# pyranha-labs/hypergrep

Measured on AMD Instinct MI355X. Metric: GiB/s scanned (256 patterns, 32 GiB synthetic log per GPU, text resident in HBM), higher is better.
Workload: dtype u8

## Files before the change

hypergrep_amd/csrc/hg_always_on.hip:

```cpp
#include <hip/hip_runtime.h>

#include "hg_confirm_dev.h"
#include "hg_core.h"
#include "hg_engine.h"
#include "hg_sink_dev.h"
#include "hg_tables_dev.h"

namespace {

__device__ __forceinline__ uint32_t wave_inclusive_scan(uint32_t v, uint32_t lane) {
#pragma unroll
  for (int o = 1; o < 64; o <<= 1) {
    uint32_t u = __shfl_up(v, o, 64);
    if (lane >= static_cast<uint32_t>(o)) v += u;
  }
  return v;
}

}

__global__ __launch_bounds__(256) void hg_always_on_kernel(HgConfirmArgs a, uint32_t first, uint32_t last) {
  __shared__ uint32_t s_n, s_base;
  if (threadIdx.x == 0) s_n = 0;
  __syncthreads();
  const uint64_t seg0 = static_cast<uint64_t>(blockIdx.x) * a.hit_seg_cap;
  const HitSink sink{a.tmp_hits + seg0, a.tmp_aux + seg0, a.hit_seg_cap, &s_n};
  const uint32_t lane = threadIdx.x & 63u;
  const uint64_t waves = (static_cast<uint64_t>(gridDim.x) * blockDim.x) >> 6;
  for (uint64_t tile = a.tile_begin + ((static_cast<uint64_t>(blockIdx.x) * blockDim.x + threadIdx.x) >> 6); tile < a.tile_end; tile += waves) {
    const uint64_t lo = (tile << HG_TILE_SHIFT) + lane * 256ull;
    uint64_t hi = lo + 256;
    if (hi > a.nbytes) hi = a.nbytes;
    uint32_t cnt = 0;
    for (uint64_t s = lo; s < hi; s++) cnt += a.text[s] == '\n';
    uint32_t rank = wave_inclusive_scan(cnt, lane) - cnt;
    for (uint64_t s = lo; s < hi; s++) {
      const bool starts = s == 0 || a.text[s - 1] == '\n';
      if (starts)
        hg_scan_line_always_on(a.db, a.text, a.nbytes, a.sums, a.bases, a.bs1, s, rank, first, last,
                               [&](uint32_t pi, uint64_t line_no, uint32_t to, uint64_t start, uint32_t len) {
                                 sink.push(a, line_no, a.db.patterns[pi].id, to, start, len, pi, a.db.patterns[pi].single != 0);
                               });
      rank += a.text[s] == '\n';
    }
  }
  flush_hits(a, &s_n, &s_base);
}

struct AlwaysOnCtx {
  const uint8_t *text;
  uint64_t nbytes;
  HgDeferred *list;
  uint32_t list_cap;
  hgdev::lds_u32 *list_count;
};
__device__ __forceinline__ void always_on_note(const AlwaysOnCtx &cx, uint32_t pi, uint64_t end, uint32_t rank_at_last) {
  const uint32_t slot = __hip_atomic_fetch_add(cx.list_count, 1u, __ATOMIC_RELAXED, __HIP_MEMORY_SCOPE_WORKGROUP);
  if (slot < cx.list_cap) cx.list[slot] = HgDeferred{end, pi, rank_at_last};
}

template <int NW, bool SIMPLE>
__device__ __forceinline__ void always_on_segment(const AlwaysOnCtx &a, const HgPattern &p, uint32_t pi, const hgdev::lds_u32 *tab, uint64_t lo, uint64_t hi,
                                                  uint64_t line_start, uint64_t bs1, uint32_t rank_lo) {
  if (lo >= hi) return;
  const hgdev::lds_u32 *reach = tab + CT_REACH, *follow = tab + CT_FOLLOW, *amask = tab + CT_AMASK, *acct = tab + CT_ACC;
  const uint8_t *text = a.text;
  uint64_t q = line_start;
  if (p.max_len && p.max_len <= HG_ALWAYS_ON_FAST_MAX_LEN) {
    const uint32_t lead = p.max_len - 1;
    q = lo > lead ? lo - lead : 0;
  } else if (lo - line_start >= bs1) {
    q = line_start + (lo - line_start) / bs1 * bs1;
  }
  const uint64_t base = q & ~15ull;
  const uint32_t first = static_cast<uint32_t>(q - base), own = static_cast<uint32_t>(lo - base), stop = static_cast<uint32_t>(hi - base);
  const bool text_ends = hi >= a.nbytes;
  uint32_t S[NW], I[NW];
#pragma unroll
  for (int u = 0; u < NW; u++) { S[u] = 0; I[u] = SIMPLE ? p.init_word : tab[CT_INIT + u]; }
  uint32_t pc = HG_PC_START;
  if (q) {
    const uint32_t before = text[q - 1];
    pc = (before == '\n' || before == 0) ? HG_PC_START : hg_prev_ctx(before);
  }
  constexpr uint32_t NO_BREAK = 0xFFFFFFFFu;
  uint32_t next_break = NO_BREAK;
  auto break_after = [&](uint64_t piece_start) {
    const uint64_t at = piece_start + bs1 - base;
    return at < 0x7FFFFFFFull ? static_cast<uint32_t>(at) : NO_BREAK;
  };
  if (q >= line_start) {
    const uint64_t d = q - line_start, k = d < bs1 ? 0 : d / bs1;
    next_break = break_after(line_start + k * bs1);
    if (k && d == k * bs1) pc = HG_PC_START;
  }
  uint32_t rank = rank_lo;
  bool reported = false;
  const bool single = p.single != 0;
  const uint32_t acc_all = p.acc_all;
  auto load16 = [&](uint32_t at) { return (at <= stop && base + at < a.nbytes) ? *reinterpret_cast<const uint4 *>(text + base + at) : make_uint4(0, 0, 0, 0); };
  uint4 chunk = make_uint4(0, 0, 0, 0), ahead = load16(0);
#pragma unroll 1
  for (uint32_t off = 0; off <= stop; off += 4) {
    if ((off & 15u) == 0) {
      chunk = ahead;
      ahead = load16(off + 16);
    }
    const uint32_t sel = (off >> 2) & 3u;
    const uint32_t v = sel == 0 ? chunk.x : (sel == 1 ? chunk.y : (sel == 2 ? chunk.z : chunk.w));
    uint32_t rc[4][NW];
#pragma unroll
    for (uint32_t i = 0; i < 4; i++)
#pragma unroll
      for (int u = 0; u < NW; u++) rc[i][u] = reach[((v >> (8 * i)) & 0xFFu) * NW + u];
#pragma unroll
    for (uint32_t i = 0; i < 4; i++) {
      const uint32_t r = off + i;
      if (r < first || r > stop) continue;
      const bool beyond = r == stop;
      const uint32_t c = (beyond && text_ends) ? 0u : ((v >> (8 * i)) & 0xFFu);
      if (r == next_break) {
        if (!SIMPLE) {
// ... 697 lines not shown
#pragma unroll
          for (uint32_t k = 0; k < 4; k++) {
            const uint32_t at = b + 16 * k;
            uint32_t m = hgdev::eq_mask16(v[k], 0x0a0a0a0au);
            if (at + 16 > seg) m &= at < seg ? (1u << (seg - at)) - 1u : 0u;
            cnt += __popc(m);
            if (m) after_last = seg_off + at + (31 - __clz(m)) + 1;
          }
        }
      }
      rank_lo = wave_inclusive_scan(cnt, lane) - cnt;
      const HgTileBase tb = a.bases[tile];
      uint32_t prev = after_last;
#pragma unroll
      for (int o = 1; o < 64; o <<= 1) {
        const uint32_t up = __shfl_up(prev, o, 64);
        if (lane >= static_cast<uint32_t>(o) && up > prev) prev = up;
      }
      prev = __shfl_up(prev, 1, 64);
      if (lane == 0) prev = 0;
      line_start = prev ? tile_start + prev : tb.cs;
    }
    for (uint32_t u = 0; u < nunits; u++) {
      if (!one_unit) {
        __syncthreads();
        always_on_stage(tab, a, u, threadIdx.x);
        __syncthreads();
      }
      if (!have) continue;
      AoUnit unit;
      bool ctx;
      if (u < ngroups) {
        const HgSlowGroup &g = a.db.groups[u];
        unit = AoUnit{g.init_word, g.acc_all, g.max_len, g.nmembers, g.single_mask, g.nnodes};
        ctx = g.ctx_off != 0;
      } else {
        const uint32_t pi = a.db.slow[a.db.nslow_grouped + (u - ngroups)];
        const HgPattern &p = a.db.patterns[pi];
        if (!p.simple && p.nw != 1) {
          always_on_word2(cx, p, pi, tab, lo, hi, line_start, a.bs1, rank_lo);
          continue;
        }
        unit = AoUnit{p.init_word, p.acc_all, p.max_len, 1u, p.single ? 1u : 0u, p.nnodes};
        ctx = !p.simple;
      }
      const uint32_t nt = (unit.nnodes + 7u) >> 3;
      const bool shift_form = nt >= 2 && tab[CT_SHIFT] <= 2u;
      if (shift_form) {
        if (ctx) always_on_word<true, 0>(cx, unit, tab, lo, hi, line_start, a.bs1, rank_lo);
        else always_on_word<false, 0>(cx, unit, tab, lo, hi, line_start, a.bs1, rank_lo);
      } else if (ctx) {
        if (nt <= 1) always_on_word<true, 1>(cx, unit, tab, lo, hi, line_start, a.bs1, rank_lo);
        else if (nt == 2) always_on_word<true, 2>(cx, unit, tab, lo, hi, line_start, a.bs1, rank_lo);
        else if (nt == 3) always_on_word<true, 3>(cx, unit, tab, lo, hi, line_start, a.bs1, rank_lo);
        else always_on_word<true, 4>(cx, unit, tab, lo, hi, line_start, a.bs1, rank_lo);
      } else {
        if (nt <= 1) always_on_word<false, 1>(cx, unit, tab, lo, hi, line_start, a.bs1, rank_lo);
        else if (nt == 2) always_on_word<false, 2>(cx, unit, tab, lo, hi, line_start, a.bs1, rank_lo);
        else if (nt == 3) always_on_word<false, 3>(cx, unit, tab, lo, hi, line_start, a.bs1, rank_lo);
        else always_on_word<false, 4>(cx, unit, tab, lo, hi, line_start, a.bs1, rank_lo);
      }
    }
  }
  __syncthreads();
  if (threadIdx.x == 0) {
    const uint32_t n = s_n;
    a.always_count[blockIdx.x] = n < list_cap ? n : list_cap;
    if (n > list_cap) atomicMax(&a.counters[HG_CNT_DEFER_NEED], static_cast<uint32_t>((static_cast<uint64_t>(n) * gridDim.x + HG_DEFER_SHARDS - 1) / HG_DEFER_SHARDS));
  }
}

__global__ __launch_bounds__(256) void hg_always_on_finish_kernel(HgConfirmArgs a) {
  __shared__ uint32_t s_n, s_base;
  if (threadIdx.x == 0) s_n = 0;
  __syncthreads();
  const uint64_t seg0 = static_cast<uint64_t>(blockIdx.x) * a.hit_seg_cap;
  const HitSink sink{a.tmp_hits + seg0, a.tmp_aux + seg0, a.hit_seg_cap, &s_n};
  const HgDeferred *list = a.deferred + static_cast<uint64_t>(blockIdx.x) * a.always_list_cap;
  const uint32_t n = a.always_count[blockIdx.x];
  for (uint32_t i = threadIdx.x; i < n; i += blockDim.x) {
    const HgDeferred d = list[i];
    const uint64_t end = d.pos, pos = end - 1;
    hgdev::PieceView pv;
    if (!hgdev::piece_view(a.text, a.nbytes, a.sums, a.bases, a.bs1, pos, d.rank, pos, &pv)) continue;
    if (!pv.whole) {
      if (pv.a > pos) continue;
      bool blocked = false;
      for (uint64_t i = pv.a; i < pos && !blocked; i++) blocked = a.text[i] == 0;
      if (blocked) continue;
    }
    const uint64_t z = a.text[pos] == '\n' ? end : hgdev::scanned_end(a.text, end, pv.limit);
    const HgPattern &pat = a.db.patterns[d.pattern];
    sink.push(a, pv.line_no, pat.id, static_cast<uint32_t>(end - pv.a), pv.a, static_cast<uint32_t>(z - pv.a), d.pattern, pat.single != 0);
  }
  flush_hits(a, &s_n, &s_base);
}
```

hypergrep_amd/csrc/hg_confirm_dev.h:

```cpp
#pragma once
#include <hip/hip_runtime.h>

#include "hg_core.h"

namespace hgdev {

using lds_u32 = __attribute__((address_space(3))) uint32_t;

__device__ __forceinline__ uint32_t load_u32_unaligned(const uint8_t *text, uint64_t off) {
  const uint32_t *p = reinterpret_cast<const uint32_t *>(text + (off & ~3ull));
  const uint32_t sh = static_cast<uint32_t>(off & 3u) * 8u;
  const uint32_t lo = p[0];
  if (sh == 0) return lo;
  return (lo >> sh) | (p[1] << (32u - sh));
}

__device__ __forceinline__ uint32_t byte_of(const uint4 &v, uint32_t i) {
  const uint32_t w = i < 8 ? (i < 4 ? v.x : v.y) : (i < 12 ? v.z : v.w);
  return (w >> ((i & 3u) * 8u)) & 0xFFu;
}
__device__ __forceinline__ uint32_t eq_mask16(const uint4 &v, uint32_t c4) {
  const uint32_t m0 = hg_zero_bytes(v.x ^ c4), m1 = hg_zero_bytes(v.y ^ c4), m2 = hg_zero_bytes(v.z ^ c4), m3 = hg_zero_bytes(v.w ^ c4);
#ifdef HG_EQMASK_BITWISE
  auto pack = [](uint32_t m) { return ((m >> 7) & 1u) | ((m >> 14) & 2u) | ((m >> 21) & 4u) | ((m >> 28) & 8u); };
// ... 36 lines not shown
      uint64_t c = base + 16u * j;
      if (c < chunk || c >= end) c = chunk;
      v[j] = *reinterpret_cast<const uint4 *>(text + c);
    }
#pragma unroll
    for (int j = 0; j < 4; j++) {
      const uint64_t c = base + 16u * j;
      if (c < chunk) continue;
      if (c >= end) return;
      if (visit(c, v[j])) return;
    }
    chunk = base + 64u;
  }
}

__device__ __forceinline__ uint64_t line_start_in_tile(const uint8_t *text, uint64_t tile_start, uint64_t pos) {
  uint64_t s = tile_start;
  walk_back4(text, (pos - 1) & ~15ull, tile_start, [&](uint64_t chunk, const uint4 &v) {
    uint32_t m = eq_mask16(v, 0x0a0a0a0au);
    if (chunk + 16 > pos) m &= (1u << static_cast<uint32_t>(pos - chunk)) - 1u;
    if (!m) return false;
    s = chunk + (31 - __clz(m)) + 1;
    return true;
  });
  return s;
}

__device__ __forceinline__ uint64_t scanned_end(const uint8_t *text, uint64_t from, uint64_t limit) {
  uint64_t z = limit;
  walk_fwd4(text, from & ~15ull, limit, [&](uint64_t chunk, const uint4 &v) {
    const uint32_t lo = chunk < from ? static_cast<uint32_t>(from - chunk) : 0u;
    const uint32_t hi = limit - chunk < 16 ? static_cast<uint32_t>(limit - chunk) : 16u;
    const uint32_t range = ((1u << hi) - 1u) & ~((1u << lo) - 1u);
    const uint32_t nl = eq_mask16(v, 0x0a0a0a0au) & range, nul = eq_mask16(v, 0u) & range;
    if (!(nl | nul)) return false;
    const uint32_t e = __ffs(nl | nul) - 1;
    z = chunk + (((nl >> e) & 1u) ? e + 1 : e);
    return true;
  });
  return z;
}

struct LineHead {
  uint64_t s;
  uint64_t a;
  bool blocked;
};
__device__ __forceinline__ LineHead line_head(const uint8_t *text, uint64_t tile_start, uint64_t carry_start, uint32_t rank, uint64_t upto) {
  const uint64_t floor = rank == 0 ? carry_start : tile_start;
  LineHead h{floor, upto, false};
  bool nul_above = false;
  if (upto > floor) {
    walk_back4(text, (upto - 1) & ~15ull, floor & ~15ull, [&](uint64_t chunk, const uint4 &v) {
      const uint32_t hi = upto - chunk < 16 ? static_cast<uint32_t>(upto - chunk) : 16u;
      uint32_t range = (1u << hi) - 1u;
      if (chunk < floor) range &= ~((1u << static_cast<uint32_t>(floor - chunk)) - 1u);
      bool stop = false;
      if (rank > 0) {
        const uint32_t nl = eq_mask16(v, 0x0a0a0a0au) & range;
        if (nl) {
          const uint32_t q = 31 - __clz(nl);
          h.s = chunk + q + 1;
          range &= ~((2u << q) - 1u);
          stop = true;
        }
      }
      const uint32_t zero = eq_mask16(v, 0u);
      const uint32_t nul = zero & range, data = ~zero & range;
      if (data) {
        if (nul_above || (nul && (data & ((1u << (31 - __clz(nul))) - 1u)))) h.blocked = true;
        h.a = chunk + (__ffs(data) - 1);
      }
      if (nul) nul_above = true;
      return stop || (h.blocked && rank == 0);
    });
  }
  return h;
}

struct PieceView {
  uint64_t line_no, a, limit;
  bool whole;
};
__device__ __forceinline__ bool piece_view(const uint8_t *text, uint64_t nbytes, const HgTileSum *sums, const HgTileBase *bases, uint64_t bs1, uint64_t pos,
                                           uint32_t rank, uint64_t upto, PieceView *out) {
  const uint64_t t = pos >> HG_TILE_SHIFT, tile_start = t << HG_TILE_SHIFT;
  const HgTileBase tb = bases[t];
  const LineHead h = line_head(text, tile_start, tb.cs, rank, upto);
  const uint64_t k = (pos - h.s) / bs1;
  const uint64_t ps = h.s + k * bs1;
  out->limit = ps + bs1 < nbytes ? ps + bs1 : nbytes;
  out->line_no = hg_line_index(text, sums[t], tb, tile_start, rank, h.s, bs1, bs1 < HG_TILE_BYTES) + k;
  out->whole = k == 0;
  if (k == 0) {
    if (h.blocked) return false;
    out->a = h.a;
    return true;
  }
  uint64_t a = ps;
  while (a < out->limit && text[a] == 0) a++;
  out->a = a;
  return a < out->limit;
}

template <typename Emit>
__device__ __forceinline__ void confirm_literal(const uint8_t *text, uint64_t nbytes, const HgTileSum *sums, const HgTileBase *bases, uint64_t bs1,
                                                uint64_t pos, uint32_t rank, uint64_t fs, uint32_t len, Emit &&emit) {
  const uint32_t last_byte = text[fs + len - 1];
  PieceView pv;
  if (!piece_view(text, nbytes, sums, bases, bs1, pos, rank, fs, &pv)) return;
  const uint64_t from = fs + len;
  if (from > pv.limit) return;
  uint64_t a = pv.a;
  if (!pv.whole) {
    if (a > fs) return;
    for (uint64_t i = a; i < fs; i++)
      if (text[i] == 0) return;
  }
  const uint64_t z = last_byte == '\n' ? from : scanned_end(text, from, pv.limit);
  emit(pv.line_no, static_cast<uint32_t>(from - a), a, static_cast<uint32_t>(z - a));
}

struct MatchWindow {
  uint64_t line_no, a, limit, q;
  uint32_t pc;
};
__device__ __forceinline__ bool match_window(const uint8_t *text, uint64_t nbytes, const HgTileSum *sums, const HgTileBase *bases, uint64_t bs1, uint64_t pos,
                                             uint32_t rank, uint64_t fs, uint32_t lead, MatchWindow *w) {
  PieceView pv;
  if (!piece_view(text, nbytes, sums, bases, bs1, pos, rank, pos, &pv)) return false;
  if (!pv.whole) {
    if (pv.a > pos) return false;
    for (uint64_t i = pv.a; i < pos; i++)
      if (text[i] == 0) return false;
  }
  if (fs < pv.a) return false;
  w->line_no = pv.line_no;
  w->a = pv.a;
  w->limit = pv.limit;
  w->q = (lead != 0xFFFFFFFFu && fs - pv.a > lead) ? fs - lead : pv.a;
  w->pc = w->q == pv.a ? static_cast<uint32_t>(HG_PC_START) : hg_prev_ctx(text[w->q - 1]);
  return true;
}
__device__ __forceinline__ uint64_t window_scanned_end(const uint8_t *text, uint64_t e, uint64_t limit) {
  return text[e - 1] == '\n' ? e : scanned_end(text, e, limit);
}

template <typename Emit>
__device__ __forceinline__ void confirm_simple(const uint8_t *text, uint64_t nbytes, const HgTileSum *sums, const HgTileBase *bases, uint64_t bs1, uint64_t pos,
                                                   uint32_t rank, uint64_t fs, uint32_t lead, uint32_t init, uint32_t acc, const lds_u32 *reach, const lds_u32 *follow,
                                                   Emit &&emit) {
  MatchWindow w;
  if (!match_window(text, nbytes, sums, bases, bs1, pos, rank, fs, lead, &w)) return;
  const uint64_t a = w.a, limit = w.limit, q = w.q;
  uint32_t S = 0, first_to = HG_NONE32;
  bool alive = true;
  for (uint64_t chunk = q & ~15ull; chunk < limit && alive; chunk += 16) {
    const uint4 v = *reinterpret_cast<const uint4 *>(text + chunk);
    const uint32_t lo = chunk < q ? static_cast<uint32_t>(q - chunk) : 0u;
    const uint32_t hi = limit - chunk < 16 ? static_cast<uint32_t>(limit - chunk) : 16u;
    const uint32_t below_lo = (1u << lo) - 1u;
    const uint32_t nl = eq_mask16(v, 0x0a0a0a0au) & ~below_lo, nul = eq_mask16(v, 0u) & ~below_lo;
    uint32_t end = hi;
    bool stop = false;
    const uint32_t stops = (nl | nul) & ((1u << hi) - 1u);
    if (stops) {
      const uint32_t e = __ffs(stops) - 1;
      end = ((nl >> e) & 1u) ? e + 1 : e;
      stop = true;
    }
    uint32_t r[16];
#pragma unroll
    for (int i = 0; i < 16; i++) r[i] = reach[byte_of(v, i)];
#pragma unroll
    for (int i = 0; i < 16; i++) {
      if (static_cast<uint32_t>(i) >= lo && static_cast<uint32_t>(i) < end && alive) {
        const uint64_t at = chunk + i;
        uint32_t T = at <= fs ? init : 0u;
        for (uint32_t x = S; x; x &= x - 1) T |= follow[__ffs(x) - 1];
        S = T & r[i];
        if (S & acc) {
          first_to = static_cast<uint32_t>(at + 1 - a);
          alive = false;
        } else if (S == 0 && at >= fs) {
          alive = false;
        }
      }
    }
    if (stop || hi < 16) break;
  }
  if (first_to != HG_NONE32) {
    const uint64_t z = window_scanned_end(text, a + first_to, limit);
    emit(w.line_no, first_to, a, static_cast<uint32_t>(z - a));
  }
}

template <int NW, typename Emit>
__device__ __forceinline__ void confirm_ctx(const uint8_t *text, uint64_t nbytes, const HgTileSum *sums, const HgTileBase *bases, uint64_t bs1, uint64_t pos,
                                                uint32_t rank, uint64_t fs, uint32_t lead, const lds_u32 *reach, const lds_u32 *follow, const lds_u32 *init,
                                                const lds_u32 *amask, const lds_u32 *acct, Emit &&emit) {
  MatchWindow w;
  if (!match_window(text, nbytes, sums, bases, bs1, pos, rank, fs, lead, &w)) return;
  const uint64_t a = w.a, limit = w.limit, q = w.q;
  uint32_t S[NW], I[NW];
#pragma unroll
  for (int u = 0; u < NW; u++) { S[u] = 0; I[u] = init[u]; }
  uint32_t pc = w.pc, first_to = HG_NONE32;
  bool alive = true;
  uint64_t z = limit;
  for (uint64_t chunk = q & ~15ull; chunk < limit && alive; chunk += 16) {
    const uint4 v = *reinterpret_cast<const uint4 *>(text + chunk);
    const uint32_t lo = chunk < q ? static_cast<uint32_t>(q - chunk) : 0u;
    const uint32_t hi = limit - chunk < 16 ? static_cast<uint32_t>(limit - chunk) : 16u;
    const uint32_t below_lo = (1u << lo) - 1u;
    const uint32_t nl = eq_mask16(v, 0x0a0a0a0au) & ~below_lo, nul = eq_mask16(v, 0u) & ~below_lo;
    uint32_t end = hi;
    bool stop = false;
    const uint32_t stops = (nl | nul) & ((1u << hi) - 1u);
    if (stops) {
      const uint32_t e = __ffs(stops) - 1;
      end = ((nl >> e) & 1u) ? e + 1 : e;
      stop = true;
    }
#pragma unroll
    for (int i = 0; i < 16; i++) {
      if (static_cast<uint32_t>(i) >= lo && static_cast<uint32_t>(i) < end && alive) {
        const uint64_t at = chunk + i;
        const uint32_t c = byte_of(v, i);
        const uint32_t cc = c == '\n' ? HG_NC_NLFINAL : (hg_is_word(c) ? HG_NC_WORD : HG_NC_OTHER);
        const lds_u32 *ac = acct + (pc * 5 + cc) * NW, *am = amask + (pc * 4 + cc) * NW, *rc = reach + c * NW;
        uint32_t hit = 0;
#pragma unroll
        for (int u = 0; u < NW; u++) hit |= S[u] & ac[u];
        if (hit) {
          first_to = static_cast<uint32_t>(at - a);
          alive = false;
        } else {
          uint32_t T[NW];
#pragma unroll
          for (int u = 0; u < NW; u++) T[u] = at <= fs ? I[u] : 0u;
#pragma unroll
          for (int u = 0; u < NW; u++)
            for (uint32_t x = S[u]; x; x &= x - 1) {
              const lds_u32 *f = follow + (u * 32 + (__ffs(x) - 1)) * NW;
#pragma unroll
              for (int k = 0; k < NW; k++) T[k] |= f[k];
            }
          uint32_t any = 0;
#pragma unroll
          for (int u = 0; u < NW; u++) any |= S[u] = T[u] & rc[u] & am[u];
          pc = hg_prev_ctx(c);
          if (any == 0 && at >= fs) alive = false;
        }
      }
    }
    if (stop || hi < 16) {
      z = chunk + end;
      break;
    }
  }
  if (first_to == HG_NONE32 && alive) {
    const lds_u32 *ac = acct + (pc * 5 + HG_NC_END) * NW;
    uint32_t hit = 0;
#pragma unroll
    for (int u = 0; u < NW; u++) hit |= S[u] & ac[u];
    if (hit) {
      first_to = static_cast<uint32_t>(z - a);
      emit(w.line_no, first_to, a, static_cast<uint32_t>(z - a));
    }
    return;
  }
  if (first_to != HG_NONE32) {
    const uint64_t e = a + first_to;
    emit(w.line_no, first_to, a, static_cast<uint32_t>((e > a ? window_scanned_end(text, e, limit) : scanned_end(text, e, limit)) - a));
  }
}

}
```

hypergrep_amd/csrc/hg_core.h:

```cpp
#pragma once
#include "hg_db.h"

constexpr uint32_t HG_TILE_BYTES = 16384;
constexpr uint32_t HG_TILE_SHIFT = 14;
constexpr uint32_t HG_NONE32 = 0xFFFFFFFFu;

struct HgTileSum {
  uint32_t nl_count;
  uint32_t first_nl;
  uint32_t last_nl;
  uint32_t inner;
};
struct HgTileBase {
  uint64_t cs;
  uint64_t L;
};
struct HgCand {
  uint64_t pos;
  uint32_t word;
  uint32_t rank;
};
struct HgHit {
  uint64_t line_no;
  uint32_t id;
  uint32_t to;
};
struct HgHitAux {
  uint64_t start;
  uint32_t len;
  uint32_t pattern;
};

struct HgDbView {
  const HgPattern *patterns;
  const uint32_t *pool;
  const HgFactor *factors;
  const HgWindow *windows;
  const uint32_t *bucket_off;
  const uint16_t *disc;
  const uint32_t *bucket_off2;
  const HgWindow *windows2;
  const HgWinBucket *wtab;
  uint32_t wtab_mask;
  uint32_t wtab_first;
  const uint32_t *slow;
  uint32_t npatterns, nslow, fold_mask;
  uint32_t window_mask;
  uint32_t nslow_fast;
  uint32_t nslow_grouped;
  uint32_t nslow_huge;
  uint32_t ngroups;
  const HgSlowGroup *groups;
  const uint32_t *bounds;
};

constexpr uint32_t HG_BOUND_NONE = 0x7FFFFFFFu;

HG_HD uint32_t hg_zero_bytes(uint32_t x) {
  uint32_t y = ((x & 0x7f7f7f7fu) + 0x7f7f7f7fu) | x;
  return ~y & 0x80808080u;
}
HG_HD uint32_t hg_newline_mask(uint32_t w) { return hg_zero_bytes(w ^ 0x0a0a0a0au); }

HG_HD uint32_t hg_popc(uint32_t x) {
#if defined(__HIP_DEVICE_COMPILE__)
  return __popc(x);
#else
  return static_cast<uint32_t>(__builtin_popcount(x));
#endif
}
HG_HD uint32_t hg_clz32(uint32_t x) {
#if defined(__HIP_DEVICE_COMPILE__)
  return static_cast<uint32_t>(__clz(static_cast<int>(x)));
#else
  return static_cast<uint32_t>(__builtin_clz(x));
#endif
}
HG_HD uint32_t hg_ctz(uint32_t x) {
#if defined(__HIP_DEVICE_COMPILE__)
  return __ffs(x) - 1;
#else
  return static_cast<uint32_t>(__builtin_ctz(x));
#endif
}

constexpr uint32_t HG_CONFIRM_MODES = 5;
HG_HD uint32_t hg_confirm_mode(const HgPattern &p) {
  if (p.nw > HG_MAX_W) return 4;
  if (p.single && p.literal_only) return 0;
  if (p.single && p.simple) return 1;
  if (p.single && p.nw <= 2) return 2;
  return 3;
}

HG_HD uint32_t hg_prev_ctx(uint32_t c) { return c == '\n' ? HG_PC_NL : (hg_is_word(c) ? HG_PC_WORD : HG_PC_OTHER); }

HG_HD void hg_disc_range(const HgDbView &db, const uint8_t *text, uint64_t nbytes, uint64_t pos, uint32_t folded, uint32_t *j0, uint32_t *j1) {
  const uint32_t h = hg_hash_window(folded);
  const uint32_t d = db.disc[h];
  const uint32_t sel = d >> 8;
  uint32_t key = 0;
  *j0 = *j1 = 0;
  if (sel) {
    const int64_t at = static_cast<int64_t>(pos) + static_cast<int8_t>(d & 0xFFu);
    const uint32_t lo = hg_ctz(sel), hi = 31u - hg_clz32(sel);
    if (at + static_cast<int64_t>(lo) < 0 || static_cast<uint64_t>(at + hi) >= nbytes) return;
    uint32_t v = 0;
    for (uint32_t b = lo; b <= hi; b++) v |= static_cast<uint32_t>(text[at + b]) << (8 * b);
    key = (v | db.fold_mask) & hg_disc_bytes(sel);
  }
  const uint32_t h2 = hg_disc_bucket(h, key);
  *j0 = db.bucket_off2[h2];
  *j1 = db.bucket_off2[h2 + 1];
}

template <typename Emit>
HG_HD void hg_verify_window(const HgDbView &db, const uint8_t *text, uint64_t nbytes, uint64_t pos, uint32_t w,
                            Emit &&emit) {
  uint32_t folded = (w | db.fold_mask) & db.window_mask;
  auto check = [&](uint32_t factor_off) {
    uint32_t off = factor_off & 0xff;
    const HgFactor &f = db.factors[factor_off >> 8];
    if (pos < off) return;
    uint64_t start = pos - off;
    if (start + f.len > nbytes) return;
    for (uint32_t b = 0; b < f.len; b++)
      if ((text[start + b] ^ f.lit[b]) & hg_factor_cmask(f, b)) return;
    emit(f.pattern, start, f.len);
  };
  const uint32_t owner = hg_wtab_find(db.wtab, db.wtab_mask, folded);
  if (owner == HG_WTAB_EMPTY) return;
  if (owner != HG_WTAB_SHARED) {
    check(owner);
    return;
  }
  uint32_t j0, j1;
  hg_disc_range(db, text, nbytes, pos, folded, &j0, &j1);
  for (uint32_t j = j0; j < j1; j++) {
    HgWindow win = db.windows2[j];
    if (win.value != folded) continue;
    check(win.factor_off);
  }
}

HG_HD uint64_t hg_pieces(uint64_t len, uint64_t bs1) { return (len + bs1 - 1) / bs1; }

HG_HD uint64_t hg_inner_pieces(const uint8_t *text, uint64_t from, uint64_t to, uint64_t bs1) {
  uint64_t total = 0, start = from;
  for (uint64_t i = from; i < to; i++)
    if (text[i] == '\n') {
      total += hg_pieces(i + 1 - start, bs1);
      start = i + 1;
    }
  return total;
}

HG_HD uint64_t hg_line_index(const uint8_t *text, const HgTileSum &ts, const HgTileBase &tb, uint64_t tile_start, uint32_t rank,
                             uint64_t s, uint64_t bs1, bool small) {
  if (rank == 0) return tb.L;
  uint64_t after_first = tile_start + ts.first_nl + 1;
  uint64_t base = tb.L + hg_pieces(after_first - tb.cs, bs1);
  if (!small) return base + (rank - 1);
  return base + hg_inner_pieces(text, after_first, s, bs1);
}

HG_HD void hg_trim_piece(const uint8_t *text, uint64_t ps, uint64_t limit, uint64_t &a, uint64_t &z) {
  a = ps;
  while (a < limit && text[a] == 0) a++;
  z = a;
  while (z < limit) {
    uint32_t c = text[z];
    if (c == 0) break;
    z++;
    if (c == '\n') break;
  }
}

struct HgHugeView {
  uint32_t nw, ncls, ctxfree, init_hi;
  const uint32_t *cls;
  const uint32_t *reach;
  const uint32_t *init, *smask, *xsrc, *xrank, *xlist, *xt;
  const uint32_t *amask;
  const uint32_t *acc;
};
HG_HD HgHugeView hg_huge_view(const uint32_t *pool, const HgPattern &p) {
  const HgHugeHeader *h = reinterpret_cast<const HgHugeHeader *>(pool + p.follow_off);
  HgHugeView v;
  v.nw = p.nw;
  v.ncls = h->ncls;
  v.ctxfree = h->ctxfree;
  v.init_hi = h->init_hi;
  v.cls = pool + h->cls_off;
  v.reach = pool + p.reach_off;
  v.init = pool + p.init_off;
  v.smask = pool + h->smask_off;
  v.xsrc = pool + h->xsrc_off;
  v.xrank = pool + h->xrank_off;
  v.xlist = pool + h->xlist_off;
  v.xt = pool + h->xt_off;
  v.amask = pool + p.amask_off;
  v.acc = pool + p.acc_off;
  return v;
}
HG_HD uint32_t hg_huge_class(const HgHugeView &v, uint32_t c) { return (v.cls[c >> 2] >> ((c & 3u) * 8u)) & 0xFFu; }
HG_HD const uint32_t *hg_huge_acc(const HgHugeView &v, uint32_t pc, uint32_t nc) { return v.ctxfree ? v.acc : v.acc + (pc * 5 + nc) * v.nw; }
HG_HD uint32_t hg_bits_from(uint32_t lo) { return 0xFFFFFFFFu << (lo & 31u); }
HG_HD uint32_t hg_bits_upto(uint32_t hi) { return 0xFFFFFFFFu >> (31u - (hi & 31u)); }

#if !defined(__HIP_DEVICE_COMPILE__)
template <typename Emit>
inline void hg_huge_scan_slice(const uint32_t *pool, const HgPattern &p, const uint8_t *data, uint64_t len, uint64_t from, uint64_t upto, Emit &&emit) {
  const HgHugeView v = hg_huge_view(pool, p);
  const uint32_t nw = v.nw;
  const bool single = p.single != 0;
  uint32_t *S = new uint32_t[2 * static_cast<size_t>(nw)](), *T = S + nw;
  uint32_t pc = from ? hg_prev_ctx(data[from - 1]) : HG_PC_START;
  bool alive = false;
  auto any_accept = [&](const uint32_t *a) {
    uint32_t any = 0;
    for (uint32_t w = 0; w < nw; w++) any |= S[w] & a[w];
    return any != 0;
  };
  for (uint64_t i = from; i < len; i++) {
    if (i >= upto && !alive) { delete[] S; return; }
    const uint32_t c = data[i];
    const uint32_t cc = c == '\n' ? (i + 1 == len ? HG_NC_NLFINAL : HG_NC_NL) : (hg_is_word(c) ? HG_NC_WORD : HG_NC_OTHER);
    if (alive && any_accept(hg_huge_acc(v, pc, cc))) {
      emit(static_cast<uint32_t>(i));
      if (single) { delete[] S; return; }
    }
    for (uint32_t w = 0; w < nw; w++) T[w] = i < upto ? v.init[w] : 0u;
    for (uint32_t w = 0; w < nw; w++) {
      const uint32_t x = S[w] & v.smask[w];
      T[w] |= x << 1;
      if (w + 1 < nw) T[w + 1] |= x >> 31;
    }
    for (uint32_t w = 0; w < nw; w++)
      for (uint32_t x = S[w] & v.xsrc[w]; x; x &= x - 1) {
        const uint32_t b = hg_ctz(x), k = v.xrank[w] + hg_popc(v.xsrc[w] & ((1u << b) - 1u));
        for (uint32_t r = v.xlist[k]; r < v.xlist[k + 1]; r++) {
          const uint32_t lo = v.xt[2 * r], hi = v.xt[2 * r + 1];
          for (uint32_t tw = lo >> 5; tw <= (hi >> 5); tw++)
            T[tw] |= (tw == (lo >> 5) ? hg_bits_from(lo) : 0xFFFFFFFFu) & (tw == (hi >> 5) ? hg_bits_upto(hi) : 0xFFFFFFFFu);
        }
      }
    const uint32_t *r = v.reach + hg_huge_class(v, c) * nw, *m = v.ctxfree ? nullptr : v.amask + (pc * 4 + cc) * nw;
// ... 404 lines not shown
}

template <typename Emit>
HG_HD uint32_t hg_flow_som_write(const uint32_t *pool, const HgPattern &p, const uint8_t *data, uint32_t len, bool close, uint32_t hdr, uint32_t *S,
                                 HgSomStarts *st, HgSomStarts *tmp, int32_t *carried, Emit &&emit) {
  uint32_t pc = hdr & HG_FLOW_PC;
  bool held = (hdr & HG_FLOW_HELD) != 0, acc_done = (hdr & HG_FLOW_ACC_DONE) != 0;
  int32_t stop = held ? -1 : 0;
  if (len > 0) {
    if (held) {
      hg_flow_som_unhold(pool, p, S, st, tmp, &pc, -1, false, acc_done, emit);
      acc_done = false;
    }
    const bool held_now = !close && data[len - 1] == '\n' && (hdr & HG_FLOW_HOLD);
    const uint32_t stop_w = held_now ? len - 1 : len;
    if (stop_w > 0) {
      hg_flow_som_scan(pool, p, data, 0, stop_w, close ? len - 1 : HG_NONE32, S, st, tmp, pc, acc_done, emit);
      pc = hg_prev_ctx(data[stop_w - 1]);
      acc_done = false;
    }
    held = held_now;
    stop = static_cast<int32_t>(stop_w);
  }
  *carried = stop;
  hdr = hg_flow_som_finish(pool, p, S, st, tmp, pc, hdr, stop, held, acc_done, close, emit);
  if (close) *carried = 0;
  return hdr;
}

HG_HD void hg_flow_som_load(const uint32_t *words, uint32_t width, const uint32_t *S, uint32_t nw, int64_t pos, HgSomStarts st) {
  for (uint32_t w = 0; w < nw; w++)
    for (uint32_t x = S[w]; x; x &= x - 1) {
      const uint32_t t = w * 32 + hg_ctz(x);
      uint64_t v;
      bool sat;
      if (width == 2) {
        v = (words[t >> 1] >> ((t & 1u) * 16u)) & 0xFFFFu;
        sat = v == 0xFFFFu;
      } else if (width == 4) {
        v = words[t];
        sat = v == 0xFFFFFFFFu;
      } else {
        v = words[2 * t] | (static_cast<uint64_t>(words[2 * t + 1]) << 32);
        sat = false;
      }
      st[t] = sat ? HG_SOM_FAR : pos - 1 - static_cast<int64_t>(v);
    }
}
HG_HD uint64_t hg_flow_som_dist(const uint32_t *S, HgSomStarts st, uint32_t t, int64_t pos, uint64_t sat) {
  if (!((S[t >> 5] >> (t & 31u)) & 1u)) return 0;
  if (st[t] == HG_SOM_FAR) return sat;
  const uint64_t d = static_cast<uint64_t>(pos - st[t] - 1);
  return d < sat ? d : sat;
}
HG_HD void hg_flow_som_store(uint32_t *words, uint32_t width, const uint32_t *S, uint32_t nnodes, int64_t pos, HgSomStarts st) {
  const uint32_t n = hg_flow_som_words(nnodes, width);
  for (uint32_t k = 0; k < n; k++) {
    uint32_t v;
    if (width == 2) {
      v = static_cast<uint32_t>(hg_flow_som_dist(S, st, 2 * k, pos, 0xFFFFu));
      if (2 * k + 1 < nnodes) v |= static_cast<uint32_t>(hg_flow_som_dist(S, st, 2 * k + 1, pos, 0xFFFFu)) << 16;
    } else if (width == 4) {
      v = static_cast<uint32_t>(hg_flow_som_dist(S, st, k, pos, 0xFFFFFFFFu));
    } else {
      v = static_cast<uint32_t>(hg_flow_som_dist(S, st, k >> 1, pos, ~0ull) >> ((k & 1u) * 32u));
    }
    words[k] = v;
  }
}

template <typename Emit>
HG_HD void hg_confirm_window(const HgDbView &db, const uint8_t *text, uint64_t nbytes, const HgTileSum *sums, const HgTileBase *bases, uint64_t bs1, uint64_t pos,
                             uint64_t fs, uint32_t pattern, uint32_t rank, Emit &&emit) {
  uint64_t t = pos >> HG_TILE_SHIFT, tile_start = t << HG_TILE_SHIFT;
  uint64_t s;
  if (rank == 0) {
    s = bases[t].cs;
  } else {
    s = pos;
    while (s > tile_start && text[s - 1] != '\n') s--;
  }
  uint64_t k = (pos - s) / bs1;
  uint64_t ps = s + k * bs1;
  uint64_t line_no = hg_line_index(text, sums[t], bases[t], tile_start, rank, s, bs1, bs1 < HG_TILE_BYTES) + k;
  uint64_t limit = ps + bs1 < nbytes ? ps + bs1 : nbytes;
  uint64_t a, z;
  hg_trim_piece(text, ps, limit, a, z);
  if (z <= a || pos < a || pos >= z || fs < a) return;
  const HgPattern &p = db.patterns[pattern];
  const uint64_t q = (p.lit_lead != 0xFFFFFFFFu && fs - a > p.lit_lead) ? fs - p.lit_lead : a;
  hg_nfa_scan_slice(db.pool, p, text + a, static_cast<uint32_t>(z - a), static_cast<uint32_t>(q - a), static_cast<uint32_t>(fs - a + 1),
                    [&](uint32_t to) { emit(line_no, to, a, static_cast<uint32_t>(z - a)); });
}

template <typename Emit, typename Claim>
HG_HD void hg_confirm(const HgDbView &db, const uint8_t *text, uint64_t nbytes, const HgTileSum *sums,
                      const HgTileBase *bases, uint64_t bs1, uint64_t pos, uint32_t pattern, uint32_t rank, Emit &&emit, Claim &&claim) {
  uint64_t t = pos >> HG_TILE_SHIFT, tile_start = t << HG_TILE_SHIFT;
  uint64_t s;
  if (rank == 0) {
    s = bases[t].cs;
  } else {
    s = pos;
    while (s > tile_start && text[s - 1] != '\n') s--;
  }
  uint64_t k = (pos - s) / bs1;
  uint64_t ps = s + k * bs1;
  uint64_t line_no = hg_line_index(text, sums[t], bases[t], tile_start, rank, s, bs1, bs1 < HG_TILE_BYTES) + k;
  uint64_t limit = ps + bs1 < nbytes ? ps + bs1 : nbytes;
  uint64_t a, z;
  hg_trim_piece(text, ps, limit, a, z);
  if (z <= a) return;
  if (!claim(ps)) return;
  const HgPattern &p = db.patterns[pattern];
  hg_nfa_scan(db.pool, p, text + a, z - a, [&](uint32_t to) { emit(line_no, to, a, static_cast<uint32_t>(z - a)); });
}
template <typename Emit>
HG_HD void hg_confirm(const HgDbView &db, const uint8_t *text, uint64_t nbytes, const HgTileSum *sums,
                      const HgTileBase *bases, uint64_t bs1, uint64_t pos, uint32_t pattern, uint32_t rank, Emit &&emit) {
  hg_confirm(db, text, nbytes, sums, bases, bs1, pos, pattern, rank, emit, [](uint64_t) { return true; });
}

template <typename Emit>
HG_HD void hg_scan_line_always_on(const HgDbView &db, const uint8_t *text, uint64_t nbytes, const HgTileSum *sums,
                                  const HgTileBase *bases, uint64_t bs1, uint64_t s, uint32_t rank, uint32_t first, uint32_t last, Emit &&emit) {
  uint64_t t = s >> HG_TILE_SHIFT, tile_start = t << HG_TILE_SHIFT;
  uint64_t line_no = hg_line_index(text, sums[t], bases[t], tile_start, rank, s, bs1, bs1 < HG_TILE_BYTES);
  uint64_t ps = s;
  for (;;) {
    uint64_t limit = ps + bs1 < nbytes ? ps + bs1 : nbytes;
    uint64_t a, z;
    hg_trim_piece(text, ps, limit, a, z);
    if (z > a) {
      for (uint32_t j = first; j < last; j++) {
        uint32_t pi = db.slow[j];
        hg_nfa_scan(db.pool, db.patterns[pi], text + a, z - a,
                    [&](uint32_t to) { emit(pi, line_no, to, a, static_cast<uint32_t>(z - a)); });
      }
    }
    uint64_t e = ps;
    bool nl = false;
    while (e < limit) {
      if (text[e++] == '\n') { nl = true; break; }
    }
    if (nl || e >= nbytes) return;
    ps = e;
    line_no++;
  }
}
```

hypergrep_amd/csrc/hg_engine.h:

```cpp
#pragma once
#include <hip/hip_runtime.h>

#include <memory>
#include <string>

#include "../../include/hypergrep_amd.h"
#include "hg_compile.h"
#include "hg_core.h"
#include "hg_post.h"

#ifndef HG_STREAM_WG_WAVES
#define HG_STREAM_WG_WAVES 8
#endif
constexpr uint32_t HG_STREAM_WG_WAVES_DEFAULT = HG_STREAM_WG_WAVES;

constexpr uint32_t HG_CONFIRM_SPLIT = 4;
constexpr uint32_t HG_DEFER_SHARDS = 64;

struct HgDeferred {
  uint64_t pos;
  uint32_t pattern;
  uint32_t rank;
};
enum { HG_ST_MINLEN_KEPT = 16, HG_ST_FIN_TOTAL = 24, HG_ST_SELECTED = 28, HG_ST_FINAL = 32, HG_ST_WORDS = 36, HG_ST_ZERO_WORDS = 32,
// ... 107 lines not shown
  uint32_t nfeed;
  uint32_t *count;
  const uint64_t *pos;
  HgHit *out_hits;
  HgHitAux *out_aux;
};
hipError_t hg_comb_launch(const HgCombArgs &a, bool emit, hipStream_t stream);

struct HgEngineKnobs {
  uint64_t fin_target = 48;
  bool no_bucket_finalize = false;
  uint64_t chunk_tiles = 0;
  uint32_t max_chunks = 0;
  std::vector<double> chunk_weights;
  long stream_wgs_per_cu = 0;
  long joiner = -1;
  bool joiner_ahead = false;
  bool no_early_finalize = false;
  uint32_t confirm_mode_mask = 0x1F;
  long confirm_blocks_per_cu = 0;
  uint64_t hit_limit = 0;
  uint64_t cand_limit = 0;
  bool verbose = false;
  static HgEngineKnobs from_env();
};

class HgScanner {
 public:
  static int create(std::shared_ptr<const HgDb> db, int device, HgScanner **out, std::string *err);
  const std::shared_ptr<const HgDb> &database() const { return db_; }
  ~HgScanner();
  int scan(const void *d_text, uint64_t nbytes, int buffer_size, uint64_t line_base, hipStream_t stream, HgScanOutput *out);
  int scan_block(const void *d_text, uint64_t nbytes, hipStream_t stream, HgScanOutput *out);
  uint32_t launch_block_small(const uint8_t *h_text, uint32_t nbytes, hipStream_t stream, HgHit *h_out, uint32_t *h_counts, uint32_t *h_flag, uint32_t seq);
  const std::string &last_error() const { return err_; }
  int device() const { return device_; }
  const HgDbView &view() const { return view_; }

 private:
  HgScanner() = default;
  int init();
  int ensure(uint64_t nbytes);
  int alloc_cands(uint64_t n);
  int alloc_hits(uint64_t n);
  int scan_impl(const void *d_text, uint64_t nbytes, int buffer_size, uint64_t line_base, bool block_mode, hipStream_t stream, HgScanOutput *out);
  struct PassRange {
    uint64_t tile_lo, tile_hi, cs0, piece0, own_lo, own_hi;
    bool last;
  };
  int scan_segments(const uint8_t *text, uint64_t nbytes, uint64_t bs1, uint64_t line_base, hipStream_t stream, HgScanOutput *out, uint32_t nsegments);
  int run_fitting(const uint8_t *text, uint64_t nbytes, uint64_t bs1, uint64_t line_base, const PassRange &range, bool block_mode, hipStream_t stream, HgScanOutput *out);
  int run_once(const uint8_t *text, uint64_t nbytes, uint64_t bs1, uint64_t line_base, const PassRange &range, bool block_mode, hipStream_t stream, HgScanOutput *out);
  struct PassPlan;
  PassPlan plan_pass(const uint8_t *text, uint64_t nbytes, uint64_t bs1, uint64_t line_base, const PassRange &range, bool block_mode, hipStream_t stream) const;
  int alloc_fin(uint32_t nb, hipStream_t stream);
  int launch_stream(PassPlan &p, uint32_t c, HgScanOutput *out);
  int launch_side(PassPlan &p, uint32_t c);
  int finalize_last(PassPlan &p, uint32_t c);
  int launch_fin(const PassPlan &p, hipStream_t s, uint32_t lo, uint32_t hi, bool beside_stream = false);
  int regrow(const PassPlan &p, uint64_t n_raw);
  int finalize_compact(const HgHit *hits, const HgHitAux *aux, uint32_t n, uint32_t id_bits, uint32_t to_bits, uint64_t line_bound, hipStream_t stream);
  int comb_pass(HgScanOutput *out, uint64_t bs1, uint64_t line_bound, hipStream_t stream);
  int minlen_pass(const uint8_t *text, uint32_t *n, hipStream_t stream);
  int huge_lds_error() { return error(HG_ERR_HIP, "the huge-automaton kernel cannot have its LDS"); }
  bool fail(hipError_t e, const char *what);
  int error(int rc, const std::string &what) { err_ = what; return rc; }

  HgEngineKnobs knobs_;
  int device_ = 0;
  int num_cus_ = 256;
  int stream_wgs_per_cu_ = 0;
  std::string err_;
  HgDbView view_{};
  std::shared_ptr<const HgDb> db_;
  void *d_disc_ = nullptr, *d_bucket2_ = nullptr, *d_windows2_ = nullptr, *d_groups_ = nullptr, *d_wtab_ = nullptr, *d_bounds_ = nullptr;
  void *d_patterns_ = nullptr, *d_pool_ = nullptr, *d_factors_ = nullptr, *d_windows_ = nullptr, *d_bucket_ = nullptr,
       *d_filter_ = nullptr, *d_ext_ = nullptr, *d_slow_ = nullptr;
  uint64_t cap_tiles_ = 0;
  uint32_t cand_cap_ = 0, hit_cap_ = 0;
  uint64_t chunk_limit_tiles_ = 0;
  uint32_t defer_spread_boost_ = 1;
  bool hit_direct_ = false;
  HgTileSum *d_sums_ = nullptr;
  HgTileBase *d_bases_ = nullptr, *d_block_base_ = nullptr, *d_final_ = nullptr;
  HgTileElem *d_agg_ = nullptr;
  HgCand *d_cands_ = nullptr;
  HgDeferred *d_deferred_ = nullptr;
  uint32_t *d_defer_count_ = nullptr;
  HgHit *d_hits_raw_ = nullptr, *d_hits_out_ = nullptr;
  HgHitAux *d_aux_raw_ = nullptr, *d_aux_out_ = nullptr;
  HgHit *d_acc_hits_ = nullptr;
  HgHitAux *d_acc_aux_ = nullptr;
  uint64_t acc_cap_ = 0;
  bool side_bound_ = false;
  uint64_t *d_key_a_ = nullptr, *d_key_b_ = nullptr;
  uint32_t *d_perm_a_ = nullptr, *d_perm_b_ = nullptr;
  uint8_t *d_keep_ = nullptr;
  uint32_t *d_counters_ = nullptr, *d_selected_ = nullptr, *d_seg_count_ = nullptr;
  uint32_t max_segs_ = 0;
  uint32_t *d_pflags_ = nullptr;
  void *d_temp_ = nullptr;
  size_t temp_bytes_ = 0;
  uint32_t *h_counters_ = nullptr;
  HgTileBase *h_final_ = nullptr;
  hipEvent_t ev_[4] = {nullptr, nullptr, nullptr, nullptr};
  static constexpr int kMaxChunks = 64;
  hipStream_t side_stream_ = nullptr;
  hipEvent_t ev_tile_done_ = nullptr;
  hipEvent_t ev_fin_early_ = nullptr;
  hipEvent_t ev_k1_begin_[kMaxChunks] = {}, ev_k1_end_[kMaxChunks] = {}, ev_side_done_[kMaxChunks] = {};
  uint32_t *d_fin_fill_ = nullptr, *d_fin_kept_ = nullptr, *d_fin_total_ = nullptr, *d_fin_big_ = nullptr;
  bool fin_fallback_ = false;
  uint32_t fin_alloc_ = 0;
  uint32_t fin_epoch_ = 0;
  uint64_t fin_expect_hits_ = 0;
  void *d_huge_claim_ = nullptr;
  uint64_t huge_claim_slots_ = 0;
  uint32_t *d_from_ = nullptr;
  uint64_t from_cap_ = 0;
  uint32_t som_max_nw_ = 0;
  uint32_t *d_min_lengths_ = nullptr;
  HgHit *d_minlen_hits_ = nullptr;
  HgHitAux *d_minlen_aux_ = nullptr;
  uint64_t minlen_cap_ = 0;
  uint32_t minlen_max_nw_ = 0;
  HgComb *d_combs_ = nullptr;
  uint32_t *d_comb_words_ = nullptr, *d_comb_feed_ = nullptr;
  uint32_t *d_comb_count_ = nullptr;
  uint64_t *d_comb_pos_ = nullptr;
  uint64_t comb_in_cap_ = 0;
  HgHit *d_comb_hits_ = nullptr;
  HgHitAux *d_comb_aux_ = nullptr;
  uint64_t comb_out_cap_ = 0;
  uint8_t *d_comb_temp_ = nullptr;
  size_t comb_temp_bytes_ = 0;
  uint32_t *d_seg_count2_ = nullptr;
  HgCand *d_cands2_ = nullptr;
};
```

hypergrep_amd/csrc/hg_engine.hip:

```cpp
#include <algorithm>
#include <array>
#include <cstdio>
#include <cstdlib>
#include <cstring>
#include <memory>

#include "hg_engine.h"
#include "hg_mem.h"

#include <rocprim/rocprim.hpp>

bool hg_launch_stream(const HgStreamArgs &a, uint32_t grid, hipStream_t stream);
bool hg_launch_stream_join(const HgStreamArgs &a, uint32_t grid, hipStream_t stream);
int hg_stream_blocks_per_cu(uint32_t filter_log2, uint32_t filter_wide, uint32_t dense);
__global__ void hg_tile_reduce_kernel(const HgTileSum *sums, uint64_t tile_begin, uint64_t tile_end, uint64_t bs1, HgTileElem *agg);
__global__ void hg_tile_spine_kernel(const HgTileElem *agg, uint32_t nblocks, uint64_t bs1, HgTileBase *block_base, HgTileBase *state);
__global__ void hg_tile_apply_kernel(const HgTileSum *sums, uint64_t tile_begin, uint64_t tile_end, uint64_t bs1, const HgTileBase *block_base,
                                     HgTileBase *bases);
__global__ void hg_tile_inner_kernel(const uint8_t *text, HgTileSum *sums, uint64_t tile_begin, uint64_t tile_end, uint64_t bs1);
__global__ void hg_verify_kernel(HgConfirmArgs a);
__global__ void hg_confirm_fast_kernel(HgConfirmArgs a, uint32_t blocks_per_mode);
__global__ void hg_confirm_generic_kernel(HgConfirmArgs a);
__global__ void hg_always_on_kernel(HgConfirmArgs a, uint32_t first, uint32_t last);
__global__ void hg_always_on_fast_kernel(HgConfirmArgs a);
__global__ void hg_always_on_finish_kernel(HgConfirmArgs a);
__global__ void hg_block_mark_kernel(HgConfirmArgs a, uint32_t *pattern_flags);
__global__ void hg_block_scan_kernel(HgConfirmArgs a, const uint32_t *pattern_flags);
__global__ void hg_block_small_kernel(HgDbView db, const uint8_t *h_text, uint32_t length, HgHit *h_out, uint32_t seg_cap, uint32_t *h_counts, uint32_t *d_done,
                                      uint32_t *h_flag, uint32_t seq, uint32_t ppw);
__global__ void hg_reset_kernel(uint32_t *state, uint32_t state_words, HgTileBase *final_state, uint64_t carry_start, uint64_t first_piece, uint32_t *fill, uint32_t nb, uint32_t *defer_count,
                                uint32_t ndefer);
__global__ void hg_fin_sort_small_kernel(const HgHit *hits, uint32_t *idx, const uint32_t *fill, uint32_t b_lo, uint32_t b_hi, uint32_t cap, uint32_t id_bits,
                                         uint32_t to_bits, uint32_t *kept_count, uint32_t *big_list, uint32_t *big_count, uint32_t big_stride);
template <uint32_t LCAP, bool IN_LDS>
__global__ void hg_fin_sort_big_kernel(const HgHit *hits, uint32_t *idx, const uint32_t *fill, const uint32_t *big_list, const uint32_t *big_count, uint32_t cap,
                                       uint32_t id_bits, uint32_t to_bits, uint32_t *kept_count, uint32_t *overflow, uint64_t *scratch_key, uint32_t *scratch_idx);
template <uint32_t THREADS>
__global__ void hg_fin_scan_kernel(uint32_t *kept_count, uint32_t b_lo, uint32_t b_hi, uint32_t *total, const uint32_t *fill, uint32_t cap, uint32_t *part, uint32_t epoch);
__global__ void hg_confirm_literal_kernel(HgConfirmArgs a);
__global__ void hg_verify_lean_kernel(HgConfirmArgs a);
__global__ void hg_fin_gather_kernel(const HgHit *hits, const HgHitAux *aux, const uint32_t *idx, const uint32_t *kept_base, const uint32_t *total, uint32_t b_lo,
                                     uint32_t b_hi, uint32_t cap, HgHit *oh, HgHitAux *oa);
__global__ void hg_key_kernel(const HgHit *hits, const HgHitAux *aux, const HgPattern *patterns, uint32_t n, uint64_t *key, uint32_t *idx);
__global__ void hg_line_key_kernel(const HgHit *hits, const uint32_t *perm, uint32_t n, uint64_t *key);
__global__ void hg_offset_kernel(uint32_t *idx, uint32_t n, uint32_t add);
__global__ void hg_key_packed_kernel(const HgHit *hits, const HgHitAux *aux, const HgPattern *patterns, uint32_t n, uint32_t id_bits, uint32_t to_bits,
                                     uint64_t *key, uint32_t *idx);
__global__ void hg_keep_kernel(const HgHit *hits, const HgHitAux *aux, const uint32_t *perm, const HgPattern *patterns, uint32_t n, uint8_t *keep);
__global__ void hg_scatter_kernel(const HgHit *hits, const HgHitAux *aux, const uint32_t *perm, const uint8_t *keep, const uint32_t *pos, uint32_t n,
                                  HgHit *oh, HgHitAux *oa, uint32_t *count);

size_t hg_huge_lds_bytes(uint32_t nw_max, uint32_t stage_cap);
bool hg_launch_confirm_huge(const HgConfirmArgs &a, uint32_t grid, uint32_t nw_max, uint32_t stage_cap, void *claim, uint32_t claim_mask, hipStream_t stream);
bool hg_launch_always_on_huge(const HgConfirmArgs &a, uint32_t grid, uint32_t nw_max, uint32_t stage_cap, uint32_t first, uint32_t last, hipStream_t stream);
bool hg_launch_block_huge(const HgConfirmArgs &a, uint32_t grid, uint32_t nw_max, uint32_t stage_cap, const uint32_t *pattern_flags, hipStream_t stream);

namespace {
constexpr int TS_BLOCK_TILES = 1024;
constexpr int STREAM_WG_WAVES = HG_STREAM_WG_WAVES;

template <typename T>
hipError_t upload(void **dst, const std::vector<T> &src, const char *name) {
  size_t bytes = std::max<size_t>(src.size() * sizeof(T), 16);
  hipError_t e = hgmem::dev_alloc(dst, bytes, name);
  if (e != hipSuccess) return e;
  if (!src.empty()) e = hipMemcpy(*dst, src.data(), src.size() * sizeof(T), hipMemcpyHostToDevice);
  return e;
}
template <typename T>
hipError_t realloc_dev(T *&ptr, size_t count, const char *name) {
  hgmem::dev_free(ptr, name);
  ptr = nullptr;
  return hgmem::dev_alloc(&ptr, std::max<size_t>(count * sizeof(T), 16), name);
}
uint32_t bits_for(uint64_t v) {
  uint32_t b = 1;
  while (b < 64 && (v >> b)) b++;
  return b;
}
}

#define HG_TRY(call, what) \
  do { if (fail((call), what)) return HG_ERR_HIP; } while (0)

HgEngineKnobs HgEngineKnobs::from_env() {
  HgEngineKnobs k;
  auto num = [](const char *name, uint64_t dflt) -> uint64_t {
    const char *env = std::getenv(name);
    return env ? std::strtoull(env, nullptr, 10) : dflt;
  };
  k.fin_target = std::max<uint64_t>(4, num("HG_FIN_TARGET", 48));
  k.no_bucket_finalize = std::getenv("HG_NO_BUCKET_FINALIZE") != nullptr;
  k.chunk_tiles = num("HG_CHUNK_TILES", 0);
  k.max_chunks = static_cast<uint32_t>(std::min<uint64_t>(num("HG_MAX_CHUNKS", 0), 1u << 20));
  if (const char *env = std::getenv("HG_CHUNK_WEIGHTS")) {
    for (const char *q = env; *q;) {
      char *e = nullptr;
      const double v = std::strtod(q, &e);
      if (e == q) break;
      if (v > 0) k.chunk_weights.push_back(v);
      q = *e ? e + 1 : e;
    }
  }
  k.stream_wgs_per_cu = static_cast<long>(num("HG_STREAM_WGS_PER_CU", 0));
  if (const char *env = std::getenv("HG_JOINER")) k.joiner = std::max(0l, std::min(2l, std::strtol(env, nullptr, 10)));
  k.joiner_ahead = std::getenv("HG_JOINER_AHEAD") != nullptr;
  k.no_early_finalize = std::getenv("HG_NO_EARLY_FINALIZE") != nullptr;
#ifdef HG_PROFILE_CONFIRM
  if (const char *env = std::getenv("HG_DEBUG_CONFIRM_MODES")) k.confirm_mode_mask = static_cast<uint32_t>(std::strtoul(env, nullptr, 0));
#endif
  k.confirm_blocks_per_cu = static_cast<long>(std::min<uint64_t>(num("HG_CONFIRM_BLOCKS_PER_CU", 0), 16));
  k.hit_limit = num("HG_HIT_LIMIT", 0);
  k.cand_limit = num("HG_CAND_LIMIT", 0);
// ... 4 lines not shown
bool HgScanner::fail(hipError_t e, const char *what) {
  if (e == hipSuccess) return false;
  err_ = std::string(what) + ": " + hipGetErrorString(e);
  return true;
}

int HgScanner::create(std::shared_ptr<const HgDb> db, int device, HgScanner **out, std::string *err) {
  *out = nullptr;
  std::unique_ptr<HgScanner> s(new HgScanner());
  s->device_ = device;
  s->db_ = std::move(db);
  if (int rc = s->init()) {
    if (err) *err = s->err_;
    return rc;
  }
  *out = s.release();
  return HG_OK;
}

int HgScanner::init() {
  if (!db_) return error(HG_ERR_ARG, "no database");
  int count = 0;
  const hipError_t e = hipGetDeviceCount(&count);
  if (e != hipSuccess || count == 0) return error(HG_ERR_HIP, std::string("no HIP device available (") + hipGetErrorString(e) + "); the scan path has no CPU fallback");
  if (device_ < 0 || device_ >= count) return error(HG_ERR_ARG, "device index out of range");
  knobs_ = HgEngineKnobs::from_env();
  const HgDb &db = *db_;
  HG_TRY(hipSetDevice(device_), "hipSetDevice");
  hipDeviceProp_t prop;
  HG_TRY(hipGetDeviceProperties(&prop, device_), "hipGetDeviceProperties");
  num_cus_ = prop.multiProcessorCount;
  HG_TRY(upload(&d_patterns_, db.patterns, "d_patterns_"), "upload patterns");
  HG_TRY(upload(&d_pool_, db.pool, "d_pool_"), "upload tables");
  HG_TRY(upload(&d_factors_, db.factors, "d_factors_"), "upload factors");
  HG_TRY(upload(&d_windows_, db.windows, "d_windows_"), "upload windows");
  HG_TRY(upload(&d_bucket_, db.bucket_off, "d_bucket_"), "upload buckets");
  HG_TRY(upload(&d_disc_, db.disc, "d_disc_"), "upload discriminators");
  HG_TRY(upload(&d_bucket2_, db.bucket_off2, "d_bucket2_"), "upload buckets");
  HG_TRY(upload(&d_windows2_, db.windows2, "d_windows2_"), "upload windows");
  HG_TRY(upload(&d_wtab_, db.wtab, "d_wtab_"), "upload window table");
  HG_TRY(upload(&d_filter_, db.filter, "d_filter_"), "upload filter");
  HG_TRY(upload(&d_ext_, db.ext, "d_ext_"), "upload filter conditions");
  HG_TRY(upload(&d_slow_, db.slow, "d_slow_"), "upload always-on list");
  HG_TRY(upload(&d_groups_, db.groups, "d_groups_"), "upload always-on groups");
  view_.patterns = static_cast<const HgPattern *>(d_patterns_);
  view_.pool = static_cast<const uint32_t *>(d_pool_);
  view_.factors = static_cast<const HgFactor *>(d_factors_);
  view_.windows = static_cast<const HgWindow *>(d_windows_);
  view_.bucket_off = static_cast<const uint32_t *>(d_bucket_);
  view_.disc = static_cast<const uint16_t *>(d_disc_);
  view_.bucket_off2 = static_cast<const uint32_t *>(d_bucket2_);
  view_.windows2 = static_cast<const HgWindow *>(d_windows2_);
  view_.wtab = static_cast<const HgWinBucket *>(d_wtab_);
  view_.wtab_mask = db.wtab_mask;
  view_.wtab_first = db.wtab_first;
  view_.slow = static_cast<const uint32_t *>(d_slow_);
  view_.npatterns = static_cast<uint32_t>(db.patterns.size());
  view_.nslow = static_cast<uint32_t>(db.slow.size());
  view_.nslow_fast = db.nslow_fast;
  view_.nslow_grouped = db.nslow_grouped;
  view_.nslow_huge = db.nslow_huge;
  view_.ngroups = static_cast<uint32_t>(db.groups.size());
  view_.groups = static_cast<const HgSlowGroup *>(d_groups_);
  if (!db.bounds.empty()) HG_TRY(upload(&d_bounds_, db.bounds, "d_bounds_"), "upload offset bounds");
  view_.bounds = static_cast<const uint32_t *>(d_bounds_);
  if (!db.min_lengths.empty()) HG_TRY(upload(reinterpret_cast<void **>(&d_min_lengths_), db.min_lengths, "d_min_lengths_"), "upload min_length");
  for (uint32_t i = 0; i < db.patterns.size(); i++) {
    const HgPattern &p = db.patterns[i];
    if (p.flags & HG_FLAG_SOM_LEFTMOST) som_max_nw_ = std::max(som_max_nw_, p.nw);
    if (!db.min_lengths.empty() && db.min_lengths[i]) minlen_max_nw_ = std::max(minlen_max_nw_, p.nw);
  }
  if (db.comb_pass()) {
    HG_TRY(upload(reinterpret_cast<void **>(&d_combs_), db.combs, "d_combs_"), "upload combinations");
    HG_TRY(upload(reinterpret_cast<void **>(&d_comb_words_), db.comb_words, "d_comb_words_"), "upload combinations");
    HG_TRY(upload(reinterpret_cast<void **>(&d_comb_feed_), db.comb_feed, "d_comb_feed_"), "upload combinations");
  }
  view_.fold_mask = db.fold_mask;
  view_.window_mask = db.window_mask;
  static_assert(HG_CNT_CURSORS == kMaxChunks, "one tile cursor per pipeline chunk");
  HG_TRY(hgmem::dev_alloc(&d_counters_, HG_ST_ALLOC_WORDS * 4, "d_state_"), "alloc state");
  HG_TRY(hipMemset(d_counters_, 0, HG_ST_ALLOC_WORDS * 4), "clear state");
  d_fin_total_ = d_counters_ + HG_ST_FIN_TOTAL;
  d_selected_ = d_counters_ + HG_ST_SELECTED;
  d_final_ = reinterpret_cast<HgTileBase *>(d_counters_ + HG_ST_FINAL);
  HG_TRY(hgmem::dev_alloc(&d_pflags_, db.patterns.size() * 4 + 16, "d_pflags_"), "alloc pattern flags");
  HG_TRY(hgmem::host_alloc(&h_counters_, (HG_CNT_WORDS + 4 + HG_DEFER_SHARDS) * 4, "h_counters_"), "alloc pinned");
  h_final_ = reinterpret_cast<HgTileBase *>(h_counters_ + HG_ST_FINAL);
  for (auto &ev : ev_) HG_TRY(hipEventCreate(&ev), "hipEventCreate");
  HG_TRY(hipStreamCreateWithFlags(&side_stream_, hipStreamNonBlocking), "hipStreamCreate");
  HG_TRY(hipEventCreateWithFlags(&ev_fin_early_, hipEventDisableTiming), "hipEventCreate");
  HG_TRY(hipEventCreateWithFlags(&ev_tile_done_, hipEventDisableTiming), "hipEventCreate");
  return HG_OK;
}

HgScanner::~HgScanner() {
  (void)hipSetDevice(device_);
  void *ptrs[] = {d_patterns_, d_pool_, d_factors_, d_windows_, d_bucket_, d_filter_, d_ext_, d_slow_, d_sums_, d_bases_, d_block_base_,
                  d_agg_, d_cands_, d_hits_raw_, d_hits_out_, d_aux_raw_, d_aux_out_,
                  d_key_a_, d_key_b_, d_perm_a_, d_perm_b_, d_keep_, d_counters_, d_temp_, d_seg_count_, d_pflags_, d_deferred_, d_defer_count_, d_seg_count2_, d_cands2_, d_disc_, d_bucket2_, d_windows2_, d_groups_, d_acc_hits_, d_acc_aux_, d_huge_claim_, d_wtab_, d_from_, d_fin_fill_, d_fin_kept_, d_fin_big_,
                  d_combs_, d_comb_words_, d_comb_feed_, d_comb_count_, d_comb_pos_, d_comb_hits_, d_comb_aux_, d_comb_temp_, d_bounds_,
                  d_min_lengths_, d_minlen_hits_, d_minlen_aux_};
  for (void *p : ptrs) hgmem::dev_free(p, "scanner");
  hgmem::host_free(h_counters_, "h_counters_");
  for (auto &ev : ev_)
    if (ev) (void)hipEventDestroy(ev);
  for (int i = 0; i < kMaxChunks; i++) {
    if (ev_k1_begin_[i]) (void)hipEventDestroy(ev_k1_begin_[i]);
    if (ev_k1_end_[i]) (void)hipEventDestroy(ev_k1_end_[i]);
    if (ev_side_done_[i]) (void)hipEventDestroy(ev_side_done_[i]);
  }
  if (side_stream_) (void)hipStreamDestroy(side_stream_);
  if (ev_fin_early_) (void)hipEventDestroy(ev_fin_early_);
  if (ev_tile_done_) (void)hipEventDestroy(ev_tile_done_);
}

int HgScanner::alloc_cands(uint64_t n) {
  n = std::min<uint64_t>(n, 0x7FFFFFF0u);
  HG_TRY(realloc_dev(d_cands_, n, "d_cands_"), "workspace alloc (candidates)");
  HG_TRY(realloc_dev(d_cands2_, n, "d_cands2_"), "workspace alloc (candidates)");
  uint32_t modes = 0;
  for (uint32_t m = 0; m < HG_CONFIRM_MODES; m++) modes += db_->n_confirm_mode[m] ? 1 : 0;
  HG_TRY(realloc_dev(d_deferred_, std::max<uint64_t>(modes, 1) * n, "d_deferred_"), "workspace alloc (deferred)");
  hgmem::dev_free(d_huge_claim_, "d_huge_claim_");
  d_huge_claim_ = nullptr;
  huge_claim_slots_ = 0;
  if (db_->n_confirm_mode[4]) {
    uint64_t slots = 1u << 12;
    while (slots < 2 * n) slots <<= 1;
    HG_TRY(hgmem::dev_alloc(&d_huge_claim_, slots * 8, "d_huge_claim_"), "workspace alloc (claim table)");
    huge_claim_slots_ = slots;
  }
  cand_cap_ = static_cast<uint32_t>(n);
  return HG_OK;
}

int HgScanner::alloc_hits(uint64_t n64) {
  const uint32_t n = static_cast<uint32_t>(std::min<uint64_t>(n64, 0x7FFFFFF0u));
  auto re = [&](auto *&ptr, size_t count, const char *name) { return fail(realloc_dev(ptr, count, name), "workspace alloc (hits)"); };
  if (re(d_hits_raw_, n, "d_hits_raw_") || re(d_hits_out_, n, "d_hits_out_") || re(d_aux_raw_, n, "d_aux_raw_") || re(d_aux_out_, n, "d_aux_out_") ||
      re(d_key_a_, n, "d_key_a_") || re(d_key_b_, n, "d_key_b_") || re(d_perm_a_, n, "d_perm_a_") || re(d_perm_b_, n, "d_perm_b_") || re(d_keep_, n, "d_keep_"))
    return HG_ERR_HIP;
  hit_cap_ = n;
  size_t t1 = 0, t2 = 0;
  (void)rocprim::radix_sort_pairs(nullptr, t1, d_key_a_, d_key_b_, d_perm_a_, d_perm_b_, n, 0, 64, hipStream_t(nullptr));
  (void)rocprim::exclusive_scan(nullptr, t2, d_keep_, d_perm_a_, 0u, n, rocprim::plus<uint32_t>(), hipStream_t(nullptr));
  size_t t3 = 0;
  (void)rocprim::merge(nullptr, t3, d_key_a_, d_key_a_, d_key_b_, d_perm_a_, d_perm_a_, d_perm_b_, n, n, rocprim::less<uint64_t>(), hipStream_t(nullptr));
  size_t need = std::max(std::max(t1, t2), t3) + 256;
  if (need > temp_bytes_) {
    hgmem::dev_free(d_temp_, "d_temp_");
    d_temp_ = nullptr;
    HG_TRY(hgmem::dev_alloc(&d_temp_, need, "d_temp_"), "workspace alloc (sort)");
    temp_bytes_ = need;
  }
  return HG_OK;
}

int HgScanner::ensure(uint64_t nbytes) {
  uint64_t ntiles = std::max<uint64_t>((nbytes + HG_TILE_BYTES - 1) / HG_TILE_BYTES, 1);
  auto re = [&](auto *&ptr, size_t count, const char *name) { return fail(realloc_dev(ptr, count, name), "workspace alloc"); };
  if (ntiles > cap_tiles_) {
    uint64_t nblocks = (ntiles + TS_BLOCK_TILES - 1) / TS_BLOCK_TILES;
    if (re(d_sums_, ntiles, "d_sums_") || re(d_bases_, ntiles + 1, "d_bases_") || re(d_agg_, nblocks, "d_agg_") || re(d_block_base_, nblocks, "d_block_base_")) return HG_ERR_HIP;
    cap_tiles_ = ntiles;
  }
  if (!d_seg_count_) {
    max_segs_ = static_cast<uint32_t>(num_cus_) * 16;
    if (re(d_seg_count_, max_segs_, "d_seg_count_") || re(d_seg_count2_, max_segs_, "d_seg_count2_") || re(d_defer_count_, HG_CONFIRM_MODES * HG_DEFER_SHARDS, "d_defer_count_")) return HG_ERR_HIP;
  }
  uint64_t want = std::max<uint64_t>(nbytes / 1024, 1u << 16);
// ... 85 lines not shown
  p.chunk_tiles = chunk_tiles;
  p.piped = nchunks > 1;
  p.side = p.piped ? side_stream_ : stream;

  if (ntiles) {
    uint32_t per_cu = p.piped ? std::max(1, stream_wgs_per_cu_ - 1) : stream_wgs_per_cu_;
    if (knobs_.stream_wgs_per_cu) {
      const long v = knobs_.stream_wgs_per_cu;
      if (v >= 1 && v <= stream_wgs_per_cu_) per_cu = static_cast<uint32_t>(v);
    }
    auto grid_for = [&](uint32_t wgs_per_cu) {
      return static_cast<uint32_t>(std::min<uint64_t>((std::min<uint64_t>(chunk_tiles, ntiles) + STREAM_WG_WAVES - 1) / STREAM_WG_WAVES,
                                                      std::min<uint64_t>(static_cast<uint64_t>(num_cus_) * wgs_per_cu, max_segs_)));
    };
    p.wgs_shared = grid_for(per_cu);
    p.wgs_alone = knobs_.stream_wgs_per_cu ? p.wgs_shared : grid_for(static_cast<uint32_t>(stream_wgs_per_cu_));
    p.joiner_wgs = (p.piped && stream_wgs_per_cu_ >= 3 && per_cu < static_cast<uint32_t>(stream_wgs_per_cu_) && chunk_limit_tiles_ == 0 && !side_bound_) ? static_cast<uint32_t>(num_cus_) : 0u;
    if (knobs_.joiner >= 0) p.joiner_wgs = p.piped ? static_cast<uint32_t>(knobs_.joiner) * static_cast<uint32_t>(num_cus_) : 0u;
    if (p.wgs_shared + p.joiner_wgs > max_segs_ || db_->filter_wide || db_->filter_log2 > 13) p.joiner_wgs = 0;
    p.wgs = std::max(p.wgs_shared + p.joiner_wgs, p.wgs_alone);
    for (uint32_t c = 0; c < std::min(nchunks, 2u); c++)
      p.cand_seg_cap[c] = static_cast<uint32_t>(static_cast<uint64_t>(cand_cap_) * 4 / (4ull * p.wgs_of(c) + p.joiners_of(c)));
  }
  HgStreamArgs &sa = p.sa;
  sa.text = text;
  sa.nbytes = nbytes;
  sa.db = view_;
  sa.filter = static_cast<const uint32_t *>(d_filter_);
  sa.filter_log2 = db_->filter_log2;
  sa.weights_a = db_->weights_a;
  sa.weights_b = db_->weights_b;
  sa.filter_wide = db_->filter_wide;
  sa.dense = db_->dense;
  sa.weights_c = db_->weights_c;
  sa.ext = static_cast<const HgSlotInfo *>(d_ext_);
  sa.sums = d_sums_;
  sa.counters = d_counters_;
  HgConfirmArgs &ca = p.ca;
  ca.text = text;
  ca.nbytes = nbytes;
  ca.bs1 = bs1;
  ca.db = view_;
  ca.sums = d_sums_;
  ca.bases = d_bases_;
  ca.hits = d_hits_raw_;
  ca.aux = d_aux_raw_;
  ca.tmp_hits = d_hits_out_;
  ca.tmp_aux = d_aux_out_;
  ca.hit_cap = hit_cap_;
  ca.hit_direct = hit_direct_ ? 1u : 0u;
  ca.bucket_shift = p.fin_shift;
  ca.counters = d_counters_;
  ca.own_lo = range.own_lo;
  ca.own_hi = range.own_hi;
  if (!block_mode && p.has_anchored) {
    const uint32_t mode_mask = knobs_.confirm_mode_mask;
    ca.deferred = d_deferred_;
    ca.defer_count = d_defer_count_;
    ca.defer_shard_cap = cand_cap_ / HG_DEFER_SHARDS;
    for (uint32_t m = 0, next = 0; m < HG_CONFIRM_MODES; m++) {
      ca.mode_present[m] = (db_->n_confirm_mode[m] && ((mode_mask >> m) & 1u)) ? 1 : 0;
      ca.list_of_mode[m] = db_->n_confirm_mode[m] ? next++ : 0;
      ca.list_spread[m] = std::min<uint32_t>(HG_DEFER_SHARDS, std::max<uint32_t>(1, HG_DEFER_SHARDS / std::max<uint32_t>(1, db_->n_confirm_mode[m])) * defer_spread_boost_);
    }
  }
  return p;
}

int HgScanner::alloc_fin(uint32_t nb, hipStream_t stream) {
  uint32_t want = 1u << 16;
  while (want < nb) want <<= 1;
  fin_alloc_ = 0;
  HG_TRY(realloc_dev(d_fin_fill_, want, "d_fin_fill_"), "alloc finalize buckets");
  HG_TRY(realloc_dev(d_fin_kept_, want, "d_fin_kept_"), "alloc finalize buckets");
  HG_TRY(realloc_dev(d_fin_big_, 2 * static_cast<size_t>(want) + 3 * 128, "d_fin_big_"), "alloc finalize buckets");
  HG_TRY(hipMemsetAsync(d_fin_big_ + 2 * static_cast<size_t>(want), 0, 3 * 128 * 4, stream), "clear scan flags");
  fin_alloc_ = want;
  return HG_OK;
}

int HgScanner::launch_fin(const PassPlan &p, hipStream_t s, uint32_t lo, uint32_t hi, bool beside_stream) {
  if (hi <= lo) return HG_OK;
  const uint32_t nbk = hi - lo, cu = static_cast<uint32_t>(num_cus_), fin_cap = p.fin_cap, id_bits = p.id_bits, to_bits = p.to_bits;
  HG_TRY(hipMemsetAsync(d_fin_total_ + 2, 0, 8, s), "memset work list");
  hipLaunchKernelGGL(hg_fin_sort_small_kernel, dim3(std::min<uint32_t>((nbk + 3) / 4, cu * 8)), dim3(256), 0, s, d_hits_raw_, d_perm_a_, d_fin_fill_, lo, hi, fin_cap, id_bits, to_bits,
                     d_fin_kept_, d_fin_big_, d_fin_total_ + 2, fin_alloc_);
  hipLaunchKernelGGL((hg_fin_sort_big_kernel<HG_FIN_MEDIUM_CAP, true>), dim3(std::min<uint32_t>(nbk, cu * 4)), dim3(256), 0, s, d_hits_raw_, d_perm_a_, d_fin_fill_, d_fin_big_, d_fin_total_ + 2,
                     fin_cap, id_bits, to_bits, d_fin_kept_, d_selected_ + 1, static_cast<uint64_t *>(nullptr), static_cast<uint32_t *>(nullptr));
  const uint32_t big_blocks = std::min<uint32_t>(std::min<uint32_t>(nbk, 64u), hit_cap_ / HG_FIN_BUCKET_CAP);
  if (big_blocks)
    hipLaunchKernelGGL((hg_fin_sort_big_kernel<HG_FIN_BUCKET_CAP, false>), dim3(big_blocks), dim3(256), 0, s, d_hits_raw_, d_perm_a_, d_fin_fill_, d_fin_big_ + fin_alloc_,
                       d_fin_total_ + 3, fin_cap, id_bits, to_bits, d_fin_kept_, d_selected_ + 1, d_key_a_, d_perm_b_);
  const uint32_t scan_blocks = std::max<uint32_t>(1, std::min<uint32_t>(128, (nbk + 8191) / 8192));
  uint32_t *part = d_fin_big_ + 2 * static_cast<size_t>(fin_alloc_);
  const uint32_t epoch = ++fin_epoch_ ? fin_epoch_ : ++fin_epoch_;
  if (beside_stream) hipLaunchKernelGGL(hg_fin_scan_kernel<512u>, dim3(scan_blocks), dim3(512), 0, s, d_fin_kept_, lo, hi, d_fin_total_, d_fin_fill_, fin_cap, part, epoch);
  else hipLaunchKernelGGL(hg_fin_scan_kernel<1024u>, dim3(scan_blocks), dim3(1024), 0, s, d_fin_kept_, lo, hi, d_fin_total_, d_fin_fill_, fin_cap, part, epoch);
  hipLaunchKernelGGL(hg_fin_gather_kernel, dim3(std::min<uint32_t>((nbk + 3) / 4, cu * 8)), dim3(256), 0, s, d_hits_raw_, d_aux_raw_, d_perm_a_, d_fin_kept_, d_fin_total_, lo, hi, fin_cap,
                     d_hits_out_, d_aux_out_);
  HG_TRY(hipGetLastError(), "finalize launch");
  return HG_OK;
}

int HgScanner::launch_stream(PassPlan &p, uint32_t c, HgScanOutput *out) {
  const uint32_t wgs_c = p.wgs_of(c), joiners_c = p.joiners_of(c);
  HgStreamArgs sa = p.sa;
  sa.tile_begin = p.cut[c];
  sa.tile_end = p.cut[c + 1];
  sa.cursor_slot = HG_CNT_CURSOR0 + c;
  sa.cands = p.set_of(c) ? d_cands2_ : d_cands_;
  sa.seg_count = p.set_of(c) ? d_seg_count2_ : d_seg_count_;
  sa.cand_seg_cap = p.cand_seg_cap[c ? 1 : 0];
  sa.alone = (c == 0 && wgs_c == p.wgs_alone && !knobs_.stream_wgs_per_cu) ? 1u : 0u;
  HgStreamArgs ja = sa;
  ja.cands = sa.cands + static_cast<uint64_t>(wgs_c) * sa.cand_seg_cap;
  ja.cand_seg_cap = sa.cand_seg_cap / 4;
  ja.seg_count = sa.seg_count + wgs_c;
  ja.alone = 0;
  auto launch_joiner = [&](hipStream_t s) -> int {
    if (!hg_launch_stream_join(ja, joiners_c, s)) return HG_ERR_ARG;
    out->joiner_launches++;
    HG_TRY(hipGetLastError(), "hg_stream_kernel launch (joiner)");
    return HG_OK;
  };
  HG_TRY(hipEventRecord(p.piped ? ev_k1_begin_[c] : ev_[1], p.stream), "event");
  if (joiners_c && knobs_.joiner_ahead)
    if (int rc = launch_joiner(p.stream)) return rc;
  if (!hg_launch_stream(sa, wgs_c, p.stream)) return error(HG_ERR_ARG, "no stream kernel for this database's filter size / mode");
  HG_TRY(hipGetLastError(), "hg_stream_kernel launch");
  HG_TRY(hipEventRecord(p.piped ? ev_k1_end_[c] : ev_[2], p.stream), "event");
  if (p.piped && p.bucketed && joiners_c && c + 1 == p.nchunks && !knobs_.no_early_finalize) {
    const uint32_t lim = p.settled_buckets(c);
    if (lim > p.fin_done) {
      if (int rc = launch_fin(p, p.side, p.fin_done, lim, true)) return rc;
      p.fin_done = lim;
    }
  }
  if (joiners_c && !knobs_.joiner_ahead)
    if (int rc = launch_joiner(p.side)) return rc;
  if (p.piped) HG_TRY(hipStreamWaitEvent(p.side, ev_k1_end_[c], 0), "stream wait");
  return HG_OK;
}

int HgScanner::launch_side(PassPlan &p, uint32_t c) {
  const uint64_t t0 = p.cut[c], t1 = p.cut[c + 1];
  const uint32_t segs_c = p.wgs_of(c) + p.joiners_of(c);
  const hipStream_t side = p.side;
  HgConfirmArgs ca = p.ca;
  ca.tile_begin = t0;
  ca.tile_end = t1;
  uint32_t *seg_count = p.set_of(c) ? d_seg_count2_ : d_seg_count_;
  ca.cands = p.set_of(c) ? d_cands2_ : d_cands_;
  ca.seg_count = seg_count;
  ca.cand_seg_cap = p.cand_seg_cap[c ? 1 : 0];
  ca.join_seg0 = p.wgs_of(c);
  ca.join_seg_cap = ca.cand_seg_cap / 4;
  uint32_t confirm_blocks = 1, always_blocks = 1;
  if (p.block_mode) {
    HG_TRY(hipMemsetAsync(d_pflags_, 0, db_->patterns.size() * 4, side), "memset pattern flags");
    if (p.has_anchored) hipLaunchKernelGGL(hg_block_mark_kernel, dim3(segs_c), dim3(256), 0, side, ca, d_pflags_);
    always_blocks = std::max<uint32_t>(static_cast<uint32_t>((db_->patterns.size() + 255) / 256), std::min<uint32_t>(db_->nhuge, 1024u));
    ca.hit_seg_cap = hit_cap_ / always_blocks;
    hipLaunchKernelGGL(hg_block_scan_kernel, dim3(static_cast<uint32_t>((db_->patterns.size() + 255) / 256)), dim3(256), 0, side, ca, d_pflags_);
    if (db_->nhuge && !hg_launch_block_huge(ca, std::min<uint32_t>(db_->nhuge, 1024u), db_->huge_max_nw, db_->huge_stage_words, d_pflags_, side)) return huge_lds_error();
    HG_TRY(hipGetLastError(), "block-mode launch");
    p.stage_blocks = std::max(confirm_blocks, always_blocks);
    return HG_OK;
  }
  const uint64_t span = t1 - t0;
  const uint32_t nblocks = static_cast<uint32_t>((span + TS_BLOCK_TILES - 1) / TS_BLOCK_TILES);
  if (p.bs1 < HG_TILE_BYTES) {
    uint32_t blocks = static_cast<uint32_t>(std::min<uint64_t>((span + 255) / 256, 4096));
    hipLaunchKernelGGL(hg_tile_inner_kernel, dim3(blocks), dim3(256), 0, side, p.text, d_sums_, t0, t1, p.bs1);
  }
  hipLaunchKernelGGL(hg_tile_reduce_kernel, dim3(nblocks), dim3(256), 0, side, d_sums_, t0, t1, p.bs1, d_agg_);
  hipLaunchKernelGGL(hg_tile_spine_kernel, dim3(1), dim3(256), 0, side, d_agg_, nblocks, p.bs1, d_block_base_, d_final_);
  hipLaunchKernelGGL(hg_tile_apply_kernel, dim3(nblocks), dim3(256), 0, side, d_sums_, t0, t1, p.bs1, d_block_base_, d_bases_);
  HG_TRY(hipGetLastError(), "tile scan launch");
  if (p.piped && c + 1 == p.nchunks) HG_TRY(hipEventRecord(ev_tile_done_, side), "event");
  if (p.has_anchored) {
    const uint32_t verify_blocks = segs_c * HG_CONFIRM_SPLIT;
    uint32_t fast_modes = 0;
    const uint32_t mode_mask = knobs_.confirm_mode_mask;
    for (uint32_t m = 0; m < 3; m++) fast_modes += (db_->n_confirm_mode[m] && ((mode_mask >> m) & 1u)) ? 1 : 0;
    uint32_t per_cu = c + 1 == p.nchunks ? 6 : 3;
    if (knobs_.confirm_blocks_per_cu) per_cu = static_cast<uint32_t>(knobs_.confirm_blocks_per_cu);
    const uint32_t mode_blocks = std::max<uint32_t>(HG_DEFER_SHARDS, static_cast<uint32_t>(num_cus_) * per_cu * (256 / HG_CONFIRM_THREADS));
    const uint32_t huge_blocks = db_->n_confirm_mode[4] ? std::max<uint32_t>(HG_DEFER_SHARDS, static_cast<uint32_t>(num_cus_) * static_cast<uint32_t>(std::max<size_t>(1, std::min<size_t>(8, (160u << 10) / std::max<size_t>(hg_huge_lds_bytes(db_->huge_max_nw, db_->huge_stage_words), 1))))) : 0u;
    confirm_blocks = std::max(std::max(mode_blocks * std::max(fast_modes, 1u), verify_blocks), huge_blocks);
    ca.hit_seg_cap = hit_cap_ / confirm_blocks;
    if (c > 0) HG_TRY(hipMemsetAsync(d_defer_count_, 0, HG_CONFIRM_MODES * HG_DEFER_SHARDS * 4, side), "memset deferred counts");
    if (ca.mode_present[1] || ca.mode_present[2]) hipLaunchKernelGGL(hg_verify_kernel, dim3(verify_blocks), dim3(256), 0, side, ca);
    else hipLaunchKernelGGL(hg_verify_lean_kernel, dim3(verify_blocks), dim3(256), 0, side, ca);
    const bool literal_only_set = ca.mode_present[0] && !ca.mode_present[1] && !ca.mode_present[2];
    if (literal_only_set) {
      hipLaunchKernelGGL(hg_confirm_literal_kernel, dim3(mode_blocks), dim3(256), 0, side, ca);
    } else if (fast_modes) {
      hipLaunchKernelGGL(hg_confirm_fast_kernel, dim3(mode_blocks * fast_modes), dim3(HG_CONFIRM_THREADS), 0, side, ca, mode_blocks);
    }
    if (db_->n_confirm_mode[3]) hipLaunchKernelGGL(hg_confirm_generic_kernel, dim3(mode_blocks), dim3(256), 0, side, ca);
    if (huge_blocks && ((mode_mask >> 4) & 1u)) {
      HG_TRY(hipMemsetAsync(d_huge_claim_, 0, huge_claim_slots_ * 8, side), "memset claim table");
      if (!hg_launch_confirm_huge(ca, huge_blocks, db_->huge_max_nw, db_->huge_stage_words, d_huge_claim_, static_cast<uint32_t>(huge_claim_slots_ - 1), side)) return huge_lds_error();
    }
    HG_TRY(hipGetLastError(), "confirm launch");
  }
  if (!db_->slow.empty()) {
    always_blocks = static_cast<uint32_t>(std::min<uint64_t>((span + 3) / 4, static_cast<uint64_t>(num_cus_) * 8));
    const uint32_t huge_always_blocks = db_->nslow_huge ? static_cast<uint32_t>(std::min<uint64_t>(span, static_cast<uint64_t>(num_cus_) * 16)) : 0u;
    ca.hit_seg_cap = hit_cap_ / std::max(always_blocks, huge_always_blocks);
    const uint32_t nfast = db_->nslow_fast, nhuge = db_->nslow_huge, nall = static_cast<uint32_t>(db_->slow.size()) - nhuge;
    if (nfast) {
      ca.deferred = d_deferred_;
      ca.always_count = seg_count;
      ca.always_list_cap = cand_cap_ / always_blocks;
      hipLaunchKernelGGL(hg_always_on_fast_kernel, dim3(always_blocks), dim3(256), 0, side, ca);
      hipLaunchKernelGGL(hg_always_on_finish_kernel, dim3(always_blocks), dim3(256), 0, side, ca);
    }
    if (nall > nfast) hipLaunchKernelGGL(hg_always_on_kernel, dim3(always_blocks), dim3(256), 0, side, ca, nfast, nall);
    if (nhuge && !hg_launch_always_on_huge(ca, huge_always_blocks, db_->huge_max_nw, db_->huge_stage_words, nall, nall + nhuge, side)) return huge_lds_error();
    always_blocks = std::max(always_blocks, huge_always_blocks);
    HG_TRY(hipGetLastError(), "hg_always_on_kernel launch");
  }
  p.stage_blocks = std::max(confirm_blocks, always_blocks);
  return HG_OK;
}

int HgScanner::finalize_last(PassPlan &p, uint32_t c) {
  bool fin_early = false;
  if (p.piped && c >= 1 && !knobs_.no_early_finalize) {
    const uint32_t lim = p.settled_buckets(c);
    if (lim > p.fin_done) {
      HG_TRY(hipStreamWaitEvent(p.stream, ev_side_done_[c - 1], 0), "stream wait");
      HG_TRY(hipStreamWaitEvent(p.stream, ev_tile_done_, 0), "stream wait");
      if (int rc = launch_fin(p, p.stream, p.fin_done, lim)) return rc;
      HG_TRY(hipEventRecord(ev_fin_early_, p.stream), "event");
      p.fin_done = lim;
      fin_early = true;
    }
  }
  if (fin_early) HG_TRY(hipStreamWaitEvent(p.side, ev_fin_early_, 0), "stream wait");
  return launch_fin(p, p.side, p.fin_done, p.fin_nb);
}

int HgScanner::regrow(const PassPlan &p, uint64_t n_raw) {
  const bool block_mode = p.block_mode, bucketed = p.bucketed;
  const uint64_t cand_need = h_counters_[HG_CNT_CAND_NEED], hit_need = h_counters_[HG_CNT_HIT_NEED];
  const uint64_t defer_need = h_counters_[HG_CNT_DEFER_NEED];
  const bool fin_overflow = bucketed && h_counters_[HG_ST_SELECTED + 1] != 0;
  uint64_t kHitLimit = 1ull << 28;
  if (knobs_.hit_limit) kHitLimit = std::max<uint64_t>(1u << 10, knobs_.hit_limit);
  if (!block_mode && (n_raw > kHitLimit || h_counters_[HG_CNT_HITS_WRAPPED])) return HG_SPLIT;
  if (!(cand_need || defer_need || hit_need || fin_overflow || (!bucketed && n_raw > hit_cap_))) return HG_OK;
  if (cand_need || defer_need) {
    if (defer_need && defer_spread_boost_ < HG_DEFER_SHARDS) defer_spread_boost_ *= 4;
    uint64_t want = std::max<uint64_t>((cand_need + cand_need / 4 + 64) * p.wgs, (defer_need + defer_need / 4 + 64) * HG_DEFER_SHARDS);
    want = std::max<uint64_t>(want, static_cast<uint64_t>(cand_cap_) * 2);
    uint64_t kCandLimit = 1ull << 30;
    if (knobs_.cand_limit) kCandLimit = std::max<uint64_t>(1u << 16, knobs_.cand_limit);
    if (want > kCandLimit) {
      const uint64_t cur = (std::min<uint64_t>(p.chunk_tiles, p.ntiles) + TS_BLOCK_TILES - 1) / TS_BLOCK_TILES * TS_BLOCK_TILES;
      if (block_mode || cur <= TS_BLOCK_TILES) return error(HG_ERR_ARG, "the candidate limit is below what one 16 MiB chunk of this text produces");
      chunk_limit_tiles_ = std::max<uint64_t>(TS_BLOCK_TILES, cur / 2 / TS_BLOCK_TILES * TS_BLOCK_TILES);
      want = std::min<uint64_t>(want / 2, kCandLimit);
    }
    if (want > cand_cap_)
      if (int rc = alloc_cands(want)) return rc;
  }
  if (bucketed && (hit_need || fin_overflow)) {
    const uint64_t want = (hit_need + hit_need / 4 + 16) * p.fin_nb;
    fin_expect_hits_ = std::max<uint64_t>(fin_expect_hits_ * 2, n_raw);
    if (fin_overflow || hit_need > HG_FIN_BUCKET_CAP || want > (128ull << 20)) {
      fin_fallback_ = true;
    } else if (int rc = alloc_hits(std::max<uint64_t>(want, static_cast<uint64_t>(hit_cap_) * 2))) {
// ... 338 lines not shown
```

hypergrep_amd/csrc/hg_huge.hip:

```cpp
#include <hip/hip_runtime.h>

#include <algorithm>

#include "hg_core.h"
#include "hg_engine.h"
#include "hg_sink_dev.h"

namespace {

__device__ __forceinline__ uint32_t wave_max_u32(uint32_t v) {
#pragma unroll
  for (int o = 32; o; o >>= 1) {
    const uint32_t u = static_cast<uint32_t>(__shfl_xor(static_cast<int>(v), o, 64));
    v = u > v ? u : v;
  }
  return v;
}

template <typename Pred>
__device__ __forceinline__ uint64_t wave_find(const uint8_t *text, uint64_t from, uint64_t limit, uint32_t lane, Pred &&pred) {
  for (uint64_t base = from; base < limit; base += 64) {
    const uint64_t p = base + lane;
    const bool hit = p < limit && pred(static_cast<uint32_t>(text[p]));
    const uint64_t m = __builtin_amdgcn_ballot_w64(hit);
// ... 228 lines not shown
      s[k] = nx[k] & r[k] & m[k];
      live |= s[k];
    }
    alive = __builtin_amdgcn_ballot_w64(live != 0) != 0;
    pc = hg_prev_ctx(c);
  }
  if (alive) {
    uint32_t any = 0;
#pragma unroll
    for (int k = 0; k < K; k++) {
      const uint32_t w = lane + 64u * k, wc = w < nw ? w : 0u;
      any |= s[k] & (v.ctxfree ? c_acc[k] : t.acc[(pc * 5 + HG_NC_END) * nw + wc]);
    }
    if (__builtin_amdgcn_ballot_w64(any != 0) && lane == 0) emit(static_cast<uint32_t>(len));
  }
}

struct HugeUnit {
  HgHugeView v;
  HugeStaged t;
  uint32_t k;
};
__device__ __forceinline__ HugeUnit huge_prepare(const HgHugeView &view, uint32_t *stage, uint32_t cap_words, uint32_t lane) {
  HugeUnit u;
  const bool fits = huge_stage_words(view) <= cap_words;
  u.v = huge_stage(view, stage, cap_words, lane);
  u.k = 0;
  u.t = HugeStaged{nullptr, nullptr, nullptr, nullptr};
  if (fits && view.nw <= 256u) {
    u.k = view.nw <= 64u ? 1u : (view.nw <= 128u ? 2u : 4u);
    const lds_u32 *base = (const lds_u32 *)stage;
    u.t.cls = base;
    u.t.reach = base + 64u;
    u.t.acc = base + 64u + view.nw * (view.ncls + 4u);
    u.t.amask = u.t.acc + (view.ctxfree ? 1u : 20u) * view.nw;
  }
  return u;
}
template <typename Emit>
__device__ __forceinline__ void huge_run_unit(const HugeUnit &u, uint32_t *S, uint32_t *T, const uint8_t *data, uint64_t len, bool single, uint32_t lane, Emit &&emit) {
  if (u.k == 1) huge_run_reg<1>(u.v, u.t, (lds_u32 *)T, data, len, 0, len, single, lane, emit);
  else if (u.k == 2) huge_run_reg<2>(u.v, u.t, (lds_u32 *)T, data, len, 0, len, single, lane, emit);
  else if (u.k == 4) huge_run_reg<4>(u.v, u.t, (lds_u32 *)T, data, len, 0, len, single, lane, emit);
  else huge_run(u.v, S, T, data, len, 0, len, single, lane, emit);
}

__device__ __forceinline__ bool claim_piece(unsigned long long *table, uint32_t mask, uint64_t ps, uint32_t pattern) {
  const unsigned long long key = ((static_cast<unsigned long long>(ps) << 24) | pattern) + 1ull;
  uint32_t h = static_cast<uint32_t>((key * 0x9E3779B97F4A7C15ull) >> 32) & mask;
  for (;;) {
    const unsigned long long old = atomicCAS(&table[h], 0ull, key);
    if (old == 0ull) return true;
    if (old == key) return false;
    h = (h + 1u) & mask;
  }
}

extern __shared__ uint32_t s_dyn[];

__global__ __launch_bounds__(64) void hg_confirm_huge_kernel(HgConfirmArgs a, uint32_t nw_max, uint32_t stage_cap, unsigned long long *claim, uint32_t claim_mask) {
  __shared__ uint32_t s_n, s_base;
  if (threadIdx.x == 0) s_n = 0;
  __syncthreads();
  uint32_t *S = s_dyn, *T = s_dyn + nw_max;
  const uint32_t lane = threadIdx.x;
  const uint64_t seg0 = static_cast<uint64_t>(blockIdx.x) * a.hit_seg_cap;
  const HitSink sink{a.tmp_hits + seg0, a.tmp_aux + seg0, a.hit_seg_cap, &s_n};
  constexpr uint32_t MODE = 4;
  uint32_t staged_pattern = HG_NONE32;
  HugeUnit unit{};
  const uint32_t shard = blockIdx.x % HG_DEFER_SHARDS, peer = blockIdx.x / HG_DEFER_SHARDS, peers = (gridDim.x + HG_DEFER_SHARDS - 1 - shard) / HG_DEFER_SHARDS;
  const HgDeferred *dlist = a.deferred + (static_cast<uint64_t>(a.list_of_mode[MODE]) * HG_DEFER_SHARDS + shard) * a.defer_shard_cap;
  uint32_t n = a.defer_count[MODE * HG_DEFER_SHARDS + shard];
  if (n > a.defer_shard_cap) n = a.defer_shard_cap;
  for (uint32_t i = peer; i < n; i += peers) {
    const HgDeferred d = dlist[i];
    const uint32_t pattern = d.pattern & (HG_MAX_PATTERNS - 1u);
    const uint64_t pos = d.pos, t = pos >> HG_TILE_SHIFT, tile_start = t << HG_TILE_SHIFT;
    const uint64_t s = d.rank == 0 ? a.bases[t].cs : wave_line_start(a.text, tile_start, pos, lane);
    const uint64_t k = (pos - s) / a.bs1, ps = s + k * a.bs1;
    uint32_t mine = 0;
    if (lane == 0) mine = claim_piece(claim, claim_mask, ps, pattern) ? 1u : 0u;
    if (!__builtin_amdgcn_readfirstlane(mine)) continue;
    const uint64_t line_no = hg_line_index(a.text, a.sums[t], a.bases[t], tile_start, d.rank, s, a.bs1, a.bs1 < HG_TILE_BYTES) + k;
    const uint64_t limit = ps + a.bs1 < a.nbytes ? ps + a.bs1 : a.nbytes;
    uint64_t pa, pz;
    wave_trim_piece(a.text, ps, limit, lane, pa, pz);
    if (pz <= pa) continue;
    const HgPattern &p = a.db.patterns[pattern];
    if (pattern != staged_pattern) {
      __syncthreads();
      unit = huge_prepare(hg_huge_view(a.db.pool, p), s_dyn + 2 * nw_max, stage_cap, lane);
      staged_pattern = pattern;
    }
    const uint32_t id = p.id, len = static_cast<uint32_t>(pz - pa);
    const bool single = p.single != 0;
    huge_run_unit(unit, S, T, a.text + pa, len, single, lane, [&](uint32_t to) { sink.push(a, line_no, id, to, pa, len, pattern, single); });
  }
  flush_hits(a, &s_n, &s_base);
}

__global__ __launch_bounds__(64) void hg_always_on_huge_kernel(HgConfirmArgs a, uint32_t nw_max, uint32_t stage_cap, uint32_t first, uint32_t last) {
  __shared__ uint32_t s_n, s_base;
  if (threadIdx.x == 0) s_n = 0;
  __syncthreads();
  uint32_t *S = s_dyn, *T = s_dyn + nw_max;
  const uint32_t lane = threadIdx.x;
  const uint64_t seg0 = static_cast<uint64_t>(blockIdx.x) * a.hit_seg_cap;
  const HitSink sink{a.tmp_hits + seg0, a.tmp_aux + seg0, a.hit_seg_cap, &s_n};
  const bool small = a.bs1 < HG_TILE_BYTES;
  uint32_t staged_pattern = HG_NONE32;
  HugeUnit unit{};
  for (uint64_t tile = a.tile_begin + blockIdx.x; tile < a.tile_end; tile += gridDim.x) {
    const uint64_t tile_start = tile << HG_TILE_SHIFT;
    uint32_t rank_base = 0;
    for (uint32_t off = 0; off < HG_TILE_BYTES && tile_start + off < a.nbytes; off += 64) {
      const uint64_t p = tile_start + off + lane;
      const bool inside = p < a.nbytes;
      const bool starts = inside && (p == 0 || a.text[p - 1] == '\n');
      const bool is_nl = inside && a.text[p] == '\n';
      const uint64_t nlm = __builtin_amdgcn_ballot_w64(is_nl);
      for (uint64_t sm = __builtin_amdgcn_ballot_w64(starts); sm; sm &= sm - 1) {
        const uint32_t b = static_cast<uint32_t>(__builtin_ctzll(sm));
        const uint64_t s = tile_start + off + b;
        const uint32_t rank = rank_base + static_cast<uint32_t>(__popcll(nlm & ((1ull << b) - 1ull)));
        uint64_t line_no = hg_line_index(a.text, a.sums[tile], a.bases[tile], tile_start, rank, s, a.bs1, small);
        for (uint64_t ps = s;;) {
          const uint64_t limit = ps + a.bs1 < a.nbytes ? ps + a.bs1 : a.nbytes;
          uint64_t pa, pz;
          wave_trim_piece(a.text, ps, limit, lane, pa, pz);
          if (pz > pa) {
            const uint32_t len = static_cast<uint32_t>(pz - pa);
            for (uint32_t j = first; j < last; j++) {
              const uint32_t pi = a.db.slow[j];
              const HgPattern &pat = a.db.patterns[pi];
              if (pi != staged_pattern) {
                __syncthreads();
                unit = huge_prepare(hg_huge_view(a.db.pool, pat), s_dyn + 2 * nw_max, stage_cap, lane);
                staged_pattern = pi;
              }
              const uint32_t id = pat.id;
              const bool single = pat.single != 0;
              huge_run_unit(unit, S, T, a.text + pa, len, single, lane, [&](uint32_t to) { sink.push(a, line_no, id, to, pa, len, pi, single); });
            }
          }
          uint64_t q;
          if (pz > pa && a.text[pz - 1] == '\n') q = pz - 1;
          else q = wave_find(a.text, pz, limit, lane, [](uint32_t c) { return c == '\n'; });
          const bool nl = q < limit;
          const uint64_t e = nl ? q + 1 : limit;
          if (nl || e >= a.nbytes) break;
          ps = e;
          line_no++;
        }
      }
      rank_base += static_cast<uint32_t>(__popcll(nlm));
    }
  }
  flush_hits(a, &s_n, &s_base);
}

__global__ __launch_bounds__(64) void hg_block_huge_kernel(HgConfirmArgs a, uint32_t nw_max, uint32_t stage_cap, const uint32_t *pattern_flags) {
  __shared__ uint32_t s_n, s_base;
  if (threadIdx.x == 0) s_n = 0;
  __syncthreads();
  uint32_t *S = s_dyn, *T = s_dyn + nw_max;
  const uint32_t lane = threadIdx.x;
  const uint64_t seg0 = static_cast<uint64_t>(blockIdx.x) * a.hit_seg_cap;
  const HitSink sink{a.tmp_hits + seg0, a.tmp_aux + seg0, a.hit_seg_cap, &s_n};
  uint32_t seen = 0;
  for (uint32_t p = 0; p < a.db.npatterns; p++) {
    const HgPattern &pat = a.db.patterns[p];
    if (pat.nw <= HG_MAX_W) continue;
    if (seen++ % gridDim.x != blockIdx.x) continue;
    if (pat.tier == 0 && !pattern_flags[p]) continue;
    __syncthreads();
    const HugeUnit unit = huge_prepare(hg_huge_view(a.db.pool, pat), s_dyn + 2 * nw_max, stage_cap, lane);
    const uint32_t id = pat.id;
    const bool single = pat.single != 0;
    huge_run_unit(unit, S, T, a.text, a.nbytes, single, lane, [&](uint32_t to) { sink.push(a, 0, id, to, 0, static_cast<uint32_t>(a.nbytes), p, single); });
  }
  flush_hits(a, &s_n, &s_base);
}

template <typename K>
bool allow_lds(K kernel, size_t bytes) {
  if (bytes <= 48 * 1024) return true;
  return hipFuncSetAttribute(reinterpret_cast<const void *>(kernel), hipFuncAttributeMaxDynamicSharedMemorySize, static_cast<int>(bytes)) == hipSuccess;
}

}

static uint32_t clamp_stage(uint32_t nw_max, uint32_t stage_cap) {
  const size_t room = (160u * 1024u - 256u) / 4u;
  const size_t state = static_cast<size_t>(nw_max) * 2u;
  return static_cast<uint32_t>(state >= room ? 0u : std::min<size_t>(stage_cap, room - state));
}
size_t hg_huge_lds_bytes(uint32_t nw_max, uint32_t stage_cap) { return (static_cast<size_t>(nw_max) * 2u + clamp_stage(nw_max, stage_cap)) * 4u; }

bool hg_launch_confirm_huge(const HgConfirmArgs &a, uint32_t grid, uint32_t nw_max, uint32_t stage_cap, void *claim, uint32_t claim_mask, hipStream_t stream) {
  const size_t lds = hg_huge_lds_bytes(nw_max, stage_cap);
  if (!allow_lds(hg_confirm_huge_kernel, lds)) return false;
  hipLaunchKernelGGL(hg_confirm_huge_kernel, dim3(grid), dim3(64), lds, stream, a, nw_max, clamp_stage(nw_max, stage_cap), static_cast<unsigned long long *>(claim), claim_mask);
  return true;
}
bool hg_launch_always_on_huge(const HgConfirmArgs &a, uint32_t grid, uint32_t nw_max, uint32_t stage_cap, uint32_t first, uint32_t last, hipStream_t stream) {
  const size_t lds = hg_huge_lds_bytes(nw_max, stage_cap);
  if (!allow_lds(hg_always_on_huge_kernel, lds)) return false;
  hipLaunchKernelGGL(hg_always_on_huge_kernel, dim3(grid), dim3(64), lds, stream, a, nw_max, clamp_stage(nw_max, stage_cap), first, last);
// ... 9 lines not shown
```

hypergrep_amd/csrc/hg_kernels.hip:

```cpp
#include <hip/hip_runtime.h>
#include <cstdlib>

#include "hg_confirm_dev.h"
#include "hg_core.h"
#include "hg_engine.h"
#include "hg_post.h"
#include "hg_sink_dev.h"
#include "hg_tables_dev.h"

namespace {

__device__ __forceinline__ uint32_t wave_inclusive_scan(uint32_t v, uint32_t lane) {
#pragma unroll
  for (int o = 1; o < 64; o <<= 1) {
    uint32_t u = __shfl_up(v, o, 64);
    if (lane >= static_cast<uint32_t>(o)) v += u;
  }
  return v;
}

}

namespace {
constexpr int TS_THREADS = 256;
constexpr int TS_PER_THREAD = 4;

__device__ HgTileElem identity_elem() {
  HgTileElem e;
  e.k1 = e.d = e.new_cs = 0;
  e.has_nl = 0;
  e.pad = 0;
  return e;
}
__device__ HgTileElem block_scan(HgTileElem v, HgTileElem *sh, uint64_t bs1) {
  const int t = threadIdx.x;
  sh[t] = v;
  __syncthreads();
  for (int o = 1; o < TS_THREADS; o <<= 1) {
    HgTileElem left = identity_elem();
    if (t >= o) left = sh[t - o];
    __syncthreads();
    if (t >= o) {
      v = hg_tile_combine(left, v, bs1);
      sh[t] = v;
    }
    __syncthreads();
  }
  return v;
}
__device__ HgTileElem thread_elems(const HgTileSum *sums, uint64_t tile_end, uint64_t first, uint64_t bs1, HgTileElem *each) {
  HgTileElem acc = identity_elem();
  for (int k = 0; k < TS_PER_THREAD; k++) {
    uint64_t t = first + k;
    HgTileElem e = identity_elem();
    if (t < tile_end) e = hg_tile_elem(sums[t], t << HG_TILE_SHIFT);
    if (each) each[k] = e;
    acc = hg_tile_combine(acc, e, bs1);
  }
  return acc;
}
}

__global__ __launch_bounds__(TS_THREADS) void hg_tile_reduce_kernel(const HgTileSum *sums, uint64_t tile_begin, uint64_t tile_end, uint64_t bs1,
                                                                    HgTileElem *agg) {
  __shared__ HgTileElem sh[TS_THREADS];
  uint64_t first = tile_begin + (static_cast<uint64_t>(blockIdx.x) * TS_THREADS + threadIdx.x) * TS_PER_THREAD;
  HgTileElem v = thread_elems(sums, tile_end, first, bs1, nullptr);
  v = block_scan(v, sh, bs1);
  if (threadIdx.x == TS_THREADS - 1) agg[blockIdx.x] = v;
}

__global__ __launch_bounds__(TS_THREADS) void hg_tile_spine_kernel(const HgTileElem *agg, uint32_t nblocks, uint64_t bs1, HgTileBase *block_base,
                                                                   HgTileBase *state) {
  __shared__ HgTileElem sh[TS_THREADS];
  __shared__ HgTileBase carry;
  if (threadIdx.x == 0) carry = *state;
  __syncthreads();
  for (uint32_t base = 0; base < nblocks; base += TS_THREADS) {
    uint32_t i = base + threadIdx.x;
    HgTileElem v = identity_elem();
    if (i < nblocks) v = agg[i];
    HgTileElem inc = block_scan(v, sh, bs1);
    HgTileBase st = carry;
    HgTileElem excl = identity_elem();
    if (threadIdx.x > 0) excl = sh[threadIdx.x - 1];
    if (i < nblocks) block_base[i] = hg_tile_apply(st, excl, bs1);
    __syncthreads();
    if (threadIdx.x == TS_THREADS - 1) carry = hg_tile_apply(st, inc, bs1);
    __syncthreads();
  }
  if (threadIdx.x == 0) *state = carry;
}

__global__ __launch_bounds__(TS_THREADS) void hg_tile_apply_kernel(const HgTileSum *sums, uint64_t tile_begin, uint64_t tile_end, uint64_t bs1,
                                                                   const HgTileBase *block_base, HgTileBase *bases) {
  __shared__ HgTileElem sh[TS_THREADS];
  uint64_t first = tile_begin + (static_cast<uint64_t>(blockIdx.x) * TS_THREADS + threadIdx.x) * TS_PER_THREAD;
  HgTileElem each[TS_PER_THREAD];
  HgTileElem v = thread_elems(sums, tile_end, first, bs1, each);
  block_scan(v, sh, bs1);
  HgTileElem excl = identity_elem();
  if (threadIdx.x > 0) excl = sh[threadIdx.x - 1];
  HgTileBase st = hg_tile_apply(block_base[blockIdx.x], excl, bs1);
  for (int k = 0; k < TS_PER_THREAD; k++) {
    uint64_t t = first + k;
    if (t < tile_end) bases[t] = st;
    st = hg_tile_apply(st, each[k], bs1);
  }
}

__global__ __launch_bounds__(256) void hg_tile_inner_kernel(const uint8_t *text, HgTileSum *sums, uint64_t tile_begin, uint64_t tile_end, uint64_t bs1) {
  for (uint64_t t = tile_begin + static_cast<uint64_t>(blockIdx.x) * blockDim.x + threadIdx.x; t < tile_end; t += static_cast<uint64_t>(gridDim.x) * blockDim.x) {
    HgTileSum s = sums[t];
    if (s.nl_count < 2) continue;
    uint64_t base = t << HG_TILE_SHIFT;
    sums[t].inner = static_cast<uint32_t>(hg_inner_pieces(text, base + s.first_nl + 1, base + s.last_nl + 1, bs1));
  }
}

typedef uint32_t hg_u32x4_unaligned __attribute__((ext_vector_type(4), aligned(1)));

constexpr uint32_t VERIFY_STAGE_CAP = 768;
struct VerifyStage {
  HgDeferred item[VERIFY_STAGE_CAP];
  uint8_t bin[VERIFY_STAGE_CAP];
  uint32_t n;
  uint32_t bin_count[2 * HG_DEFER_SHARDS], bin_base[2 * HG_DEFER_SHARDS];
};
__device__ __forceinline__ void verify_stage_flush(const HgConfirmArgs &a, VerifyStage &st) {
  __syncthreads();
  const uint32_t n = st.n < VERIFY_STAGE_CAP ? st.n : VERIFY_STAGE_CAP;
  if (threadIdx.x < 2 * HG_DEFER_SHARDS) st.bin_count[threadIdx.x] = 0;
  __syncthreads();
  constexpr uint32_t PER_THREAD = (VERIFY_STAGE_CAP + 255) / 256;
  uint32_t rank[PER_THREAD];
#pragma unroll
  for (uint32_t q = 0; q < PER_THREAD; q++) {
    const uint32_t i = threadIdx.x + q * 256u;
    rank[q] = i < n ? atomicAdd(&st.bin_count[st.bin[i]], 1u) : 0u;
  }
  __syncthreads();
  if (threadIdx.x < 2 * HG_DEFER_SHARDS && st.bin_count[threadIdx.x])
    st.bin_base[threadIdx.x] = atomicAdd(&a.defer_count[HG_DEFER_SHARDS + threadIdx.x], st.bin_count[threadIdx.x]);
  __syncthreads();
#pragma unroll
  for (uint32_t q = 0; q < PER_THREAD; q++) {
    const uint32_t i = threadIdx.x + q * 256u;
    if (i < n) {
      const uint32_t bin = st.bin[i], m = 1u + bin / HG_DEFER_SHARDS, list = bin % HG_DEFER_SHARDS;
      const uint32_t slot = st.bin_base[bin] + rank[q];
      if (slot < a.defer_shard_cap) a.deferred[(static_cast<uint64_t>(a.list_of_mode[m]) * HG_DEFER_SHARDS + list) * a.defer_shard_cap + slot] = st.item[i];
      else atomicMax(&a.counters[HG_CNT_DEFER_NEED], slot + 1);
    }
  }
  __syncthreads();
  if (threadIdx.x == 0) st.n = 0;
  __syncthreads();
}

__device__ __forceinline__ uint32_t wtab_lookup(const HgWinBucket *tab, uint32_t bucket_mask, uint32_t folded) {
  for (uint32_t b = hg_wtab_bucket(folded, bucket_mask);; b = (b + 1u) & bucket_mask) {
    const uint4 *e = reinterpret_cast<const uint4 *>(tab + b);
    uint4 v = e[0], p = e[1];
    asm volatile("" : "+v"(v.x), "+v"(v.y), "+v"(v.z), "+v"(v.w), "+v"(p.x), "+v"(p.y), "+v"(p.z), "+v"(p.w));
    if (v.x == folded) return p.x;
    if (v.y == folded) return p.y;
    if (v.z == folded) return p.z;
    if (v.w == folded) return p.w;
    if (p.w == HG_WTAB_EMPTY) return HG_WTAB_EMPTY;
  }
}
__device__ __forceinline__ bool literal_occurs(const HgFactor *f, uint32_t len, const uint8_t *text, uint64_t fs, uint64_t readable) {
  const uint8_t *tp = text + fs;
  const uint32_t cb = f->casebits;
  uint32_t diff = 0;
  if (fs + (len > 16 ? 32u : 16u) <= readable) {
    const uint4 l0 = *reinterpret_cast<const uint4 *>(f->lit);
    const hg_u32x4_unaligned x0 = *reinterpret_cast<const hg_u32x4_unaligned *>(tp);
    diff = ((x0[0] ^ l0.x) & hg_factor_mask_dword(cb, len, 0)) | ((x0[1] ^ l0.y) & hg_factor_mask_dword(cb, len, 1)) |
           ((x0[2] ^ l0.z) & hg_factor_mask_dword(cb, len, 2)) | ((x0[3] ^ l0.w) & hg_factor_mask_dword(cb, len, 3));
    if (len > 16) {
      const uint4 l1 = *reinterpret_cast<const uint4 *>(f->lit + 16);
      const hg_u32x4_unaligned x1 = *reinterpret_cast<const hg_u32x4_unaligned *>(tp + 16);
      diff |= ((x1[0] ^ l1.x) & hg_factor_mask_dword(cb, len, 4)) | ((x1[1] ^ l1.y) & hg_factor_mask_dword(cb, len, 5)) |
              ((x1[2] ^ l1.z) & hg_factor_mask_dword(cb, len, 6)) | ((x1[3] ^ l1.w) & hg_factor_mask_dword(cb, len, 7));
    }
  } else {
    for (uint32_t b = 0; b < len; b++) diff |= (tp[b] ^ f->lit[b]) & (((cb >> b) & 1u) ? 0xDFu : 0xFFu);
  }
  return diff == 0;
// ... 104 lines not shown
          const uint4 hdr = *reinterpret_cast<const uint4 *>(f);
          const uint32_t len = hdr.y;
          if (pos >= off && pos - off + len <= a.nbytes) {
            const uint64_t fs = pos - off;
            const uint32_t diff = literal_occurs(f, len, a.text, fs, readable) ? 0u : 1u;
            if (diff == 0) {
              ok = true;
              mode = hdr.z;
              mode_rank = hdr.w;
              tag = hdr.x | (off << 24);
            }
          }
        }
      }
      if (!__builtin_amdgcn_ballot_w64(ok)) continue;
#pragma unroll
      for (uint32_t m = 0; m < HG_CONFIRM_MODES; m++) {
        const uint64_t mm = __builtin_amdgcn_ballot_w64(ok && mode == m);
        if (!mm) continue;
        if (STAGED && (m == 1 || m == 2)) {
          uint32_t at0 = 0;
          if (lane == 0) at0 = atomicAdd(&s_stage.n, static_cast<uint32_t>(__popcll(mm)));
          at0 = __builtin_amdgcn_readfirstlane(at0);
          if (ok && mode == m) {
            const uint32_t at = at0 + __builtin_amdgcn_mbcnt_hi(static_cast<uint32_t>(mm >> 32), __builtin_amdgcn_mbcnt_lo(static_cast<uint32_t>(mm), 0u));
            const uint32_t list = (mode_rank * a.list_spread[m] + blockIdx.x % a.list_spread[m]) % HG_DEFER_SHARDS;
            if (at < VERIFY_STAGE_CAP) {
              s_stage.item[at] = HgDeferred{pos, tag, o_rank};
              s_stage.bin[at] = static_cast<uint8_t>((m - 1u) * HG_DEFER_SHARDS + list);
            } else {
              const uint32_t slot = atomicAdd(&a.defer_count[m * HG_DEFER_SHARDS + list], 1u);
              if (slot < a.defer_shard_cap) a.deferred[(static_cast<uint64_t>(a.list_of_mode[m]) * HG_DEFER_SHARDS + list) * a.defer_shard_cap + slot] = HgDeferred{pos, tag, o_rank};
              else atomicMax(&a.counters[HG_CNT_DEFER_NEED], slot + 1);
            }
          }
          continue;
        }
        uint32_t slot0 = 0;
        if (lane == 0) slot0 = atomicAdd(&a.defer_count[m * HG_DEFER_SHARDS + shard], static_cast<uint32_t>(__popcll(mm)));
        slot0 = __builtin_amdgcn_readfirstlane(slot0);
        if (ok && mode == m) {
          const uint32_t slot = slot0 + __builtin_amdgcn_mbcnt_hi(static_cast<uint32_t>(mm >> 32), __builtin_amdgcn_mbcnt_lo(static_cast<uint32_t>(mm), 0u));
          if (slot < a.defer_shard_cap) a.deferred[(static_cast<uint64_t>(a.list_of_mode[m]) * HG_DEFER_SHARDS + shard) * a.defer_shard_cap + slot] = HgDeferred{pos, tag, o_rank};
          else atomicMax(&a.counters[HG_CNT_DEFER_NEED], slot + 1);
        }
      }
    }
  }
  if (STAGED) verify_stage_flush(a, s_stage);
#ifdef HG_PROFILE_CONFIRM
  if (lane == 0) a.tmp_hits[(6u << 20) + 65536u + blockIdx.x * 4u + wave] = HgHit{pf_t0, static_cast<uint32_t>(wall_clock64() - pf_t0), pf_rounds | (pf_pairs << 8)};
#endif
}
#ifndef HG_VERIFY_WAVES
#define HG_VERIFY_WAVES 4
#endif
#ifndef HG_LITERAL_WAVES
#define HG_LITERAL_WAVES 3
#endif
__global__ __launch_bounds__(256) __attribute__((amdgpu_waves_per_eu(HG_VERIFY_WAVES, HG_VERIFY_WAVES))) void hg_verify_kernel(HgConfirmArgs a) {
  __shared__ VerifyStage s_stage;
  verify_body<true>(a, &s_stage);
}
__global__ __launch_bounds__(256) __attribute__((amdgpu_waves_per_eu(HG_VERIFY_WAVES, HG_VERIFY_WAVES))) void hg_verify_lean_kernel(HgConfirmArgs a) { verify_body<false>(a, nullptr); }

template <int MODE>
__device__ __forceinline__ void confirm_body(const HgConfirmArgs &a, uint32_t vblock, uint32_t vgrid) {
  __shared__ uint32_t s_n, s_base;
  if (threadIdx.x == 0) s_n = 0;
  __syncthreads();
  const uint64_t seg0 = static_cast<uint64_t>(blockIdx.x) * a.hit_seg_cap;
  const HitSink sink{a.tmp_hits + seg0, a.tmp_aux + seg0, a.hit_seg_cap, &s_n};
  const uint32_t shard = vblock % HG_DEFER_SHARDS, peer = vblock / HG_DEFER_SHARDS, peers = (vgrid + HG_DEFER_SHARDS - 1 - shard) / HG_DEFER_SHARDS;
  const HgDeferred *dlist = a.deferred + (static_cast<uint64_t>(a.list_of_mode[MODE]) * HG_DEFER_SHARDS + shard) * a.defer_shard_cap;
  uint32_t n = a.defer_count[MODE * HG_DEFER_SHARDS + shard];
  if (n > a.defer_shard_cap) n = a.defer_shard_cap;
  for (uint32_t i = peer * blockDim.x + threadIdx.x; i < n; i += peers * blockDim.x) {
    const HgDeferred d = dlist[i];
    const uint32_t pattern = d.pattern & (HG_MAX_PATTERNS - 1u);
    const HgPattern &p = a.db.patterns[pattern];
    const uint32_t id = p.id;
    const bool single = MODE != 3 || p.single != 0;
    auto emit = [&](uint64_t line_no, uint32_t to, uint64_t start, uint32_t len) { sink.push(a, line_no, id, to, start, len, pattern, single); };
    if (MODE == 0) hgdev::confirm_literal(a.text, a.nbytes, a.sums, a.bases, a.bs1, d.pos, d.rank, d.pos - (d.pattern >> 24), p.max_len, emit);
    else hg_confirm(a.db, a.text, a.nbytes, a.sums, a.bases, a.bs1, d.pos, pattern, d.rank, emit);
  }
  flush_hits(a, &s_n, &s_base);
}

template <bool WITH_CONTEXT>
__device__ __forceinline__ void stage_tables(hgdev::lds_u32 *tab, const uint32_t *pool, const HgPattern &p, uint32_t nw, uint32_t lane) {
  const uint4 *rsrc = reinterpret_cast<const uint4 *>(pool + p.reach_off);
  const uint4 r0 = rsrc[lane];
  tab[CT_REACH + 4 * lane + 0] = r0.x; tab[CT_REACH + 4 * lane + 1] = r0.y; tab[CT_REACH + 4 * lane + 2] = r0.z; tab[CT_REACH + 4 * lane + 3] = r0.w;
  if (nw == 2) {
    const uint4 r1 = rsrc[64 + lane];
    tab[CT_REACH + 256 + 4 * lane + 0] = r1.x; tab[CT_REACH + 256 + 4 * lane + 1] = r1.y; tab[CT_REACH + 256 + 4 * lane + 2] = r1.z; tab[CT_REACH + 256 + 4 * lane + 3] = r1.w;
  }
  const uint32_t nfollow = p.nnodes * nw;
  for (uint32_t i = lane; i < nfollow; i += 64) tab[CT_FOLLOW + i] = pool[p.follow_off + i];
  if (WITH_CONTEXT) {
    if (lane < nw) tab[CT_INIT + lane] = pool[p.init_off + lane];
    if (lane < 16 * nw) tab[CT_AMASK + lane] = pool[p.amask_off + lane];
    if (lane < 20 * nw) tab[CT_ACC + lane] = pool[p.acc_off + lane];
  }
}

template <int MODE>
__device__ __forceinline__ void confirm_tables_body(const HgConfirmArgs &a, uint32_t vblock, uint32_t vgrid, uint32_t *s_tab) {
  __shared__ uint32_t s_n, s_base;
  if (threadIdx.x == 0) s_n = 0;
  __syncthreads();
  const uint64_t seg0 = static_cast<uint64_t>(blockIdx.x) * a.hit_seg_cap;
  const HitSink sink{a.tmp_hits + seg0, a.tmp_aux + seg0, a.hit_seg_cap, &s_n};
  const uint32_t lane = threadIdx.x & 63u, wave = threadIdx.x >> 6;
  hgdev::lds_u32 *tab = (hgdev::lds_u32 *)(&s_tab[0]) + wave * CT_WORDS;
  static_assert(HG_DEFER_SHARDS == 64, "one list per lane");
  uint32_t cnt = a.defer_count[MODE * HG_DEFER_SHARDS + lane];
  if (cnt > a.defer_shard_cap) cnt = a.defer_shard_cap;
  const uint32_t incl = wave_inclusive_scan(cnt, lane), start = incl - cnt;
  const uint32_t total = __shfl(incl, 63, 64);
  const uint32_t busy = total ? (total + HG_CONFIRM_THREADS - 1) / HG_CONFIRM_THREADS : 0u;
  if (busy < vgrid) vgrid = busy;
  if (vblock >= vgrid) return;
  const uint32_t lo = static_cast<uint32_t>(static_cast<uint64_t>(total) * vblock / vgrid), hi = static_cast<uint32_t>(static_cast<uint64_t>(total) * (vblock + 1) / vgrid);
  const HgDeferred *lists = a.deferred + static_cast<uint64_t>(a.list_of_mode[MODE]) * HG_DEFER_SHARDS * a.defer_shard_cap;
#ifdef HG_PROFILE_CONFIRM
  uint64_t pf_load = 0, pf_stage = 0, pf_run = 0;
  uint32_t pf_pats = 0;
#endif
  for (uint32_t g0 = lo + wave * 64u; g0 < hi; g0 += HG_CONFIRM_THREADS) {
#ifdef HG_PROFILE_CONFIRM
    uint64_t pf_t = wall_clock64();
#endif
    const uint32_t g = g0 + lane;
    uint32_t list = 0;
#pragma unroll
    for (uint32_t step = 32; step; step >>= 1) {
      const uint32_t probe = list + step;
      const uint32_t sp = __shfl(start, probe & 63u, 64);
      if (probe < 64u && sp <= g) list = probe;
    }
    const uint32_t l_start = __shfl(start, list, 64);
    const bool valid = g < hi;
    HgDeferred d{0, 0, 0};
    if (valid) d = lists[static_cast<uint64_t>(list) * a.defer_shard_cap + (g - l_start)];
    const uint32_t pattern = d.pattern & (HG_MAX_PATTERNS - 1u);
#ifdef HG_PROFILE_CONFIRM
    { const uint64_t n = wall_clock64(); pf_load += n - pf_t; pf_t = n; }
#endif
    for (uint64_t todo = __builtin_amdgcn_ballot_w64(valid); todo;) {
      const uint32_t pat = __builtin_amdgcn_readlane(pattern, __builtin_ctzll(todo));
      const bool mine = valid && pattern == pat;
      todo &= ~__builtin_amdgcn_ballot_w64(mine);
      const HgPattern &p = a.db.patterns[pat];
      const uint32_t nw = MODE == 1 ? 1u : p.nw;
      stage_tables<MODE == 2>(tab, a.db.pool, p, nw, lane);
      __builtin_amdgcn_fence(__ATOMIC_RELEASE, "wavefront");
      __builtin_amdgcn_wave_barrier();
#ifdef HG_PROFILE_CONFIRM
      { const uint64_t n = wall_clock64(); pf_stage += n - pf_t; pf_t = n; pf_pats++; }
#endif
      if (mine) {
        const uint32_t id = p.id;
        auto emit = [&](uint64_t line_no, uint32_t to, uint64_t start_, uint32_t len) { sink.push(a, line_no, id, to, start_, len, pat, true); };
        const uint64_t fs = d.pos - (d.pattern >> 24);
        const uint32_t lead = p.lit_lead;
        if (MODE == 1) {
          hgdev::confirm_simple(a.text, a.nbytes, a.sums, a.bases, a.bs1, d.pos, d.rank, fs, lead, p.init_word, p.acc_all, tab + CT_REACH, tab + CT_FOLLOW, emit);
        } else if (nw == 1) {
          hgdev::confirm_ctx<1>(a.text, a.nbytes, a.sums, a.bases, a.bs1, d.pos, d.rank, fs, lead, tab + CT_REACH, tab + CT_FOLLOW, tab + CT_INIT, tab + CT_AMASK,
                                    tab + CT_ACC, emit);
        } else {
          hgdev::confirm_ctx<2>(a.text, a.nbytes, a.sums, a.bases, a.bs1, d.pos, d.rank, fs, lead, tab + CT_REACH, tab + CT_FOLLOW, tab + CT_INIT, tab + CT_AMASK,
                                    tab + CT_ACC, emit);
        }
      }
      __builtin_amdgcn_wave_barrier();
#ifdef HG_PROFILE_CONFIRM
      { const uint64_t n = wall_clock64(); pf_run += n - pf_t; pf_t = n; }
#endif
    }
  }
#ifdef HG_PROFILE_CONFIRM
  if (lane == 0) a.tmp_hits[(6u << 20) + 32768u + blockIdx.x * (HG_CONFIRM_THREADS / 64) + wave] = HgHit{pf_load | (pf_stage << 32), static_cast<uint32_t>(pf_run), pf_pats | (MODE << 28)};
#endif
  flush_hits(a, &s_n, &s_base);
}

#ifdef HG_CONFIRM_WAVES
__attribute__((amdgpu_waves_per_eu(HG_CONFIRM_WAVES, HG_CONFIRM_WAVES)))
#endif
__global__ __launch_bounds__(HG_CONFIRM_THREADS) void hg_confirm_fast_kernel(HgConfirmArgs a, uint32_t blocks_per_mode) {
  uint32_t nmodes = 0;
  for (uint32_t m = 0; m < 3; m++) nmodes += a.mode_present[m] ? 1u : 0u;
  if (nmodes == 0) return;
  const uint32_t k = nmodes - 1u - blockIdx.x / blocks_per_mode, vblock = blockIdx.x % blocks_per_mode;
  uint32_t mode = 0, seen = 0;
  for (uint32_t m = 0; m < 3; m++)
    if (a.mode_present[m] && seen++ == k) mode = m;
  __shared__ __attribute__((aligned(16))) uint32_t s_tab[(HG_CONFIRM_THREADS / 64) * CT_WORDS];
#ifdef HG_PROFILE_CONFIRM
  const uint64_t t0 = wall_clock64();
#endif
  if (mode == 0) confirm_body<0>(a, vblock, blocks_per_mode);
  else if (mode == 1) confirm_tables_body<1>(a, vblock, blocks_per_mode, s_tab);
  else confirm_tables_body<2>(a, vblock, blocks_per_mode, s_tab);
#ifdef HG_PROFILE_CONFIRM
  if ((threadIdx.x & 63u) == 0) {
    const uint64_t t1 = wall_clock64();
    const uint32_t w = blockIdx.x * (HG_CONFIRM_THREADS / 64) + (threadIdx.x >> 6);
    a.tmp_hits[(6u << 20) + w] = HgHit{t0, static_cast<uint32_t>(t1 - t0), mode | (vblock << 4)};
  }
#endif
}
__global__ __launch_bounds__(256) void hg_confirm_generic_kernel(HgConfirmArgs a) { confirm_body<3>(a, blockIdx.x, gridDim.x); }
__attribute__((amdgpu_waves_per_eu(HG_LITERAL_WAVES, HG_LITERAL_WAVES)))
__global__ __launch_bounds__(256) void hg_confirm_literal_kernel(HgConfirmArgs a) { confirm_body<0>(a, blockIdx.x, gridDim.x); }

__global__ __launch_bounds__(256) void hg_block_mark_kernel(HgConfirmArgs a, uint32_t *pattern_flags) {
  const HgCand *cseg = a.cands + static_cast<uint64_t>(blockIdx.x) * a.cand_seg_cap;
  const uint32_t n = a.seg_count[blockIdx.x];
  for (uint32_t i = threadIdx.x; i < n; i += blockDim.x) {
    const HgCand c = cseg[i];
    hg_verify_window(a.db, a.text, a.nbytes, c.pos, c.word, [&](uint32_t pattern, uint64_t, uint32_t) { pattern_flags[pattern] = 1; });
  }
}

__global__ __launch_bounds__(256) void hg_block_scan_kernel(HgConfirmArgs a, const uint32_t *pattern_flags) {
  __shared__ uint32_t s_n, s_base;
  if (threadIdx.x == 0) s_n = 0;
  __syncthreads();
  const uint64_t seg0 = static_cast<uint64_t>(blockIdx.x) * a.hit_seg_cap;
  const HitSink sink{a.tmp_hits + seg0, a.tmp_aux + seg0, a.hit_seg_cap, &s_n};
  for (uint32_t p = blockIdx.x * blockDim.x + threadIdx.x; p < a.db.npatterns; p += gridDim.x * blockDim.x) {
    const HgPattern &pat = a.db.patterns[p];
    if (pat.tier == 0 && !pattern_flags[p]) continue;
    if (pat.tier == HG_TIER_COMB) continue;
    if (pat.nw > HG_MAX_W) continue;
    hg_nfa_scan(a.db.pool, pat, a.text, a.nbytes,
                [&](uint32_t to) { sink.push(a, 0, pat.id, to, 0, static_cast<uint32_t>(a.nbytes), p, pat.single != 0); });
  }
  flush_hits(a, &s_n, &s_base);
}

__global__ __launch_bounds__(256) void hg_block_small_kernel(HgDbView db, const uint8_t *h_text, uint32_t length, HgHit *h_out, uint32_t seg_cap, uint32_t *h_counts,
                                                             uint32_t *d_done, uint32_t *h_flag, uint32_t seq, uint32_t ppw) {
  __shared__ __attribute__((aligned(16))) uint8_t s_text[HG_BLOCK_SMALL_MAX + 16];
  __shared__ __attribute__((aligned(16))) uint32_t s_pool[HG_BLOCK_SMALL_POOL];
  __shared__ uint32_t s_seen[32 * HG_BLOCK_SLICED_WORDS];
  __shared__ uint32_t s_n;
  if (threadIdx.x == 0) s_n = 0;
  const uint32_t chunks = (length + 15u) >> 4;
  for (uint32_t i = threadIdx.x; i < chunks; i += blockDim.x) reinterpret_cast<uint4 *>(s_text)[i] = reinterpret_cast<const uint4 *>(h_text)[i];
  const uint32_t first = blockIdx.x * ppw, last = min(first + ppw, db.npatterns);
  const uint32_t npat = last - first;
  const HgPattern &pl = db.patterns[last - 1];
  const uint32_t lo = db.patterns[first].reach_off, hi = pl.acc_off + 20u * pl.nw;
  const bool staged = hi - lo <= HG_BLOCK_SMALL_POOL;
  if (staged)
    for (uint32_t i = threadIdx.x; i < hi - lo; i += blockDim.x) s_pool[i] = db.pool[lo + i];
  const bool sliced = ppw <= 32 && length <= HG_BLOCK_SLICED_MAX;
  uint32_t slice_len = length, nslices = 1;
  if (sliced) {
    const uint32_t most = blockDim.x / npat;
    slice_len = max(8u, (length + most - 1) / most);
    nslices = (length + slice_len - 1) / slice_len;
    const uint32_t words = (length >> 5) + 1;
    for (uint32_t i = threadIdx.x; i < npat * HG_BLOCK_SLICED_WORDS; i += blockDim.x)
      if ((i & (HG_BLOCK_SLICED_WORDS - 1)) < words) s_seen[i] = 0;
  }
  __syncthreads();
  const uint32_t j = threadIdx.x % npat, k = threadIdx.x / npat;
  if (k < nslices) {
    const HgPattern pat = db.patterns[first + j];
    const uint32_t single = pat.single ? HG_HIT_SINGLE_BIT : 0u;
    HgHit *seg = h_out + static_cast<uint64_t>(blockIdx.x) * seg_cap;
    auto emit = [&](uint32_t to) {
      if (sliced && (atomicOr(&s_seen[j * HG_BLOCK_SLICED_WORDS + (to >> 5)], 1u << (to & 31)) >> (to & 31) & 1)) return;
      const uint32_t slot = atomicAdd(&s_n, 1u);
      if (slot < seg_cap) seg[slot] = HgHit{0, pat.id, to | single};
    };
    const uint32_t from = k * slice_len, upto = min(from + slice_len, length);
    if (staged) {
      HgPattern q = pat;
      q.reach_off -= lo, q.follow_off -= lo, q.init_off -= lo, q.amask_off -= lo, q.acc_off -= lo;
      hg_nfa_scan_slice(s_pool, q, s_text, length, from, upto, emit);
    } else {
      hg_nfa_scan_slice(db.pool, pat, s_text, length, from, upto, emit);
    }
  }
  __syncthreads();
  if (threadIdx.x == 0) {
    h_counts[blockIdx.x] = s_n;
    __threadfence_system();
    if (atomicAdd(d_done, 1u) == gridDim.x - 1) {
      *d_done = 0;
      __threadfence_system();
      __hip_atomic_store(h_flag, seq, __ATOMIC_RELEASE, __HIP_MEMORY_SCOPE_SYSTEM);
    }
  }
}

__global__ void hg_reset_kernel(uint32_t *state, uint32_t state_words, HgTileBase *final_state, uint64_t carry_start, uint64_t first_piece, uint32_t *fill, uint32_t nb,
                                uint32_t *defer_count, uint32_t ndefer) {
  const uint32_t i0 = blockIdx.x * blockDim.x + threadIdx.x, stride = gridDim.x * blockDim.x;
  for (uint32_t i = i0; i < state_words; i += stride) state[i] = 0;
  for (uint32_t i = i0; i < HG_CNT_CURSORS; i += stride) state[HG_CNT_CURSOR0 + i] = 0;
  for (uint32_t i = i0; i < nb; i += stride) fill[i] = 0;
  for (uint32_t i = i0; i < ndefer; i += stride) defer_count[i] = 0;
  if (i0 == 0) *final_state = HgTileBase{carry_start, first_piece};
}

__device__ __forceinline__ uint64_t fin_key(const HgHit &h, uint32_t id_bits, uint32_t to_bits) {
  HgHit c = h;
  c.line_no = h.line_no >> HG_HIT_REL_SHIFT;
  c.to &= ~HG_HIT_SINGLE_BIT;
  return hg_sort_key_packed(c, (h.to & HG_HIT_SINGLE_BIT) != 0, id_bits, to_bits);
}
__global__ __launch_bounds__(256) void hg_fin_sort_small_kernel(const HgHit *hits, uint32_t *idx, const uint32_t *fill, uint32_t b_lo, uint32_t b_hi, uint32_t cap,
                                                                uint32_t id_bits, uint32_t to_bits, uint32_t *kept_count, uint32_t *big_list, uint32_t *big_count,
                                                                uint32_t big_stride) {
  const uint32_t lane = threadIdx.x & 63u, wave = (blockIdx.x * blockDim.x + threadIdx.x) >> 6, waves = (gridDim.x * blockDim.x) >> 6;
  const uint32_t group_shift = to_bits + 1;
  const uint4 *hits4 = reinterpret_cast<const uint4 *>(hits);
  static_assert(sizeof(HgHit) == 16, "one 16-byte load per record");
  uint32_t b = b_lo + wave;
  uint32_t n_next = b < b_hi ? fill[b] : 0u;
  uint4 h_next = make_uint4(0, 0, 0, 0);
  if (b < b_hi && lane < cap) h_next = hits4[static_cast<uint64_t>(b) * cap + lane];
  for (; b < b_hi; b += waves) {
    uint32_t n = n_next;
    const uint4 hv = h_next;
    const uint32_t bn = b + waves;
    n_next = bn < b_hi ? fill[bn] : 0u;
    h_next = make_uint4(0, 0, 0, 0);
    if (bn < b_hi && lane < cap) h_next = hits4[static_cast<uint64_t>(bn) * cap + lane];
    if (n > cap) n = cap;
    if (n > 64) {
      if (lane == 0) {
        const uint32_t cls = n <= HG_FIN_MEDIUM_CAP ? 0u : 1u;
        big_list[cls * big_stride + atomicAdd(big_count + cls, 1u)] = b;
      }
      continue;
    }
    if (n == 0) {
      if (lane == 0) kept_count[b] = 0;
      continue;
    }
    const uint32_t b0 = b * cap;
    const HgHit h{(static_cast<uint64_t>(hv.y) << 32) | hv.x, hv.z, hv.w};
    uint64_t k = lane < n ? fin_key(h, id_bits, to_bits) : ~0ull;
    uint32_t x = b0 + lane;
    if (n > 1) {
      const uint32_t klo = static_cast<uint32_t>(k), khi = static_cast<uint32_t>(k >> 32);
      const uint32_t nu = __builtin_amdgcn_readfirstlane(n);
      uint32_t rank = 0;
      for (uint32_t i = 0; i < nu; i++) {
        const uint64_t ki = (static_cast<uint64_t>(static_cast<uint32_t>(__builtin_amdgcn_readlane(khi, i))) << 32) | static_cast<uint32_t>(__builtin_amdgcn_readlane(klo, i));
        rank += (ki < k || (ki == k && i < lane)) ? 1u : 0u;
      }
      if (lane >= nu) rank = lane;
      const uint32_t slo = __builtin_amdgcn_ds_permute(rank << 2, klo), shi = __builtin_amdgcn_ds_permute(rank << 2, khi);
      x = __builtin_amdgcn_ds_permute(rank << 2, x);
      k = (static_cast<uint64_t>(shi) << 32) | slo;
    }
    const uint32_t plo = __shfl_up(static_cast<uint32_t>(k), 1, 64), phi = __shfl_up(static_cast<uint32_t>(k >> 32), 1, 64);
    const uint64_t prev = (static_cast<uint64_t>(phi) << 32) | plo;
    const bool valid = lane < n;
    const bool dup = valid && lane > 0 && (prev >> 1) == (k >> 1);
    const bool head = valid && (lane == 0 || (prev >> group_shift) != (k >> group_shift));
    const uint64_t head_mask = __builtin_amdgcn_ballot_w64(head), single_mask = __builtin_amdgcn_ballot_w64(valid && (k & 1u));
    const uint64_t upto = lane == 63 ? ~0ull : ((2ull << lane) - 1ull), below = (1ull << lane) - 1ull;
    const uint32_t group_start = 63u - static_cast<uint32_t>(__builtin_clzll((head_mask & upto) | 1ull));
    const bool earlier_single = (single_mask & below & ~((1ull << group_start) - 1ull)) != 0;
    const bool keep = valid && !dup && !((k & 1u) && earlier_single);
    const uint64_t km = __builtin_amdgcn_ballot_w64(keep);
    if (keep) idx[b0 + __builtin_amdgcn_mbcnt_hi(static_cast<uint32_t>(km >> 32), __builtin_amdgcn_mbcnt_lo(static_cast<uint32_t>(km), 0u))] = x;
    if (lane == 0) kept_count[b] = static_cast<uint32_t>(__popcll(km));
  }
}
template <uint32_t LCAP, bool IN_LDS>
__global__ __launch_bounds__(256) void hg_fin_sort_big_kernel(const HgHit *hits, uint32_t *idx, const uint32_t *fill, const uint32_t *big_list, const uint32_t *big_count,
                                                              uint32_t cap, uint32_t id_bits, uint32_t to_bits, uint32_t *kept_count, uint32_t *overflow, uint64_t *scratch_key,
                                                              uint32_t *scratch_idx) {
  __shared__ uint64_t l_key[IN_LDS ? LCAP : 1];
  __shared__ uint32_t l_idx[IN_LDS ? LCAP : 1];
  volatile uint64_t *s_key = IN_LDS ? l_key : scratch_key + static_cast<uint64_t>(blockIdx.x) * LCAP;
  volatile uint32_t *s_idx = IN_LDS ? l_idx : scratch_idx + static_cast<uint64_t>(blockIdx.x) * LCAP;
  const uint32_t tid = threadIdx.x, lane = tid & 63u;
  const uint32_t group_shift = to_bits + 1;
  const uint32_t nbig = *big_count;
  for (uint32_t q = blockIdx.x; q < nbig; q += gridDim.x) {
    const uint32_t b = big_list[q];
// ... 49 lines not shown
            }
          }
        }
        const uint64_t km = __builtin_amdgcn_ballot_w64(keep);
        if (keep) idx[b0 + kept + __builtin_amdgcn_mbcnt_hi(static_cast<uint32_t>(km >> 32), __builtin_amdgcn_mbcnt_lo(static_cast<uint32_t>(km), 0u))] = s_idx[i];
        kept += static_cast<uint32_t>(__popcll(km));
      }
      if (lane == 0) kept_count[b] = kept;
    }
    __syncthreads();
  }
}
template __global__ void hg_fin_sort_big_kernel<HG_FIN_MEDIUM_CAP, true>(const HgHit *, uint32_t *, const uint32_t *, const uint32_t *, const uint32_t *, uint32_t, uint32_t, uint32_t,
                                                                          uint32_t *, uint32_t *, uint64_t *, uint32_t *);
template __global__ void hg_fin_sort_big_kernel<HG_FIN_BUCKET_CAP, false>(const HgHit *, uint32_t *, const uint32_t *, const uint32_t *, const uint32_t *, uint32_t, uint32_t, uint32_t,
                                                                           uint32_t *, uint32_t *, uint64_t *, uint32_t *);
template <uint32_t HG_FIN_SCAN_THREADS>
__global__ __launch_bounds__(HG_FIN_SCAN_THREADS) void hg_fin_scan_kernel(uint32_t *kept_count, uint32_t b_lo, uint32_t b_hi, uint32_t *total, const uint32_t *fill,
                                                                          uint32_t cap, uint32_t *part, uint32_t epoch) {
  __shared__ uint32_t s_wave[HG_FIN_SCAN_THREADS / 64], s_raw[HG_FIN_SCAN_THREADS / 64], s_base[2];
  constexpr uint32_t WAVES = HG_FIN_SCAN_THREADS / 64;
  const uint32_t lane = threadIdx.x & 63u, wave = threadIdx.x >> 6;
  const uint32_t carry = total[0], carry_raw = total[1];
  const uint32_t nb = b_hi - b_lo;
  const uint32_t span = (((nb + gridDim.x - 1) / gridDim.x + WAVES * 64u - 1) / (WAVES * 64u)) * (WAVES * 64u);
  const uint32_t s_lo = b_lo + (blockIdx.x * span < nb ? blockIdx.x * span : nb);
  const uint32_t s_hi = s_lo + span < b_hi ? s_lo + span : b_hi;
  const uint32_t share = span / WAVES;
  const uint32_t w_lo = s_lo + wave * share < s_hi ? s_lo + wave * share : s_hi, w_hi = w_lo + share < s_hi ? w_lo + share : s_hi;
  uint32_t sum = 0, raw = 0;
#pragma unroll 4
  for (uint32_t i = w_lo + lane; i < w_hi; i += 64) {
    sum += kept_count[i];
    const uint32_t f = fill[i];
    raw += f < cap ? f : cap;
  }
  sum = wave_inclusive_scan(sum, lane);
  raw = wave_inclusive_scan(raw, lane);
  if (lane == 63) {
    s_wave[wave] = sum;
    s_raw[wave] = raw;
  }
  __syncthreads();
  uint32_t run = 0, all = 0, all_raw = 0;
#pragma unroll
  for (uint32_t w = 0; w < WAVES; w++) {
    const uint32_t t = s_wave[w];
    run += w < wave ? t : 0u;
    all += t;
    all_raw += s_raw[w];
  }
  if (threadIdx.x == 0) {
    part[3 * blockIdx.x] = all;
    part[3 * blockIdx.x + 1] = all_raw;
    __threadfence();
    __hip_atomic_store(&part[3 * blockIdx.x + 2], epoch, __ATOMIC_RELEASE, __HIP_MEMORY_SCOPE_AGENT);
  }
  if (wave == 0) {
    uint32_t before = 0, before_raw = 0;
    for (uint32_t p = lane; p < blockIdx.x; p += 64) {
      while (__hip_atomic_load(&part[3 * p + 2], __ATOMIC_ACQUIRE, __HIP_MEMORY_SCOPE_AGENT) != epoch) __builtin_amdgcn_s_sleep(2);
      before += __hip_atomic_load(&part[3 * p], __ATOMIC_RELAXED, __HIP_MEMORY_SCOPE_AGENT);
      before_raw += __hip_atomic_load(&part[3 * p + 1], __ATOMIC_RELAXED, __HIP_MEMORY_SCOPE_AGENT);
    }
    before = wave_inclusive_scan(before, lane);
    before_raw = wave_inclusive_scan(before_raw, lane);
    if (lane == 63) {
      s_base[0] = before;
      s_base[1] = before_raw;
    }
  }
  __syncthreads();
  run += carry + s_base[0];
  for (uint32_t i0 = w_lo; i0 < w_hi; i0 += 64) {
    const uint32_t i = i0 + lane;
    const uint32_t c = i < w_hi ? kept_count[i] : 0u;
    const uint32_t incl = wave_inclusive_scan(c, lane);
    if (i < w_hi) kept_count[i] = run + incl - c;
    run += __builtin_amdgcn_readlane(incl, 63);
  }
  if (blockIdx.x == gridDim.x - 1 && threadIdx.x == 0) {
    total[0] = carry + s_base[0] + all;
    total[1] = carry_raw + s_base[1] + all_raw;
  }
}
template __global__ void hg_fin_scan_kernel<512u>(uint32_t *, uint32_t, uint32_t, uint32_t *, const uint32_t *, uint32_t, uint32_t *, uint32_t);
template __global__ void hg_fin_scan_kernel<1024u>(uint32_t *, uint32_t, uint32_t, uint32_t *, const uint32_t *, uint32_t, uint32_t *, uint32_t);
__global__ void hg_fin_gather_kernel(const HgHit *hits, const HgHitAux *aux, const uint32_t *idx, const uint32_t *kept_base, const uint32_t *total, uint32_t b_lo,
                                     uint32_t b_hi, uint32_t cap, HgHit *oh, HgHitAux *oa) {
  const uint32_t lane = threadIdx.x & 63u, wave = (blockIdx.x * blockDim.x + threadIdx.x) >> 6, waves = (gridDim.x * blockDim.x) >> 6;
  auto base_of = [&](uint32_t b) { return b < b_hi ? kept_base[b] : *total; };
  uint32_t b = b_lo + wave;
  uint32_t k0_next = b < b_hi ? kept_base[b] : 0u, k1_next = b < b_hi ? base_of(b + 1) : 0u;
  uint32_t src_next = (b < b_hi && lane < cap) ? idx[b * cap + lane] : 0u;
  for (; b < b_hi; b += waves) {
    const uint32_t k0 = k0_next, n = k1_next - k0, b0 = b * cap;
    const uint32_t src0 = src_next;
    const uint32_t bn = b + waves;
    k0_next = bn < b_hi ? kept_base[bn] : 0u;
    k1_next = bn < b_hi ? base_of(bn + 1) : 0u;
    src_next = (bn < b_hi && lane < cap) ? idx[bn * cap + lane] : 0u;
    for (uint32_t i = lane; i < n; i += 64) {
      const uint32_t src = i < 64 ? src0 : idx[b0 + i];
      HgHit h = hits[src];
      h.to &= ~HG_HIT_SINGLE_BIT;
      h.line_no &= (1ull << HG_HIT_REL_SHIFT) - 1ull;
      oh[k0 + i] = h;
      oa[k0 + i] = aux[src];
    }
  }
}

__global__ void hg_key_kernel(const HgHit *hits, const HgHitAux *aux, const HgPattern *patterns, uint32_t n, uint64_t *key, uint32_t *idx) {
  uint32_t i = blockIdx.x * blockDim.x + threadIdx.x;
  if (i >= n) return;
  key[i] = hg_sort_key(hits[i], hg_report_single(patterns[aux[i].pattern]));
  idx[i] = i;
}
__global__ void hg_line_key_kernel(const HgHit *hits, const uint32_t *perm, uint32_t n, uint64_t *key) {
  uint32_t i = blockIdx.x * blockDim.x + threadIdx.x;
  if (i < n) key[i] = hits[perm[i]].line_no;
}
__global__ void hg_offset_kernel(uint32_t *idx, uint32_t n, uint32_t add) {
  uint32_t i = blockIdx.x * blockDim.x + threadIdx.x;
  if (i < n) idx[i] += add;
}
__global__ void hg_key_packed_kernel(const HgHit *hits, const HgHitAux *aux, const HgPattern *patterns, uint32_t n, uint32_t id_bits, uint32_t to_bits,
                                     uint64_t *key, uint32_t *idx) {
  uint32_t i = blockIdx.x * blockDim.x + threadIdx.x;
  if (i >= n) return;
  key[i] = hg_sort_key_packed(hits[i], hg_report_single(patterns[aux[i].pattern]), id_bits, to_bits);
  idx[i] = i;
}
__global__ void hg_keep_kernel(const HgHit *hits, const HgHitAux *aux, const uint32_t *perm, const HgPattern *patterns, uint32_t n, uint8_t *keep) {
  uint32_t i = blockIdx.x * blockDim.x + threadIdx.x;
  if (i >= n) return;
  keep[i] = hg_keep_hit_at([&](size_t j) { return hits[perm[j]]; }, [&](size_t j) { return hg_report_single(patterns[aux[perm[j]].pattern]); }, i) ? 1 : 0;
}
__global__ void hg_scatter_kernel(const HgHit *hits, const HgHitAux *aux, const uint32_t *perm, const uint8_t *keep, const uint32_t *pos, uint32_t n,
                                  HgHit *oh, HgHitAux *oa, uint32_t *count) {
  uint32_t i = blockIdx.x * blockDim.x + threadIdx.x;
  if (i >= n) return;
  if (keep[i]) {
    oh[pos[i]] = hits[perm[i]];
    oa[pos[i]] = aux[perm[i]];
  }
  if (i == n - 1) *count = pos[i] + keep[i];
}
```

hypergrep_amd/csrc/hg_post.h:

```cpp
#pragma once
#include "hg_core.h"

struct HgTileElem {
  uint64_t k1;
  uint64_t d;
  uint64_t new_cs;
  uint32_t has_nl, pad;
};

HG_HD HgTileElem hg_tile_elem(const HgTileSum &s, uint64_t tile_start) {
  HgTileElem e;
  e.has_nl = s.nl_count != 0;
  e.pad = 0;
  e.k1 = e.has_nl ? tile_start + s.first_nl + 1 : 0;
  e.d = e.has_nl ? s.inner : 0;
  e.new_cs = e.has_nl ? tile_start + s.last_nl + 1 : 0;
  return e;
}
HG_HD HgTileElem hg_tile_combine(const HgTileElem &a, const HgTileElem &b, uint64_t bs1) {
  if (!a.has_nl) return b;
  if (!b.has_nl) return a;
  HgTileElem r;
  r.has_nl = 1;
  r.pad = 0;
  r.k1 = a.k1;
  r.d = a.d + hg_pieces(b.k1 - a.new_cs, bs1) + b.d;
  r.new_cs = b.new_cs;
  return r;
}
HG_HD HgTileBase hg_tile_apply(const HgTileBase &st, const HgTileElem &e, uint64_t bs1) {
  if (!e.has_nl) return st;
  HgTileBase r;
  r.L = st.L + hg_pieces(e.k1 - st.cs, bs1) + e.d;
  r.cs = e.new_cs;
  return r;
}

HG_HD uint64_t hg_sort_key(const HgHit &h, uint32_t single) {
  return (static_cast<uint64_t>(h.id) << 32) | (static_cast<uint64_t>(h.to) << 1) | (single ? 1u : 0u);
}
HG_HD uint64_t hg_sort_key_packed(const HgHit &h, uint32_t single, uint32_t id_bits, uint32_t to_bits) {
  return (((h.line_no << id_bits) | h.id) << (to_bits + 1)) | (static_cast<uint64_t>(h.to) << 1) | (single ? 1u : 0u);
}
template <typename HitAt, typename SingleAt>
HG_HD bool hg_keep_hit_at(HitAt &&hit_at, SingleAt &&single_at, size_t i) {
  const HgHit h = hit_at(i);
  bool single = single_at(i);
  if (i > 0) {
    const HgHit p = hit_at(i - 1);
    if (p.line_no == h.line_no && p.id == h.id && p.to == h.to) {
      bool psingle = single_at(i - 1);
      if (!single) return false;
      if (!psingle) return false;
    }
  }
  if (!single) return true;
  for (size_t j = i; j > 0; j--) {
    const HgHit p = hit_at(j - 1);
    if (p.line_no != h.line_no || p.id != h.id) break;
    if (single_at(j - 1)) return false;
  }
  return true;
}
HG_HD bool hg_keep_hit(const HgHit *hits, const HgHitAux *aux, const HgPattern *patterns, size_t i) {
  const HgHit &h = hits[i];
  bool single = hg_report_single(patterns[aux[i].pattern]);
  if (i > 0) {
    const HgHit &p = hits[i - 1];
    if (p.line_no == h.line_no && p.id == h.id && p.to == h.to) {
      bool psingle = hg_report_single(patterns[aux[i - 1].pattern]);
      if (!single) return false;
      if (!psingle) return false;
    }
  }
  if (!single) return true;
  for (size_t j = i; j > 0; j--) {
    const HgHit &p = hits[j - 1];
    if (p.line_no != h.line_no || p.id != h.id) break;
    if (hg_report_single(patterns[aux[j - 1].pattern])) return false;
  }
  return true;
}
```

Measured before the change: 4938.

## Precompute per-tile line-index fields into a 32-byte tile base record

Widens HgTileBase to carry the line index at the first newline (L1) and first_nl offset, computed once in the tile apply kernel, so device confirm paths compute line numbers from one 32-byte record instead of reading both sums and bases. The scan-state carry moves to a separate HgTileState type. Separately, the work-list memset before the fin kernels is dropped: the fin scan kernel now zeroes those two words, and the spine kernel clears the defer counters. This trades a larger bases array and extra apply-time arithmetic for fewer scattered loads in confirmation and fewer host-issued memsets.

Result: no change. 4914 (-0.5%).

```diff
diff --git a/hypergrep_amd/csrc/hg_always_on.hip b/hypergrep_amd/csrc/hg_always_on.hip
--- a/hypergrep_amd/csrc/hg_always_on.hip
+++ b/hypergrep_amd/csrc/hg_always_on.hip
@@ -37,7 +37,7 @@
     for (uint64_t s = lo; s < hi; s++) {
       const bool starts = s == 0 || a.text[s - 1] == '\n';
       if (starts)
-        hg_scan_line_always_on(a.db, a.text, a.nbytes, a.sums, a.bases, a.bs1, s, rank, first, last,
+        hg_scan_line_always_on(a.db, a.text, a.nbytes, a.bases, a.bs1, s, rank, first, last,
                                [&](uint32_t pi, uint64_t line_no, uint32_t to, uint64_t start, uint32_t len) {
                                  sink.push(a, line_no, a.db.patterns[pi].id, to, start, len, pi, a.db.patterns[pi].single != 0);
                                });
@@ -901,7 +901,7 @@
     const HgDeferred d = list[i];
     const uint64_t end = d.pos, pos = end - 1;
     hgdev::PieceView pv;
-    if (!hgdev::piece_view(a.text, a.nbytes, a.sums, a.bases, a.bs1, pos, d.rank, pos, &pv)) continue;
+    if (!hgdev::piece_view(a.text, a.nbytes, a.bases, a.bs1, pos, d.rank, pos, &pv)) continue;
     if (!pv.whole) {
       if (pv.a > pos) continue;
       bool blocked = false;
diff --git a/hypergrep_amd/csrc/hg_confirm_dev.h b/hypergrep_amd/csrc/hg_confirm_dev.h
--- a/hypergrep_amd/csrc/hg_confirm_dev.h
+++ b/hypergrep_amd/csrc/hg_confirm_dev.h
@@ -142,7 +142,7 @@
   uint64_t line_no, a, limit;
   bool whole;
 };
-__device__ __forceinline__ bool piece_view(const uint8_t *text, uint64_t nbytes, const HgTileSum *sums, const HgTileBase *bases, uint64_t bs1, uint64_t pos,
+__device__ __forceinline__ bool piece_view(const uint8_t *text, uint64_t nbytes, const HgTileBase *bases, uint64_t bs1, uint64_t pos,
                                            uint32_t rank, uint64_t upto, PieceView *out) {
   const uint64_t t = pos >> HG_TILE_SHIFT, tile_start = t << HG_TILE_SHIFT;
   const HgTileBase tb = bases[t];
@@ -150,7 +150,7 @@
   const uint64_t k = (pos - h.s) / bs1;
   const uint64_t ps = h.s + k * bs1;
   out->limit = ps + bs1 < nbytes ? ps + bs1 : nbytes;
-  out->line_no = hg_line_index(text, sums[t], tb, tile_start, rank, h.s, bs1, bs1 < HG_TILE_BYTES) + k;
+  out->line_no = hg_line_index(text, tb, tile_start, rank, h.s, bs1, bs1 < HG_TILE_BYTES) + k;
   out->whole = k == 0;
   if (k == 0) {
     if (h.blocked) return false;
@@ -164,11 +164,11 @@
 }
 
 template <typename Emit>
-__device__ __forceinline__ void confirm_literal(const uint8_t *text, uint64_t nbytes, const HgTileSum *sums, const HgTileBase *bases, uint64_t bs1,
+__device__ __forceinline__ void confirm_literal(const uint8_t *text, uint64_t nbytes, const HgTileBase *bases, uint64_t bs1,
                                                 uint64_t pos, uint32_t rank, uint64_t fs, uint32_t len, Emit &&emit) {
   const uint32_t last_byte = text[fs + len - 1];
   PieceView pv;
-  if (!piece_view(text, nbytes, sums, bases, bs1, pos, rank, fs, &pv)) return;
+  if (!piece_view(text, nbytes, bases, bs1, pos, rank, fs, &pv)) return;
   const uint64_t from = fs + len;
   if (from > pv.limit) return;
   uint64_t a = pv.a;
@@ -185,10 +185,10 @@
   uint64_t line_no, a, limit, q;
   uint32_t pc;
 };
-__device__ __forceinline__ bool match_window(const uint8_t *text, uint64_t nbytes, const HgTileSum *sums, const HgTileBase *bases, uint64_t bs1, uint64_t pos,
+__device__ __forceinline__ bool match_window(const uint8_t *text, uint64_t nbytes, const HgTileBase *bases, uint64_t bs1, uint64_t pos,
                                              uint32_t rank, uint64_t fs, uint32_t lead, MatchWindow *w) {
   PieceView pv;
-  if (!piece_view(text, nbytes, sums, bases, bs1, pos, rank, pos, &pv)) return false;
+  if (!piece_view(text, nbytes, bases, bs1, pos, rank, pos, &pv)) return false;
   if (!pv.whole) {
     if (pv.a > pos) return false;
     for (uint64_t i = pv.a; i < pos; i++)
@@ -207,11 +207,11 @@
 }
 
 template <typename Emit>
-__device__ __forceinline__ void confirm_simple(const uint8_t *text, uint64_t nbytes, const HgTileSum *sums, const HgTileBase *bases, uint64_t bs1, uint64_t pos,
+__device__ __forceinline__ void confirm_simple(const uint8_t *text, uint64_t nbytes, const HgTileBase *bases, uint64_t bs1, uint64_t pos,
                                                    uint32_t rank, uint64_t fs, uint32_t lead, uint32_t init, uint32_t acc, const lds_u32 *reach, const lds_u32 *follow,
                                                    Emit &&emit) {
   MatchWindow w;
-  if (!match_window(text, nbytes, sums, bases, bs1, pos, rank, fs, lead, &w)) return;
+  if (!match_window(text, nbytes, bases, bs1, pos, rank, fs, lead, &w)) return;
   const uint64_t a = w.a, limit = w.limit, q = w.q;
   uint32_t S = 0, first_to = HG_NONE32;
   bool alive = true;
@@ -256,11 +256,11 @@
 }
 
 template <int NW, typename Emit>
-__device__ __forceinline__ void confirm_ctx(const uint8_t *text, uint64_t nbytes, const HgTileSum *sums, const HgTileBase *bases, uint64_t bs1, uint64_t pos,
+__device__ __forceinline__ void confirm_ctx(const uint8_t *text, uint64_t nbytes, const HgTileBase *bases, uint64_t bs1, uint64_t pos,
                                                 uint32_t rank, uint64_t fs, uint32_t lead, const lds_u32 *reach, const lds_u32 *follow, const lds_u32 *init,
                                                 const lds_u32 *amask, const lds_u32 *acct, Emit &&emit) {
   MatchWindow w;
-  if (!match_window(text, nbytes, sums, bases, bs1, pos, rank, fs, lead, &w)) return;
+  if (!match_window(text, nbytes, bases, bs1, pos, rank, fs, lead, &w)) return;
   const uint64_t a = w.a, limit = w.limit, q = w.q;
   uint32_t S[NW], I[NW];
 #pragma unroll
diff --git a/hypergrep_amd/csrc/hg_core.h b/hypergrep_amd/csrc/hg_core.h
--- a/hypergrep_amd/csrc/hg_core.h
+++ b/hypergrep_amd/csrc/hg_core.h
@@ -11,10 +11,17 @@
   uint32_t last_nl;
   uint32_t inner;
 };
-struct HgTileBase {
+struct HgTileState {
   uint64_t cs;
   uint64_t L;
 };
+struct HgTileBase {
+  uint64_t cs, L;
+  uint64_t L1;
+  uint32_t first_nl;
+  uint32_t pad;
+};
+static_assert(sizeof(HgTileBase) == 32, "one aligned 32-byte record per tile");
 struct HgCand {
   uint64_t pos;
   uint32_t word;
@@ -163,6 +170,22 @@
   if (!small) return base + (rank - 1);
   return base + hg_inner_pieces(text, after_first, s, bs1);
 }
+template <typename State>
+HG_HD HgTileBase hg_tile_base_record(const State &st, const HgTileSum &ts, uint64_t tile_start, uint64_t bs1) {
+  HgTileBase r;
+  r.cs = st.cs;
+  r.L = st.L;
+  r.L1 = ts.nl_count ? st.L + hg_pieces(tile_start + ts.first_nl + 1 - st.cs, bs1) : 0;
+  r.first_nl = ts.first_nl;
+  r.pad = 0;
+  return r;
+}
+HG_HD uint64_t hg_line_index(const uint8_t *text, const HgTileBase &tb, uint64_t tile_start, uint32_t rank, uint64_t s, uint64_t bs1,
+                             bool small) {
+  if (rank == 0) return tb.L;
+  if (!small) return tb.L1 + (rank - 1);
+  return tb.L1 + hg_inner_pieces(text, tile_start + tb.first_nl + 1, s, bs1);
+}
 
 HG_HD void hg_trim_piece(const uint8_t *text, uint64_t ps, uint64_t limit, uint64_t &a, uint64_t &z) {
   a = ps;
@@ -733,7 +756,7 @@
   }
   uint64_t k = (pos - s) / bs1;
   uint64_t ps = s + k * bs1;
-  uint64_t line_no = hg_line_index(text, sums[t], bases[t], tile_start, rank, s, bs1, bs1 < HG_TILE_BYTES) + k;
+  uint64_t line_no = hg_line_index(text, hg_tile_base_record(bases[t], sums[t], tile_start, bs1), tile_start, rank, s, bs1, bs1 < HG_TILE_BYTES) + k;
   uint64_t limit = ps + bs1 < nbytes ? ps + bs1 : nbytes;
   uint64_t a, z;
   hg_trim_piece(text, ps, limit, a, z);
@@ -745,19 +768,19 @@
 }
 
 template <typename Emit, typename Claim>
-HG_HD void hg_confirm(const HgDbView &db, const uint8_t *text, uint64_t nbytes, const HgTileSum *sums,
-                      const HgTileBase *bases, uint64_t bs1, uint64_t pos, uint32_t pattern, uint32_t rank, Emit &&emit, Claim &&claim) {
+HG_HD void hg_confirm_at(const HgDbView &db, const uint8_t *text, uint64_t nbytes, const HgTileBase &tb, uint64_t bs1, uint64_t pos, uint32_t pattern,
+                         uint32_t rank, Emit &&emit, Claim &&claim) {
   uint64_t t = pos >> HG_TILE_SHIFT, tile_start = t << HG_TILE_SHIFT;
   uint64_t s;
   if (rank == 0) {
-    s = bases[t].cs;
+    s = tb.cs;
   } else {
     s = pos;
     while (s > tile_start && text[s - 1] != '\n') s--;
   }
   uint64_t k = (pos - s) / bs1;
   uint64_t ps = s + k * bs1;
-  uint64_t line_no = hg_line_index(text, sums[t], bases[t], tile_start, rank, s, bs1, bs1 < HG_TILE_BYTES) + k;
+  uint64_t line_no = hg_line_index(text, tb, tile_start, rank, s, bs1, bs1 < HG_TILE_BYTES) + k;
   uint64_t limit = ps + bs1 < nbytes ? ps + bs1 : nbytes;
   uint64_t a, z;
   hg_trim_piece(text, ps, limit, a, z);
@@ -767,16 +790,27 @@
   hg_nfa_scan(db.pool, p, text + a, z - a, [&](uint32_t to) { emit(line_no, to, a, static_cast<uint32_t>(z - a)); });
 }
 template <typename Emit>
+HG_HD void hg_confirm(const HgDbView &db, const uint8_t *text, uint64_t nbytes, const HgTileBase *bases, uint64_t bs1, uint64_t pos, uint32_t pattern,
+                      uint32_t rank, Emit &&emit) {
+  hg_confirm_at(db, text, nbytes, bases[pos >> HG_TILE_SHIFT], bs1, pos, pattern, rank, emit, [](uint64_t) { return true; });
+}
+template <typename Emit, typename Claim>
+HG_HD void hg_confirm(const HgDbView &db, const uint8_t *text, uint64_t nbytes, const HgTileSum *sums,
+                      const HgTileBase *bases, uint64_t bs1, uint64_t pos, uint32_t pattern, uint32_t rank, Emit &&emit, Claim &&claim) {
+  const uint64_t t = pos >> HG_TILE_SHIFT;
+  hg_confirm_at(db, text, nbytes, hg_tile_base_record(bases[t], sums[t], t << HG_TILE_SHIFT, bs1), bs1, pos, pattern, rank, emit, claim);
+}
+template <typename Emit>
 HG_HD void hg_confirm(const HgDbView &db, const uint8_t *text, uint64_t nbytes, const HgTileSum *sums,
                       const HgTileBase *bases, uint64_t bs1, uint64_t pos, uint32_t pattern, uint32_t rank, Emit &&emit) {
   hg_confirm(db, text, nbytes, sums, bases, bs1, pos, pattern, rank, emit, [](uint64_t) { return true; });
 }
 
 template <typename Emit>
-HG_HD void hg_scan_line_always_on(const HgDbView &db, const uint8_t *text, uint64_t nbytes, const HgTileSum *sums,
-                                  const HgTileBase *bases, uint64_t bs1, uint64_t s, uint32_t rank, uint32_t first, uint32_t last, Emit &&emit) {
-  uint64_t t = s >> HG_TILE_SHIFT, tile_start = t << HG_TILE_SHIFT;
-  uint64_t line_no = hg_line_index(text, sums[t], bases[t], tile_start, rank, s, bs1, bs1 < HG_TILE_BYTES);
+HG_HD void hg_scan_line_always_on_at(const HgDbView &db, const uint8_t *text, uint64_t nbytes, const HgTileBase &tb, uint64_t bs1, uint64_t s, uint32_t rank,
+                                     uint32_t first, uint32_t last, Emit &&emit) {
+  uint64_t tile_start = s >> HG_TILE_SHIFT << HG_TILE_SHIFT;
+  uint64_t line_no = hg_line_index(text, tb, tile_start, rank, s, bs1, bs1 < HG_TILE_BYTES);
   uint64_t ps = s;
   for (;;) {
     uint64_t limit = ps + bs1 < nbytes ? ps + bs1 : nbytes;
@@ -799,3 +833,14 @@
     line_no++;
   }
 }
+template <typename Emit>
+HG_HD void hg_scan_line_always_on(const HgDbView &db, const uint8_t *text, uint64_t nbytes, const HgTileBase *bases, uint64_t bs1, uint64_t s, uint32_t rank,
+                                  uint32_t first, uint32_t last, Emit &&emit) {
+  hg_scan_line_always_on_at(db, text, nbytes, bases[s >> HG_TILE_SHIFT], bs1, s, rank, first, last, emit);
+}
+template <typename Emit>
+HG_HD void hg_scan_line_always_on(const HgDbView &db, const uint8_t *text, uint64_t nbytes, const HgTileSum *sums,
+                                  const HgTileBase *bases, uint64_t bs1, uint64_t s, uint32_t rank, uint32_t first, uint32_t last, Emit &&emit) {
+  const uint64_t t = s >> HG_TILE_SHIFT;
+  hg_scan_line_always_on_at(db, text, nbytes, hg_tile_base_record(bases[t], sums[t], t << HG_TILE_SHIFT, bs1), bs1, s, rank, first, last, emit);
+}
diff --git a/hypergrep_amd/csrc/hg_engine.h b/hypergrep_amd/csrc/hg_engine.h
--- a/hypergrep_amd/csrc/hg_engine.h
+++ b/hypergrep_amd/csrc/hg_engine.h
@@ -213,7 +213,8 @@
   uint32_t defer_spread_boost_ = 1;
   bool hit_direct_ = false;
   HgTileSum *d_sums_ = nullptr;
-  HgTileBase *d_bases_ = nullptr, *d_block_base_ = nullptr, *d_final_ = nullptr;
+  HgTileBase *d_bases_ = nullptr;
+  HgTileState *d_block_base_ = nullptr, *d_final_ = nullptr;
   HgTileElem *d_agg_ = nullptr;
   HgCand *d_cands_ = nullptr;
   HgDeferred *d_deferred_ = nullptr;
@@ -233,7 +234,7 @@
   void *d_temp_ = nullptr;
   size_t temp_bytes_ = 0;
   uint32_t *h_counters_ = nullptr;
-  HgTileBase *h_final_ = nullptr;
+  HgTileState *h_final_ = nullptr;
   hipEvent_t ev_[4] = {nullptr, nullptr, nullptr, nullptr};
   static constexpr int kMaxChunks = 64;
   hipStream_t side_stream_ = nullptr;
diff --git a/hypergrep_amd/csrc/hg_engine.hip b/hypergrep_amd/csrc/hg_engine.hip
--- a/hypergrep_amd/csrc/hg_engine.hip
+++ b/hypergrep_amd/csrc/hg_engine.hip
@@ -14,8 +14,9 @@
 bool hg_launch_stream_join(const HgStreamArgs &a, uint32_t grid, hipStream_t stream);
 int hg_stream_blocks_per_cu(uint32_t filter_log2, uint32_t filter_wide, uint32_t dense);
 __global__ void hg_tile_reduce_kernel(const HgTileSum *sums, uint64_t tile_begin, uint64_t tile_end, uint64_t bs1, HgTileElem *agg);
-__global__ void hg_tile_spine_kernel(const HgTileElem *agg, uint32_t nblocks, uint64_t bs1, HgTileBase *block_base, HgTileBase *state);
-__global__ void hg_tile_apply_kernel(const HgTileSum *sums, uint64_t tile_begin, uint64_t tile_end, uint64_t bs1, const HgTileBase *block_base,
+__global__ void hg_tile_spine_kernel(const HgTileElem *agg, uint32_t nblocks, uint64_t bs1, HgTileState *block_base, HgTileState *state, uint32_t *defer_count,
+                                     uint32_t defer_clear);
+__global__ void hg_tile_apply_kernel(const HgTileSum *sums, uint64_t tile_begin, uint64_t tile_end, uint64_t bs1, const HgTileState *block_base,
                                      HgTileBase *bases);
 __global__ void hg_tile_inner_kernel(const uint8_t *text, HgTileSum *sums, uint64_t tile_begin, uint64_t tile_end, uint64_t bs1);
 __global__ void hg_verify_kernel(HgConfirmArgs a);
@@ -28,7 +29,7 @@
 __global__ void hg_block_scan_kernel(HgConfirmArgs a, const uint32_t *pattern_flags);
 __global__ void hg_block_small_kernel(HgDbView db, const uint8_t *h_text, uint32_t length, HgHit *h_out, uint32_t seg_cap, uint32_t *h_counts, uint32_t *d_done,
                                       uint32_t *h_flag, uint32_t seq, uint32_t ppw);
-__global__ void hg_reset_kernel(uint32_t *state, uint32_t state_words, HgTileBase *final_state, uint64_t carry_start, uint64_t first_piece, uint32_t *fill, uint32_t nb, uint32_t *defer_count,
+__global__ void hg_reset_kernel(uint32_t *state, uint32_t state_words, HgTileState *final_state, uint64_t carry_start, uint64_t first_piece, uint32_t *fill, uint32_t nb, uint32_t *defer_count,
                                 uint32_t ndefer);
 __global__ void hg_fin_sort_small_kernel(const HgHit *hits, uint32_t *idx, const uint32_t *fill, uint32_t b_lo, uint32_t b_hi, uint32_t cap, uint32_t id_bits,
                                          uint32_t to_bits, uint32_t *kept_count, uint32_t *big_list, uint32_t *big_count, uint32_t big_stride);
@@ -199,10 +200,10 @@
   HG_TRY(hipMemset(d_counters_, 0, HG_ST_ALLOC_WORDS * 4), "clear state");
   d_fin_total_ = d_counters_ + HG_ST_FIN_TOTAL;
   d_selected_ = d_counters_ + HG_ST_SELECTED;
-  d_final_ = reinterpret_cast<HgTileBase *>(d_counters_ + HG_ST_FINAL);
+  d_final_ = reinterpret_cast<HgTileState *>(d_counters_ + HG_ST_FINAL);
   HG_TRY(hgmem::dev_alloc(&d_pflags_, db.patterns.size() * 4 + 16, "d_pflags_"), "alloc pattern flags");
   HG_TRY(hgmem::host_alloc(&h_counters_, (HG_CNT_WORDS + 4 + HG_DEFER_SHARDS) * 4, "h_counters_"), "alloc pinned");
-  h_final_ = reinterpret_cast<HgTileBase *>(h_counters_ + HG_ST_FINAL);
+  h_final_ = reinterpret_cast<HgTileState *>(h_counters_ + HG_ST_FINAL);
   for (auto &ev : ev_) HG_TRY(hipEventCreate(&ev), "hipEventCreate");
   HG_TRY(hipStreamCreateWithFlags(&side_stream_, hipStreamNonBlocking), "hipStreamCreate");
   HG_TRY(hipEventCreateWithFlags(&ev_fin_early_, hipEventDisableTiming), "hipEventCreate");
@@ -454,7 +455,6 @@
 int HgScanner::launch_fin(const PassPlan &p, hipStream_t s, uint32_t lo, uint32_t hi, bool beside_stream) {
   if (hi <= lo) return HG_OK;
   const uint32_t nbk = hi - lo, cu = static_cast<uint32_t>(num_cus_), fin_cap = p.fin_cap, id_bits = p.id_bits, to_bits = p.to_bits;
-  HG_TRY(hipMemsetAsync(d_fin_total_ + 2, 0, 8, s), "memset work list");
   hipLaunchKernelGGL(hg_fin_sort_small_kernel, dim3(std::min<uint32_t>((nbk + 3) / 4, cu * 8)), dim3(256), 0, s, d_hits_raw_, d_perm_a_, d_fin_fill_, lo, hi, fin_cap, id_bits, to_bits,
                      d_fin_kept_, d_fin_big_, d_fin_total_ + 2, fin_alloc_);
   hipLaunchKernelGGL((hg_fin_sort_big_kernel<HG_FIN_MEDIUM_CAP, true>), dim3(std::min<uint32_t>(nbk, cu * 4)), dim3(256), 0, s, d_hits_raw_, d_perm_a_, d_fin_fill_, d_fin_big_, d_fin_total_ + 2,
@@ -545,8 +545,9 @@
     uint32_t blocks = static_cast<uint32_t>(std::min<uint64_t>((span + 255) / 256, 4096));
     hipLaunchKernelGGL(hg_tile_inner_kernel, dim3(blocks), dim3(256), 0, side, p.text, d_sums_, t0, t1, p.bs1);
   }
+  const uint32_t defer_clear = (c > 0 && p.has_anchored) ? HG_CONFIRM_MODES * HG_DEFER_SHARDS : 0u;
   hipLaunchKernelGGL(hg_tile_reduce_kernel, dim3(nblocks), dim3(256), 0, side, d_sums_, t0, t1, p.bs1, d_agg_);
-  hipLaunchKernelGGL(hg_tile_spine_kernel, dim3(1), dim3(256), 0, side, d_agg_, nblocks, p.bs1, d_block_base_, d_final_);
+  hipLaunchKernelGGL(hg_tile_spine_kernel, dim3(1), dim3(256), 0, side, d_agg_, nblocks, p.bs1, d_block_base_, d_final_, d_defer_count_, defer_clear);
   hipLaunchKernelGGL(hg_tile_apply_kernel, dim3(nblocks), dim3(256), 0, side, d_sums_, t0, t1, p.bs1, d_block_base_, d_bases_);
   HG_TRY(hipGetLastError(), "tile scan launch");
   if (p.piped && c + 1 == p.nchunks) HG_TRY(hipEventRecord(ev_tile_done_, side), "event");
@@ -561,7 +562,6 @@
     const uint32_t huge_blocks = db_->n_confirm_mode[4] ? std::max<uint32_t>(HG_DEFER_SHARDS, static_cast<uint32_t>(num_cus_) * static_cast<uint32_t>(std::max<size_t>(1, std::min<size_t>(8, (160u << 10) / std::max<size_t>(hg_huge_lds_bytes(db_->huge_max_nw, db_->huge_stage_words), 1))))) : 0u;
     confirm_blocks = std::max(std::max(mode_blocks * std::max(fast_modes, 1u), verify_blocks), huge_blocks);
     ca.hit_seg_cap = hit_cap_ / confirm_blocks;
-    if (c > 0) HG_TRY(hipMemsetAsync(d_defer_count_, 0, HG_CONFIRM_MODES * HG_DEFER_SHARDS * 4, side), "memset deferred counts");
     if (ca.mode_present[1] || ca.mode_present[2]) hipLaunchKernelGGL(hg_verify_kernel, dim3(verify_blocks), dim3(256), 0, side, ca);
     else hipLaunchKernelGGL(hg_verify_lean_kernel, dim3(verify_blocks), dim3(256), 0, side, ca);
     const bool literal_only_set = ca.mode_present[0] && !ca.mode_present[1] && !ca.mode_present[2];
diff --git a/hypergrep_amd/csrc/hg_huge.hip b/hypergrep_amd/csrc/hg_huge.hip
--- a/hypergrep_amd/csrc/hg_huge.hip
+++ b/hypergrep_amd/csrc/hg_huge.hip
@@ -334,7 +334,7 @@
     uint32_t mine = 0;
     if (lane == 0) mine = claim_piece(claim, claim_mask, ps, pattern) ? 1u : 0u;
     if (!__builtin_amdgcn_readfirstlane(mine)) continue;
-    const uint64_t line_no = hg_line_index(a.text, a.sums[t], a.bases[t], tile_start, d.rank, s, a.bs1, a.bs1 < HG_TILE_BYTES) + k;
+    const uint64_t line_no = hg_line_index(a.text, a.bases[t], tile_start, d.rank, s, a.bs1, a.bs1 < HG_TILE_BYTES) + k;
     const uint64_t limit = ps + a.bs1 < a.nbytes ? ps + a.bs1 : a.nbytes;
     uint64_t pa, pz;
     wave_trim_piece(a.text, ps, limit, lane, pa, pz);
@@ -376,7 +376,7 @@
         const uint32_t b = static_cast<uint32_t>(__builtin_ctzll(sm));
         const uint64_t s = tile_start + off + b;
         const uint32_t rank = rank_base + static_cast<uint32_t>(__popcll(nlm & ((1ull << b) - 1ull)));
-        uint64_t line_no = hg_line_index(a.text, a.sums[tile], a.bases[tile], tile_start, rank, s, a.bs1, small);
+        uint64_t line_no = hg_line_index(a.text, a.bases[tile], tile_start, rank, s, a.bs1, small);
         for (uint64_t ps = s;;) {
           const uint64_t limit = ps + a.bs1 < a.nbytes ? ps + a.bs1 : a.nbytes;
           uint64_t pa, pz;
diff --git a/hypergrep_amd/csrc/hg_kernels.hip b/hypergrep_amd/csrc/hg_kernels.hip
--- a/hypergrep_amd/csrc/hg_kernels.hip
+++ b/hypergrep_amd/csrc/hg_kernels.hip
@@ -48,14 +48,14 @@
   }
   return v;
 }
-__device__ HgTileElem thread_elems(const HgTileSum *sums, uint64_t tile_end, uint64_t first, uint64_t bs1, HgTileElem *each) {
+__device__ HgTileElem thread_elems(const HgTileSum *sums, uint64_t tile_end, uint64_t first, uint64_t bs1, HgTileSum *own) {
   HgTileElem acc = identity_elem();
   for (int k = 0; k < TS_PER_THREAD; k++) {
     uint64_t t = first + k;
-    HgTileElem e = identity_elem();
-    if (t < tile_end) e = hg_tile_elem(sums[t], t << HG_TILE_SHIFT);
-    if (each) each[k] = e;
-    acc = hg_tile_combine(acc, e, bs1);
+    HgTileSum s{0, HG_NONE32, HG_NONE32, 0};
+    if (t < tile_end) s = sums[t];
+    if (own) own[k] = s;
+    acc = hg_tile_combine(acc, hg_tile_elem(s, t << HG_TILE_SHIFT), bs1);
   }
   return acc;
 }
@@ -70,10 +70,11 @@
   if (threadIdx.x == TS_THREADS - 1) agg[blockIdx.x] = v;
 }
 
-__global__ __launch_bounds__(TS_THREADS) void hg_tile_spine_kernel(const HgTileElem *agg, uint32_t nblocks, uint64_t bs1, HgTileBase *block_base,
-                                                                   HgTileBase *state) {
+__global__ __launch_bounds__(TS_THREADS) void hg_tile_spine_kernel(const HgTileElem *agg, uint32_t nblocks, uint64_t bs1, HgTileState *block_base,
+                                                                   HgTileState *state, uint32_t *defer_count, uint32_t defer_clear) {
   __shared__ HgTileElem sh[TS_THREADS];
-  __shared__ HgTileBase carry;
+  __shared__ HgTileState carry;
+  for (uint32_t i = threadIdx.x; i < defer_clear; i += TS_THREADS) defer_count[i] = 0;
   if (threadIdx.x == 0) carry = *state;
   __syncthreads();
   for (uint32_t base = 0; base < nblocks; base += TS_THREADS) {
@@ -81,7 +82,7 @@
     HgTileElem v = identity_elem();
     if (i < nblocks) v = agg[i];
     HgTileElem inc = block_scan(v, sh, bs1);
-    HgTileBase st = carry;
+    HgTileState st = carry;
     HgTileElem excl = identity_elem();
     if (threadIdx.x > 0) excl = sh[threadIdx.x - 1];
     if (i < nblocks) block_base[i] = hg_tile_apply(st, excl, bs1);
@@ -93,19 +94,19 @@
 }
 
 __global__ __launch_bounds__(TS_THREADS) void hg_tile_apply_kernel(const HgTileSum *sums, uint64_t tile_begin, uint64_t tile_end, uint64_t bs1,
-                                                                   const HgTileBase *block_base, HgTileBase *bases) {
+                                                                   const HgTileState *block_base, HgTileBase *bases) {
   __shared__ HgTileElem sh[TS_THREADS];
   uint64_t first = tile_begin + (static_cast<uint64_t>(blockIdx.x) * TS_THREADS + threadIdx.x) * TS_PER_THREAD;
-  HgTileElem each[TS_PER_THREAD];
-  HgTileElem v = thread_elems(sums, tile_end, first, bs1, each);
+  HgTileSum own[TS_PER_THREAD];
+  HgTileElem v = thread_elems(sums, tile_end, first, bs1, own);
   block_scan(v, sh, bs1);
   HgTileElem excl = identity_elem();
   if (threadIdx.x > 0) excl = sh[threadIdx.x - 1];
-  HgTileBase st = hg_tile_apply(block_base[blockIdx.x], excl, bs1);
+  HgTileState st = hg_tile_apply(block_base[blockIdx.x], excl, bs1);
   for (int k = 0; k < TS_PER_THREAD; k++) {
     uint64_t t = first + k;
-    if (t < tile_end) bases[t] = st;
-    st = hg_tile_apply(st, each[k], bs1);
+    if (t < tile_end) bases[t] = hg_tile_base_record(st, own[k], t << HG_TILE_SHIFT, bs1);
+    st = hg_tile_apply(st, hg_tile_elem(own[k], t << HG_TILE_SHIFT), bs1);
   }
 }
 
@@ -376,8 +377,8 @@
     const uint32_t id = p.id;
     const bool single = MODE != 3 || p.single != 0;
     auto emit = [&](uint64_t line_no, uint32_t to, uint64_t start, uint32_t len) { sink.push(a, line_no, id, to, start, len, pattern, single); };
-    if (MODE == 0) hgdev::confirm_literal(a.text, a.nbytes, a.sums, a.bases, a.bs1, d.pos, d.rank, d.pos - (d.pattern >> 24), p.max_len, emit);
-    else hg_confirm(a.db, a.text, a.nbytes, a.sums, a.bases, a.bs1, d.pos, pattern, d.rank, emit);
+    if (MODE == 0) hgdev::confirm_literal(a.text, a.nbytes, a.bases, a.bs1, d.pos, d.rank, d.pos - (d.pattern >> 24), p.max_len, emit);
+    else hg_confirm(a.db, a.text, a.nbytes, a.bases, a.bs1, d.pos, pattern, d.rank, emit);
   }
   flush_hits(a, &s_n, &s_base);
 }
@@ -461,12 +462,12 @@
         const uint64_t fs = d.pos - (d.pattern >> 24);
         const uint32_t lead = p.lit_lead;
         if (MODE == 1) {
-          hgdev::confirm_simple(a.text, a.nbytes, a.sums, a.bases, a.bs1, d.pos, d.rank, fs, lead, p.init_word, p.acc_all, tab + CT_REACH, tab + CT_FOLLOW, emit);
+          hgdev::confirm_simple(a.text, a.nbytes, a.bases, a.bs1, d.pos, d.rank, fs, lead, p.init_word, p.acc_all, tab + CT_REACH, tab + CT_FOLLOW, emit);
         } else if (nw == 1) {
-          hgdev::confirm_ctx<1>(a.text, a.nbytes, a.sums, a.bases, a.bs1, d.pos, d.rank, fs, lead, tab + CT_REACH, tab + CT_FOLLOW, tab + CT_INIT, tab + CT_AMASK,
+          hgdev::confirm_ctx<1>(a.text, a.nbytes, a.bases, a.bs1, d.pos, d.rank, fs, lead, tab + CT_REACH, tab + CT_FOLLOW, tab + CT_INIT, tab + CT_AMASK,
                                     tab + CT_ACC, emit);
         } else {
-          hgdev::confirm_ctx<2>(a.text, a.nbytes, a.sums, a.bases, a.bs1, d.pos, d.rank, fs, lead, tab + CT_REACH, tab + CT_FOLLOW, tab + CT_INIT, tab + CT_AMASK,
+          hgdev::confirm_ctx<2>(a.text, a.nbytes, a.bases, a.bs1, d.pos, d.rank, fs, lead, tab + CT_REACH, tab + CT_FOLLOW, tab + CT_INIT, tab + CT_AMASK,
                                     tab + CT_ACC, emit);
         }
       }
@@ -596,14 +597,14 @@
   }
 }
 
-__global__ void hg_reset_kernel(uint32_t *state, uint32_t state_words, HgTileBase *final_state, uint64_t carry_start, uint64_t first_piece, uint32_t *fill, uint32_t nb,
+__global__ void hg_reset_kernel(uint32_t *state, uint32_t state_words, HgTileState *final_state, uint64_t carry_start, uint64_t first_piece, uint32_t *fill, uint32_t nb,
                                 uint32_t *defer_count, uint32_t ndefer) {
   const uint32_t i0 = blockIdx.x * blockDim.x + threadIdx.x, stride = gridDim.x * blockDim.x;
   for (uint32_t i = i0; i < state_words; i += stride) state[i] = 0;
   for (uint32_t i = i0; i < HG_CNT_CURSORS; i += stride) state[HG_CNT_CURSOR0 + i] = 0;
   for (uint32_t i = i0; i < nb; i += stride) fill[i] = 0;
   for (uint32_t i = i0; i < ndefer; i += stride) defer_count[i] = 0;
-  if (i0 == 0) *final_state = HgTileBase{carry_start, first_piece};
+  if (i0 == 0) *final_state = HgTileState{carry_start, first_piece};
 }
 
 __device__ __forceinline__ uint64_t fin_key(const HgHit &h, uint32_t id_bits, uint32_t to_bits) {
@@ -819,6 +820,8 @@
   if (blockIdx.x == gridDim.x - 1 && threadIdx.x == 0) {
     total[0] = carry + s_base[0] + all;
     total[1] = carry_raw + s_base[1] + all_raw;
+    total[2] = 0;
+    total[3] = 0;
   }
 }
 template __global__ void hg_fin_scan_kernel<512u>(uint32_t *, uint32_t, uint32_t, uint32_t *, const uint32_t *, uint32_t, uint32_t *, uint32_t);
diff --git a/hypergrep_amd/csrc/hg_post.h b/hypergrep_amd/csrc/hg_post.h
--- a/hypergrep_amd/csrc/hg_post.h
+++ b/hypergrep_amd/csrc/hg_post.h
@@ -28,14 +28,14 @@
   r.new_cs = b.new_cs;
   return r;
 }
-HG_HD HgTileBase hg_tile_apply(const HgTileBase &st, const HgTileElem &e, uint64_t bs1) {
+template <typename State>
+HG_HD State hg_tile_apply(const State &st, const HgTileElem &e, uint64_t bs1) {
   if (!e.has_nl) return st;
-  HgTileBase r;
+  State r = st;
   r.L = st.L + hg_pieces(e.k1 - st.cs, bs1) + e.d;
   r.cs = e.new_cs;
   return r;
 }
-
 HG_HD uint64_t hg_sort_key(const HgHit &h, uint32_t single) {
   return (static_cast<uint64_t>(h.id) << 32) | (static_cast<uint64_t>(h.to) << 1) | (single ? 1u : 0u);
 }
```
